# ha7ilm/csdr

Measured on AMD Instinct MI355X. Metric: complex MS/s in->out, WFM demod chain @2.4 MS/s x N streams, higher is better.
Workload: dtype f32

## Files before the change

### csdr_amd/__init__.py

```python
import ctypes as C
import os
import sys
import subprocess
import numpy as np

HERE = os.path.dirname(os.path.abspath(__file__))
LIB_PATH = os.environ.get("CSDR_AMD_LIB") or os.path.join(HERE, "libcsdr_amd.so")
ROOT = os.path.dirname(HERE)

c64 = np.complex64
f32 = np.float32

SHIFT = {"addition": 0, "math": 1, "table": 2, "unroll": 3, "addfast": 4}
WINDOWS = {"BOXCAR": 0, "BLACKMAN": 1, "HAMMING": 2}


class CsdrAmdError(RuntimeError):
    pass


def build(verbose=False):
    r = subprocess.run(["make", "-C", os.path.join(HERE, "csrc"), "-j8"], capture_output=True, text=True)
    if r.returncode != 0:
        raise CsdrAmdError("libcsdr_amd build failed:\n" + r.stdout[-4000:] + r.stderr[-4000:])
    if verbose:
        print(r.stdout)
    return LIB_PATH


class FastDDC(C.Structure):
    _fields_ = [(n, C.c_int) for n in ("pre_decimation", "post_decimation", "taps_length", "taps_min_length",
                                       "overlap_length", "fft_size", "fft_inv_size", "input_size", "post_input_size")] + \
               [("pre_shift", C.c_float), ("startbin", C.c_int), ("v", C.c_int), ("offsetbin", C.c_int),
                ("post_shift", C.c_float), ("output_scrape", C.c_int), ("scrap", C.c_int),
                ("sindelta", C.c_float), ("cosdelta", C.c_float), ("rate", C.c_float)]

    def as_dict(self):
        d = {n: getattr(self, n) for n, _ in self._fields_ if n not in ("sindelta", "cosdelta", "rate")}
        d["dsadata"] = (self.sindelta, self.cosdelta, self.rate)
        return d


_lib = None


def lib():
    global _lib
    if _lib is not None:
        return _lib
    if not os.path.exists(LIB_PATH):
        raise CsdrAmdError("%s is missing -- run `python -c 'import __graft_entry__ as g; g.build()'` first" % LIB_PATH)
    if "torch" not in sys.modules and not os.environ.get("CSDR_AMD_NO_TORCH_PRELOAD"):
        try:
            import torch
        except Exception:
            pass
    L = C.CDLL(LIB_PATH)
    vp, sz, i, fl = C.c_void_p, C.c_size_t, C.c_int, C.c_float
    L.csdr_amd_ctx_create.restype = vp; L.csdr_amd_ctx_create.argtypes = [i, vp]
    L.csdr_amd_ctx_destroy.argtypes = [vp]
    L.csdr_amd_ctx_sync.argtypes = [vp]
    L.csdr_amd_ctx_stream.restype = vp; L.csdr_amd_ctx_stream.argtypes = [vp]
    L.csdr_amd_last_error.restype = C.c_char_p
    L.csdr_amd_device_arch.restype = C.c_char_p; L.csdr_amd_device_arch.argtypes = [vp]
    L.csdr_amd_malloc.restype = vp; L.csdr_amd_malloc.argtypes = [vp, sz]
    L.csdr_amd_free.argtypes = [vp, vp]
    L.csdr_amd_h2d.argtypes = [vp, vp, vp, sz]
    L.csdr_amd_d2h.argtypes = [vp, vp, vp, sz]
    L.csdr_amd_memset.argtypes = [vp, vp, i, sz]
    sh = C.c_short
    L.csdr_amd_d2d.argtypes = [vp, vp, vp, sz]
    L.csdr_amd_amdemod_cf.argtypes = [vp, vp, vp, sz]
    L.csdr_amd_amdemod_estimator_cf.argtypes = [vp, vp, vp, sz, fl, fl]
    L.csdr_amd_realpart_cf.argtypes = [vp, vp, vp, sz]
    L.csdr_amd_logpower_cf.argtypes = [vp, vp, vp, sz, fl]
    L.csdr_amd_fmdemod_atan_cf.argtypes = [vp, vp, vp, i, sz, sz, sz, vp]
    L.csdr_amd_dcblock_ff.argtypes = [vp, vp, vp, i, sz, sz, sz, fl, vp]
    L.csdr_amd_fastdcblock_ff.argtypes = [vp, vp, vp, i, i, i, sz, sz, vp]
    L.csdr_amd_agc_ff.argtypes = [vp, vp, vp, i, sz, i, sz, sz, fl, fl, fl, fl, sh, sh, fl, vp]
    L.csdr_amd_precalculate_window.argtypes = [vp, i, i]; L.csdr_amd_precalculate_window.restype = None
    L.csdr_amd_fftcc_create.restype = vp; L.csdr_amd_fftcc_create.argtypes = [vp, i, i, i, i]
    L.csdr_amd_fftcc_destroy.argtypes = [vp]; L.csdr_amd_fftcc_destroy.restype = None
    L.csdr_amd_fftcc_process.argtypes = [vp, vp, sz, vp, C.POINTER(sz)]
    L.csdr_amd_encode_ima_adpcm_i16_u8.argtypes = [vp, vp, vp, i, sz, sz, sz, vp]
    L.csdr_amd_decode_ima_adpcm_u8_i16.argtypes = [vp, vp, vp, i, sz, sz, sz, vp]
    L.csdr_amd_compress_fft_adpcm_f_u8.argtypes = [vp, vp, vp, i, i]
    L.csdr_amd_waterfall_create.restype = vp; L.csdr_amd_waterfall_create.argtypes = [vp, i, i, i, i, fl, i, i, i, sz]
    L.csdr_amd_waterfall_process.argtypes = [vp, vp, sz, sz, vp, sz, C.POINTER(i)]
    L.csdr_amd_waterfall_reset.argtypes = [vp]
    L.csdr_amd_waterfall_kernel_name.restype = C.c_char_p; L.csdr_amd_waterfall_kernel_name.argtypes = [vp]
    L.csdr_amd_waterfall_force_generic.argtypes = [vp, i]
    L.csdr_amd_waterfall_destroy.argtypes = [vp]; L.csdr_amd_waterfall_destroy.restype = None
    ll = C.c_longlong
    L.csdr_amd_resampler_create.restype = vp; L.csdr_amd_resampler_create.argtypes = [vp, i, i, vp, i, i]
    L.csdr_amd_resampler_process.argtypes = [vp, vp, ll, sz, vp, sz, C.POINTER(ll)]
    L.csdr_amd_resampler_max_out.restype = ll; L.csdr_amd_resampler_max_out.argtypes = [vp, ll]
    L.csdr_amd_resampler_reset.argtypes = [vp]
    L.csdr_amd_resampler_set_cli_bufsize.argtypes = [vp, i]
    L.csdr_amd_resampler_set_last_taps_delay.argtypes = [vp, i]
    L.csdr_amd_resampler_force_generic.argtypes = [vp, i]
    L.csdr_amd_resampler_kernel_name.restype = C.c_char_p; L.csdr_amd_resampler_kernel_name.argtypes = [vp]
    L.csdr_amd_resampler_destroy.argtypes = [vp]; L.csdr_amd_resampler_destroy.restype = None
    L.csdr_amd_resampler_window.argtypes = [i, i, i, i, i, vp]
    L.csdr_amd_interp_create.restype = vp; L.csdr_amd_interp_create.argtypes = [vp, i, vp, i, i]
    L.csdr_amd_interp_process.argtypes = [vp, vp, ll, sz, vp, sz, C.POINTER(ll)]
    L.csdr_amd_interp_max_out.restype = ll; L.csdr_amd_interp_max_out.argtypes = [vp, ll]
    L.csdr_amd_interp_reset.argtypes = [vp]
    L.csdr_amd_interp_set_cli_bufsize.argtypes = [vp, i]
    L.csdr_amd_interp_force_generic.argtypes = [vp, i]
    L.csdr_amd_interp_kernel_name.restype = C.c_char_p; L.csdr_amd_interp_kernel_name.argtypes = [vp]
    L.csdr_amd_interp_destroy.argtypes = [vp]; L.csdr_amd_interp_destroy.restype = None
    L.csdr_amd_psk31_create.restype = vp; L.csdr_amd_psk31_create.argtypes = [vp, vp, i, i, i]
    L.csdr_amd_psk31_process.argtypes = [vp, vp, ll, sz, vp, sz, vp, vp, vp]
    L.csdr_amd_psk31_max_out.restype = ll; L.csdr_amd_psk31_max_out.argtypes = [vp, ll]
    L.csdr_amd_psk31_reset.argtypes = [vp]
    L.csdr_amd_psk31_reset_channel.argtypes = [vp, i]
    L.csdr_amd_psk31_get_channel.argtypes = [vp, i, vp]
    L.csdr_amd_psk31_set_channel.argtypes = [vp, i, vp]
    L.csdr_amd_psk31_set_lanes.argtypes = [vp, i]
    L.csdr_amd_psk31_force_generic.argtypes = [vp, i]
    L.csdr_amd_psk31_lanes.argtypes = [vp]
    L.csdr_amd_psk31_kernel_name.restype = C.c_char_p; L.csdr_amd_psk31_kernel_name.argtypes = [vp]
    L.csdr_amd_psk31_destroy.argtypes = [vp]; L.csdr_amd_psk31_destroy.restype = None
    L.csdr_amd_simple_agc_cc.argtypes = [vp, vp, vp, i, ll, sz, sz, C.c_float, C.c_float, C.c_float, vp]
    L.csdr_amd_psk31_varicode_decoder_push.restype = C.c_char; L.csdr_amd_psk31_varicode_decoder_push.argtypes = [vp, C.c_ubyte]
    L.csdr_amd_psk31_varicode_table.restype = None; L.csdr_amd_psk31_varicode_table.argtypes = [vp]
    L.csdr_amd_debug_psk31_walk.restype = ll; L.csdr_amd_debug_psk31_walk.argtypes = [vp, i, i, vp, ll, vp, i, vp, vp, vp, vp]
    L.csdr_amd_rtty_create.restype = vp; L.csdr_amd_rtty_create.argtypes = [vp, vp, i, i, i]
    L.csdr_amd_rtty_process.argtypes = [vp, vp, ll, sz, vp, sz, vp]
    L.csdr_amd_rtty_max_out.restype = ll; L.csdr_amd_rtty_max_out.argtypes = [vp, ll]
    L.csdr_amd_rtty_reset.argtypes = [vp]
    L.csdr_amd_rtty_reset_channel.argtypes = [vp, i]
    L.csdr_amd_rtty_force_generic.argtypes = [vp, i]
    L.csdr_amd_rtty_kernel_name.restype = C.c_char_p; L.csdr_amd_rtty_kernel_name.argtypes = [vp]
    L.csdr_amd_rtty_destroy.argtypes = [vp]; L.csdr_amd_rtty_destroy.restype = None
    L.csdr_amd_bfsk_demod_cf.argtypes = [vp, vp, vp, i, ll, sz, sz, vp, vp, i, i]
    L.csdr_amd_bfsk_last_kernel.restype = C.c_char_p; L.csdr_amd_bfsk_last_kernel.argtypes = []
    L.csdr_amd_binary_slicer_f_u8.argtypes = [vp, vp, vp, i, ll, sz, sz]
    L.csdr_amd_rtty_line_decoder_u8_u8.argtypes = [vp, vp, vp, i, ll, sz, sz, vp, vp]
    L.csdr_amd_serial_line_decoder_f_u8.argtypes = [vp, vp, vp, i, i, sz, sz, C.c_float, i, C.c_float, C.c_float, vp, vp]
    L.csdr_amd_rtty_baudot_decoder_lookup.restype = C.c_char; L.csdr_amd_rtty_baudot_decoder_lookup.argtypes = [vp, C.c_ubyte]
    L.csdr_amd_rtty_baudot_decoder_push.restype = C.c_char; L.csdr_amd_rtty_baudot_decoder_push.argtypes = [vp, C.c_ubyte]
    L.csdr_amd_firdes_add_peak_c.restype = None; L.csdr_amd_firdes_add_peak_c.argtypes = [vp, i, C.c_float, i, i, i]
    L.csdr_amd_firdes_peak_c.restype = None; L.csdr_amd_firdes_peak_c.argtypes = [vp, i, C.c_float, i]
    L.csdr_amd_debug_rtty_walk.restype = ll; L.csdr_amd_debug_rtty_walk.argtypes = [vp, i, i, vp, ll, vp, i, vp]
    L.csdr_amd_squelch_create.restype = vp; L.csdr_amd_squelch_create.argtypes = [vp, i, i, i, vp, ll]
    L.csdr_amd_squelch_process.argtypes = [vp, vp, ll, sz, vp, sz, vp, sz, vp, vp]
    L.csdr_amd_squelch_set_level.argtypes = [vp, i, fl]
    L.csdr_amd_squelch_get_level.restype = fl; L.csdr_amd_squelch_get_level.argtypes = [vp, i]
    L.csdr_amd_squelch_block_index.restype = ll; L.csdr_amd_squelch_block_index.argtypes = [vp, i]
    L.csdr_amd_squelch_max_blocks.argtypes = [vp]
    L.csdr_amd_squelch_reset.argtypes = [vp]
    L.csdr_amd_squelch_reset_channel.argtypes = [vp, i]
    L.csdr_amd_squelch_force_generic.argtypes = [vp, i]
    L.csdr_amd_squelch_kernel_name.restype = C.c_char_p; L.csdr_amd_squelch_kernel_name.argtypes = [vp]
    L.csdr_amd_squelch_destroy.argtypes = [vp]; L.csdr_amd_squelch_destroy.restype = None
    L.csdr_amd_get_power_c.argtypes = [vp, vp, i, i, i, i, sz, vp]
    L.csdr_amd_get_power_f.argtypes = [vp, vp, i, i, i, i, sz, vp]
    L.csdr_amd_squelch_report_due.argtypes = [i, ll]
    L.csdr_amd_squelch_gate_open.argtypes = [fl, fl]
    L.csdr_amd_debug_squelch_power.restype = fl; L.csdr_amd_debug_squelch_power.argtypes = [vp, i, i, i]
    L.csdr_amd_costas_params.argtypes = [fl, fl, i, vp]
    L.csdr_amd_pll_params_p.argtypes = [fl, vp]
    L.csdr_amd_pll_params_pi.argtypes = [fl, fl, fl, fl, vp]
    L.csdr_amd_carrier_create.restype = vp; L.csdr_amd_carrier_create.argtypes = [vp, vp, i]
    L.csdr_amd_carrier_process.argtypes = [vp, vp, ll, sz, vp, vp, vp, vp, sz]
    L.csdr_amd_carrier_reset.argtypes = [vp]
    L.csdr_amd_carrier_reset_channel.argtypes = [vp, i]
    L.csdr_amd_carrier_get_channel.argtypes = [vp, i, vp]
    L.csdr_amd_carrier_set_channel.argtypes = [vp, i, vp]
    L.csdr_amd_carrier_set_lanes.argtypes = [vp, i]
    L.csdr_amd_carrier_lanes.argtypes = [vp]
    L.csdr_amd_carrier_force_generic.argtypes = [vp, i]
    L.csdr_amd_carrier_kernel_name.restype = C.c_char_p; L.csdr_amd_carrier_kernel_name.argtypes = [vp]
    L.csdr_amd_carrier_destroy.argtypes = [vp]; L.csdr_amd_carrier_destroy.restype = None
    L.csdr_amd_debug_carrier_walk.restype = ll; L.csdr_amd_debug_carrier_walk.argtypes = [vp, vp, ll, vp, i, vp, vp, vp, vp, vp]
    L.csdr_amd_fmmod_fc.argtypes = [vp, vp, vp, i, sz, sz, sz, vp]
    L.csdr_amd_dsb_fc.argtypes = [vp, vp, vp, sz, fl]
    L.csdr_amd_add_dcoffset_cc.argtypes = [vp, vp, vp, sz]
    L.csdr_amd_fixed_amplitude_cc.argtypes = [vp, vp, vp, sz, fl]
    L.csdr_amd_convert_f_samplerf.argtypes = [vp, vp, vp, sz, C.c_uint]
    L.csdr_amd_debug_fmmod_walk.restype = ll; L.csdr_amd_debug_fmmod_walk.argtypes = [vp, ll, vp, i, vp, vp, vp]
    L.csdr_amd_txbank_create.restype = vp; L.csdr_amd_txbank_create.argtypes = [vp, i, i, fl, fl, i, vp, i, vp, i, sz]
    L.csdr_amd_txbank_process.argtypes = [vp, vp, sz, ll, vp, sz, C.POINTER(ll)]
    L.csdr_amd_txbank_set_rate.argtypes = [vp, i, fl]
    L.csdr_amd_txbank_get_rate.restype = fl; L.csdr_amd_txbank_get_rate.argtypes = [vp, i]
    L.csdr_amd_txbank_reset.argtypes = [vp]
    L.csdr_amd_txbank_max_out.restype = ll; L.csdr_amd_txbank_max_out.argtypes = [vp, ll]
    L.csdr_amd_txbank_force_generic.argtypes = [vp, i]
    L.csdr_amd_txbank_kernel_name.restype = C.c_char_p; L.csdr_amd_txbank_kernel_name.argtypes = [vp]
    L.csdr_amd_txbank_destroy.argtypes = [vp]; L.csdr_amd_txbank_destroy.restype = None
    L.csdr_amd_rational_resampler_get_lowpass_f.restype = None; L.csdr_amd_rational_resampler_get_lowpass_f.argtypes = [vp, i, i, i, i]
    L.csdr_amd_debug_resampler_schedule.argtypes = [i, i, i, i, i, vp]
    L.csdr_amd_logaveragepower_cf.argtypes = [vp, vp, vp, i, i, i, fl]
    L.csdr_amd_fft_exchange_sides_ff.argtypes = [vp, vp, vp, i, i]
    L.csdr_amd_accumulate_power_cf.argtypes = [vp, vp, vp, sz]
    L.csdr_amd_log_ff.argtypes = [vp, vp, vp, sz, fl]
    L.csdr_amd_timer_start.argtypes = [vp]
    L.csdr_amd_timer_stop_ms.argtypes = [vp, C.POINTER(fl)]
    L.csdr_amd_firdes_filter_len.argtypes = [fl]
    L.csdr_amd_firdes_lowpass_f.argtypes = [vp, i, fl, i]
    L.csdr_amd_firdes_bandpass_c.argtypes = [vp, i, fl, fl, i]
    L.csdr_amd_nfm_deemph_taps.argtypes = [i, C.POINTER(vp)]
    L.csdr_amd_shift_addition_init.argtypes = [fl, vp]
    for nm in ("u8_f", "s8_f", "s16_f", "f_u8", "f_s8", "f_s16"):
        getattr(L, "csdr_amd_convert_" + nm).argtypes = [vp, vp, vp, sz]
    L.csdr_amd_convert_f_s24.argtypes = [vp, vp, vp, sz, i]
    L.csdr_amd_convert_s24_f.argtypes = [vp, vp, vp, sz, i]
    L.csdr_amd_rotator_generate.argtypes = [vp, i, fl, C.POINTER(fl), vp, sz, i, i]
    L.csdr_amd_mix_cc.argtypes = [vp, vp, vp, vp, i, sz, sz, sz]
    L.csdr_amd_mix_fc.argtypes = [vp, vp, vp, vp, i, sz, sz, sz]
    L.csdr_amd_shift_cc.argtypes = [vp, i, fl, C.POINTER(fl), vp, vp, i, sz, sz, sz, i, i]
    L.csdr_amd_decimating_shift_addition_cc.argtypes = [vp, vp, vp, i, i, sz, sz, vp, i, vp]
    L.csdr_amd_fir_decimate_cc.argtypes = [vp, vp, vp, i, i, sz, sz, i, vp, i]
    L.csdr_amd_fir_last_kernel.restype = C.c_char_p; L.csdr_amd_fir_last_kernel.argtypes = []
    L.csdr_amd_fir_last_instance.restype = C.c_char_p; L.csdr_amd_fir_last_instance.argtypes = []
    L.csdr_amd_fir_ff_last_instance.restype = C.c_char_p; L.csdr_amd_fir_ff_last_instance.argtypes = []
    L.csdr_amd_fir_ff.argtypes = [vp, vp, vp, i, i, sz, sz, vp, i]
    L.csdr_amd_fmdemod_quadri_cf.argtypes = [vp, vp, vp, i, sz, sz, sz, vp]
    L.csdr_amd_limit_ff.argtypes = [vp, vp, vp, sz, fl]
    L.csdr_amd_gain_ff.argtypes = [vp, vp, vp, sz, fl]
    L.csdr_amd_deemphasis_wfm_ff.argtypes = [vp, vp, vp, i, sz, sz, sz, fl, i, vp]
    L.csdr_amd_fastagc_ff.argtypes = [vp, vp, vp, i, i, i, sz, sz, fl, vp]
    L.csdr_amd_fracdec_create.restype = vp; L.csdr_amd_fracdec_create.argtypes = [fl, i, vp, i]
    L.csdr_amd_fracdec_destroy.argtypes = [vp]
    L.csdr_amd_fractional_decimator_ff.argtypes = [vp, vp, vp, vp, i, i, sz, sz, C.POINTER(i)]
    L.csdr_amd_fracdec_set_cli_bufsize.restype = None; L.csdr_amd_fracdec_set_cli_bufsize.argtypes = [vp, i]
    L.csdr_amd_fftfilt_create.restype = vp; L.csdr_amd_fftfilt_create.argtypes = [vp, i, vp, i, i, i]
    L.csdr_amd_fftfilt_destroy.argtypes = [vp]
    L.csdr_amd_fftfilt_input_size.argtypes = [vp]
    L.csdr_amd_fftfilt_reset.argtypes = [vp]
    L.csdr_amd_fftfilt_kernel_name.restype = C.c_char_p; L.csdr_amd_fftfilt_kernel_name.argtypes = [vp]
    L.csdr_amd_fftfilt_window.argtypes = [vp]
    L.csdr_amd_fftfilt_process.argtypes = [vp, vp, vp, i, sz, sz]
    L.csdr_amd_fft_c2c.argtypes = [vp, vp, vp, i, i]
    L.csdr_amd_fastddc_init.argtypes = [vp, fl, i, fl]
    L.csdr_amd_fastddc_fwd_create.restype = vp; L.csdr_amd_fastddc_fwd_create.argtypes = [vp, vp, i]
    L.csdr_amd_fastddc_fwd_destroy.argtypes = [vp]
    L.csdr_amd_fastddc_fwd_process.argtypes = [vp, vp, vp, i]
    L.csdr_amd_fastddc_inv_create.restype = vp; L.csdr_amd_fastddc_inv_create.argtypes = [vp, fl, i, vp, i, i, i]
    L.csdr_amd_fastddc_inv_destroy.argtypes = [vp]
    L.csdr_amd_fastddc_inv_geometry.argtypes = [vp, i, vp]
    L.csdr_amd_fastddc_inv_max_output.argtypes = [vp, i]
    L.csdr_amd_fastddc_inv_process.argtypes = [vp, vp, i, vp, sz, vp]
    L.csdr_amd_fastddc_bank_create.restype = vp; L.csdr_amd_fastddc_bank_create.argtypes = [vp, fl, i, vp, i, i, i]
    L.csdr_amd_fastddc_bank_destroy.argtypes = [vp]; L.csdr_amd_fastddc_bank_destroy.restype = None
    L.csdr_amd_fastddc_bank_set_rate.argtypes = [vp, i, fl]
    L.csdr_amd_fastddc_bank_input_size.argtypes = [vp]
    L.csdr_amd_fastddc_bank_max_output.argtypes = [vp, i]
    L.csdr_amd_fastddc_bank_process.argtypes = [vp, vp, i, vp, sz, vp]
    L.csdr_amd_fastddc_bank_inverse.restype = vp; L.csdr_amd_fastddc_bank_inverse.argtypes = [vp]
    L.csdr_amd_fastddc_bank_submit.argtypes = [vp, vp, i]
    L.csdr_amd_fastddc_bank_collect.argtypes = [vp, vp, sz, vp]
    L.csdr_amd_comm_unique_id.argtypes = [vp]
    L.csdr_amd_comm_create.restype = vp; L.csdr_amd_comm_create.argtypes = [vp, vp, i, i]
    L.csdr_amd_comm_destroy.argtypes = [vp]; L.csdr_amd_comm_destroy.restype = None
    L.csdr_amd_comm_rank.argtypes = [vp]; L.csdr_amd_comm_world.argtypes = [vp]
    L.csdr_amd_comm_broadcast.argtypes = [vp, vp, sz, i]
    L.csdr_amd_comm_dup.restype = vp; L.csdr_amd_comm_dup.argtypes = [vp]
    L.csdr_amd_comm_selftest.argtypes = [vp, sz, C.c_char_p, sz]
    L.csdr_amd_fastddc_bank_create_sharded.restype = vp; L.csdr_amd_fastddc_bank_create_sharded.argtypes = [vp, fl, i, vp, i, i, i, vp]
    L.csdr_amd_fastddc_bank_channel_slice.argtypes = [vp, C.POINTER(i), C.POINTER(i)]
    L.csdr_amd_fastddc_bank_create_sharded_by.restype = vp; L.csdr_amd_fastddc_bank_create_sharded_by.argtypes = [vp, fl, i, vp, i, i, i, vp, i]
    L.csdr_amd_fastddc_bank_shard_mode.argtypes = [vp]
    L.csdr_amd_fastddc_bank_default_shard_mode.argtypes = [i]
    L.csdr_amd_fastddc_bank_local_blocks.argtypes = [vp, i, C.POINTER(i), C.POINTER(i)]
    L.csdr_amd_fastddc_bank_overlap.argtypes = [vp]
    L.csdr_amd_fastddc_bank_submit_local.argtypes = [vp, vp, i]
    if hasattr(L, "csdr_amd_fastddc_bank_process_s16"):
        for nm in ("s16", "u8"):
            getattr(L, "csdr_amd_fastddc_bank_process_" + nm).argtypes = [vp, vp, i, vp, sz, vp]
            getattr(L, "csdr_amd_fastddc_bank_submit_" + nm).argtypes = [vp, vp, i]
            getattr(L, "csdr_amd_fastddc_bank_submit_local_" + nm).argtypes = [vp, vp, i]
    L.csdr_amd_fastddc_bank_finish.argtypes = [vp, vp]
    L.csdr_amd_fastddc_bank_set_rate_global.argtypes = [vp, i, fl]
    L.csdr_amd_loopback_create.restype = vp; L.csdr_amd_loopback_create.argtypes = [i]
    L.csdr_amd_loopback_destroy.argtypes = [vp]; L.csdr_amd_loopback_destroy.restype = None
    L.csdr_amd_loopback_abort.argtypes = [vp]; L.csdr_amd_loopback_abort.restype = None
    L.csdr_amd_comm_create_loopback.restype = vp; L.csdr_amd_comm_create_loopback.argtypes = [vp, vp, i]
    L.csdr_amd_comm_create_null.restype = vp; L.csdr_amd_comm_create_null.argtypes = [vp, i, i]
    L.csdr_amd_comm_create_ipc.restype = vp; L.csdr_amd_comm_create_ipc.argtypes = [vp, C.c_char_p, i, i]
    L.csdr_amd_fastddc_inv_kernel_name.restype = C.c_char_p; L.csdr_amd_fastddc_inv_kernel_name.argtypes = [vp]
    L.csdr_amd_fastddc_inv_set_profiling.argtypes = [vp, i]
    L.csdr_amd_fastddc_inv_kernel_time.argtypes = [vp, C.POINTER(C.c_double), C.POINTER(C.c_long)]
    L.csdr_amd_fastddc_inv_stage_time.argtypes = [vp, i, C.POINTER(C.c_double), C.POINTER(C.c_long)]
    L.csdr_amd_wfm_create.restype = vp; L.csdr_amd_wfm_create.argtypes = [vp, i, fl, i, vp, i, i, fl, i, sz]
    L.csdr_amd_wfm_destroy.argtypes = [vp]
    L.csdr_amd_wfm_reset.argtypes = [vp]
    L.csdr_amd_wfm_process.restype = C.c_long; L.csdr_amd_wfm_process.argtypes = [vp, vp, sz, sz, vp, vp, sz]
    L.csdr_amd_wfm_kernel_name.restype = C.c_char_p; L.csdr_amd_wfm_kernel_name.argtypes = [vp]
    ll = C.c_longlong; db = C.c_double
    L.csdr_amd_wfm_ring_create.restype = vp; L.csdr_amd_wfm_ring_create.argtypes = [vp, i, fl, i, vp, i, i, fl, i, sz, i]
    L.csdr_amd_wfm_ring_destroy.argtypes = [vp]; L.csdr_amd_wfm_ring_destroy.restype = None
    L.csdr_amd_wfm_ring_reset.argtypes = [vp]
    L.csdr_amd_wfm_ring_acquire.argtypes = [vp, ll, db]
    L.csdr_amd_wfm_ring_input.restype = vp; L.csdr_amd_wfm_ring_input.argtypes = [vp, ll, C.POINTER(sz)]
    L.csdr_amd_wfm_ring_submit.restype = ll; L.csdr_amd_wfm_ring_submit.argtypes = [vp]
    L.csdr_amd_wfm_ring_wait.restype = C.c_long; L.csdr_amd_wfm_ring_wait.argtypes = [vp, ll, db]
    L.csdr_amd_wfm_ring_output.restype = vp; L.csdr_amd_wfm_ring_output.argtypes = [vp, ll, C.POINTER(sz)]
    L.csdr_amd_wfm_ring_set_rate.argtypes = [vp, fl]
    L.csdr_amd_wfm_ring_get_rate.restype = fl; L.csdr_amd_wfm_ring_get_rate.argtypes = [vp]
    L.csdr_amd_wfm_ring_set_timeouts.argtypes = [vp, db, db]
    L.csdr_amd_wfm_ring_resident.argtypes = [vp]
    L.csdr_amd_wfm_ring_stop.argtypes = [vp]
    L.csdr_amd_wfm_ring_slots.argtypes = [vp]
    L.csdr_amd_wfm_ring_grid.argtypes = [vp]
    L.csdr_amd_wfm_ring_launches.restype = C.c_long; L.csdr_amd_wfm_ring_launches.argtypes = [vp]
    L.csdr_amd_wfm_ring_submitted.restype = ll; L.csdr_amd_wfm_ring_submitted.argtypes = [vp]
    L.csdr_amd_wfm_ring_block_times.argtypes = [vp, ll, C.POINTER(db), C.POINTER(db)]
    L.csdr_amd_wfm_ring_replay.argtypes = [vp, C.c_long, vp, vp]
    L.csdr_amd_wfm_ring_stats.argtypes = [vp, vp]
    L.csdr_amd_wfm_set_profiling.argtypes = [vp, i]
    L.csdr_amd_wfm_kernel_time.argtypes = [vp, C.POINTER(C.c_double), C.POINTER(C.c_long)]
    L.csdr_amd_ddc_create.restype = vp; L.csdr_amd_ddc_create.argtypes = [vp, i, fl, i, vp, i, sz]
    if hasattr(L, "csdr_amd_ddc_create_rates"):
        L.csdr_amd_ddc_create_rates.restype = vp; L.csdr_amd_ddc_create_rates.argtypes = [vp, i, vp, i, vp, i, sz]
        L.csdr_amd_ddc_set_rate.argtypes = [vp, i, fl]
        L.csdr_amd_ddc_get_rate.restype = fl; L.csdr_amd_ddc_get_rate.argtypes = [vp, i]
        L.csdr_amd_ddc_fallback.argtypes = [vp]
        L.csdr_amd_wfm_fallback.argtypes = [vp]
        L.csdr_amd_wfm_create_rates.restype = vp; L.csdr_amd_wfm_create_rates.argtypes = [vp, i, vp, i, vp, i, i, fl, i, sz]
        L.csdr_amd_wfm_set_rate.argtypes = [vp, i, fl]
        L.csdr_amd_wfm_get_rate.restype = fl; L.csdr_amd_wfm_get_rate.argtypes = [vp, i]
        L.csdr_amd_nfm_create_rates.restype = vp; L.csdr_amd_nfm_create_rates.argtypes = [vp, i, vp, i, vp, i, i, i, fl, fl, sz]
        L.csdr_amd_nfm_set_rate.argtypes = [vp, i, fl]
    L.csdr_amd_ddc_destroy.argtypes = [vp]
    L.csdr_amd_ddc_reset.argtypes = [vp]
    L.csdr_amd_ddc_process.restype = C.c_long; L.csdr_amd_ddc_process.argtypes = [vp, vp, sz, sz, vp, sz]
    L.csdr_amd_ddc_kernel_name.restype = C.c_char_p; L.csdr_amd_ddc_kernel_name.argtypes = [vp]
    L.csdr_amd_ddc_set_profiling.argtypes = [vp, i]
    L.csdr_amd_ddc_kernel_time.argtypes = [vp, C.POINTER(C.c_double), C.POINTER(C.c_long)]
    L.csdr_amd_nfm_create.restype = vp; L.csdr_amd_nfm_create.argtypes = [vp, i, fl, i, vp, i, i, i, fl, fl, sz]
    L.csdr_amd_nfm_destroy.argtypes = [vp]
    L.csdr_amd_nfm_reset.argtypes = [vp]
    L.csdr_amd_nfm_process.restype = C.c_long; L.csdr_amd_nfm_process.argtypes = [vp, vp, sz, sz, vp, vp, sz]
    L.csdr_amd_nfm_front_end.restype = vp; L.csdr_amd_nfm_front_end.argtypes = [vp]
    _lib = L
    return L


def _hp(a):
    return a.ctypes.data_as(C.c_void_p)


class DevBuf:

    def __init__(self, ctx, nbytes):
        self.ctx, self.nbytes = ctx, int(nbytes)
        self.ptr = lib().csdr_amd_malloc(ctx.h, max(self.nbytes, 16))
        if not self.ptr:
            raise CsdrAmdError(ctx.err())

    def free(self):
        if self.ptr and self.ctx.h:
            lib().csdr_amd_free(self.ctx.h, self.ptr)
        self.ptr = None

    def __del__(self):
        try:
            self.free()
        except Exception:
            pass

    def at(self, byte_offset):
        return C.c_void_p(self.ptr + int(byte_offset))


class Waterfall:

    def __init__(self, ctx, fft_size, every_n, avgnumber, add_db, window, in_format, out_format, n_streams, max_samples_per_call):
        self.ctx, self.fft, self.every, self.avg, self.n_streams, self.max_in = ctx, fft_size, every_n, avgnumber, n_streams, int(max_samples_per_call)
        self.in_format, self.out_format = in_format, out_format
        self.h = ctx.L.csdr_amd_waterfall_create(ctx.h, fft_size, every_n, WINDOWS[window], avgnumber, add_db, 1 if in_format == "u8" else 0,
                                                 1 if out_format == "adpcm" else 0, n_streams, self.max_in)
        if not self.h:
            raise CsdrAmdError(ctx.err())
        self.row_bytes = 4 * fft_size if out_format == "db" else (fft_size + 10) // 2

    def max_rows(self, n_in):
        return (n_in + self.fft) // self.every + 2

    def process_dev(self, d_in, n_in, in_pitch, d_out, out_pitch):
        rows = C.c_int(0)
        self.ctx.check(self.ctx.L.csdr_amd_waterfall_process(self.h, d_in, n_in, in_pitch, d_out, out_pitch, C.byref(rows)), "waterfall_process")
        return rows.value

    def process(self, x, calls=None):
        x = np.ascontiguousarray(x, np.uint8 if self.in_format == "u8" else c64)
        if x.ndim == 1:
            x = x[None]
        n = x.shape[1] // 2 if self.in_format == "u8" else x.shape[1]
        eb = 2 if self.in_format == "u8" else 8
        calls = [n] if calls is None else list(calls)
        di = self.ctx.upload(x)
        opitch = (self.max_rows(max(calls)) * self.row_bytes + 255) // 256 * 256
        do = self.ctx.alloc(opitch * self.n_streams + 256)
        out = [[] for _ in range(self.n_streams)]
        at = 0
        for k in calls:
            r = self.process_dev(di.at(eb * at), k, n, do.ptr, opitch)
            if r:
                y = self.ctx.download(do, np.uint8, opitch * self.n_streams).reshape(self.n_streams, opitch)[:, :r * self.row_bytes]
                for s in range(self.n_streams):
                    out[s].append(y[s].copy())
            at += k
        dt = f32 if self.out_format == "db" else np.uint8
        per = self.fft if self.out_format == "db" else self.row_bytes
        return np.stack([np.concatenate(o).view(dt).reshape(-1, per) if o else np.zeros((0, per), dt) for o in out])

    def kernel_name(self):
        return self.ctx.L.csdr_amd_waterfall_kernel_name(self.h).decode()

    def force_generic(self, on=True):
        self.ctx.check(self.ctx.L.csdr_amd_waterfall_force_generic(self.h, int(on)), "waterfall_force_generic")

    def reset(self):
        self.ctx.check(self.ctx.L.csdr_amd_waterfall_reset(self.h), "waterfall_reset")

    def close(self):
        if self.h:
            self.ctx.L.csdr_amd_waterfall_destroy(self.h)
            self.h = None

    def __del__(self):
        try:
            self.close()
        except Exception:
            pass


def rational_resampler_get_lowpass_f(taps_length, interpolation, decimation, window="HAMMING"):
    t = np.zeros(taps_length, f32)
    lib().csdr_amd_rational_resampler_get_lowpass_f(_hp(t), taps_length, interpolation, decimation, WINDOWS[window])
    return t


def fir_interpolate_lowpass_f(taps_length, interpolation, window="HAMMING"):
    t = np.zeros(taps_length, f32)
    lib().csdr_amd_firdes_lowpass_f(_hp(t), taps_length, C.c_float(np.float32(0.5) / np.float32(interpolation)), WINDOWS[window])
    return t


def resampler_schedule(interpolation, decimation, taps_length, n, last_taps_delay=0):
    out = np.zeros((n, 3), np.int32)
    if lib().csdr_amd_debug_resampler_schedule(interpolation, decimation, taps_length, last_taps_delay, n, _hp(out)) < 0:
        raise CsdrAmdError(lib().csdr_amd_last_error().decode())
    return out


def resampler_window(interpolation, decimation, taps_length, input_size, last_taps_delay=0):
    st = np.zeros(3, np.int32)
    if lib().csdr_amd_resampler_window(interpolation, decimation, taps_length, input_size, last_taps_delay, _hp(st)) < 0:
        raise CsdrAmdError(lib().csdr_amd_last_error().decode())
    return tuple(int(v) for v in st)


class _Resampling:
    _dt, _eb, _pre = f32, 4, "resampler"

    def _fn(self, name):
        return getattr(self.ctx.L, "csdr_amd_%s_%s" % (self._pre, name))

    def max_out(self, n_in):
        return int(self._fn("max_out")(self.h, n_in))

    def process_dev(self, d_in, n_in, in_pitch, d_out, out_pitch):
        n = C.c_longlong(0)
        self.ctx.check(self._fn("process")(self.h, d_in, n_in, in_pitch, d_out, out_pitch, C.byref(n)), self._pre + "_process")
        return n.value

    def process(self, x, calls=None):
        x = np.ascontiguousarray(x, self._dt)
        squeeze = x.ndim == 1
        if squeeze:
            x = x[None]
        s, n = x.shape
        calls = [n] if calls is None else list(calls)
        di = self.ctx.upload(x)
        opitch = max(self.max_out(max(calls) if calls else 0), 1)
        do = self.ctx.alloc(self._eb * opitch * s + 256)
        out, at = [], 0
        for k in calls:
            r = self.process_dev(di.at(self._eb * at), k, n, do.ptr, opitch)
            if r:
                out.append(self.ctx.download(do, self._dt, opitch * s).reshape(s, opitch)[:, :r].copy())
            at += k
        y = np.concatenate(out, axis=1) if out else np.zeros((s, 0), self._dt)
        return y[0] if squeeze else y

    def reset(self):
        self.ctx.check(self._fn("reset")(self.h), self._pre + "_reset")

    def set_cli_bufsize(self, the_bufsize):
        self.ctx.check(self._fn("set_cli_bufsize")(self.h, int(the_bufsize)), self._pre + "_set_cli_bufsize")

    def force_generic(self, on=True):
        self.ctx.check(self._fn("force_generic")(self.h, int(on)), self._pre + "_force_generic")

    def kernel_name(self):
        return self._fn("kernel_name")(self.h).decode()

    def close(self):
        if self.h:
            self._fn("destroy")(self.h)
            self.h = None

    def __del__(self):
        try:
            self.close()
        except Exception:
            pass


class Resampler(_Resampling):

    def __init__(self, ctx, interpolation, decimation, taps, n_streams=1, bufsize=None, last_taps_delay=0):
        self.ctx, self.I, self.D, self.n_streams = ctx, interpolation, decimation, n_streams
        self.taps = np.ascontiguousarray(taps, f32)
        self.h = ctx.L.csdr_amd_resampler_create(ctx.h, interpolation, decimation, _hp(self.taps), self.taps.size, n_streams)
        if not self.h:
            raise CsdrAmdError(ctx.err())
        if bufsize:
            self.set_cli_bufsize(bufsize)
        if last_taps_delay:
            self.set_last_taps_delay(last_taps_delay)

    def set_last_taps_delay(self, d):
        self.ctx.check(self.ctx.L.csdr_amd_resampler_set_last_taps_delay(self.h, int(d)), "resampler_set_last_taps_delay")


class Psk31Params(C.Structure):
    _fields_ = [("rate", C.c_float), ("reference", C.c_float), ("max_gain", C.c_float), ("algorithm", C.c_int), ("decimation", C.c_int),
                ("loop_gain", C.c_float), ("max_error", C.c_float), ("use_q", C.c_int)]


class Psk31Chan(C.Structure):
    _fields_ = [("gain", C.c_float), ("tail_len", C.c_int), ("correction_offset", C.c_int), ("base", C.c_uint), ("last_i", C.c_float),
                ("last_q", C.c_float), ("varicode_shr", C.c_ulonglong)]


PSK31_STAGES = {"agc": 0, "timing": 1, "dbpsk": 2, "varicode": 3}
TIMING_ALGORITHMS = {"GARDNER": 0, "EARLYLATE": 1}


def psk31_params(rate=0.001, reference=0.5, max_gain=65535.0, algorithm="GARDNER", decimation=256, loop_gain=0.5, max_error=2.0, use_q=True):
    alg = TIMING_ALGORITHMS[algorithm] if isinstance(algorithm, str) else int(algorithm)
    return Psk31Params(rate, reference, max_gain, alg, decimation, loop_gain, max_error, int(bool(use_q)))


def _psk31_stage(s):
    return PSK31_STAGES[s] if isinstance(s, str) else int(s)


def _psk31_types(first, last):
    return (np.uint8 if first == 3 else c64), (c64 if last <= 1 else np.uint8)


def psk31_debug_walk(params, first="agc", last="varicode", x=None, cuts=(), state=None, with_extras=False):
    f, l = _psk31_stage(first), _psk31_stage(last)
    ti, to = _psk31_types(f, l)
    x = np.ascontiguousarray(x, ti)
    n = x.size
    cap = n + 16 if (f >= 2 or l == 0) else 2 * n // max(params.decimation, 1) + 3 * len(cuts) + 16
    out = np.zeros(cap, to)
    err = np.zeros(cap, f32) if with_extras else None
    idx = np.zeros(cap, np.uint32) if with_extras else None
    cu = np.ascontiguousarray(cuts, np.int64)
    k = lib().csdr_amd_debug_psk31_walk(C.byref(params), f, l, _hp(x), n, _hp(cu) if cu.size else None, cu.size, _hp(out),
                                        _hp(err) if with_extras else None, _hp(idx) if with_extras else None, C.byref(state) if state is not None else None)
    if k < 0:
        raise CsdrAmdError(lib().csdr_amd_last_error().decode())
    return (out[:k], err[:k], idx[:k]) if with_extras else out[:k]


def psk31_varicode_table():
    t = np.zeros(256, np.int32)
    lib().csdr_amd_psk31_varicode_table(_hp(t))
    return t.reshape(128, 2)


class Psk31:

    def __init__(self, ctx, params=None, n_channels=1, first="agc", last="varicode"):
        self.ctx, self.n_channels = ctx, n_channels
        self.params = params if params is not None else psk31_params()
        self.first, self.last = _psk31_stage(first), _psk31_stage(last)
        self.in_dtype, self.out_dtype = _psk31_types(self.first, self.last)
        self.h = ctx.L.csdr_amd_psk31_create(ctx.h, C.byref(self.params), n_channels, self.first, self.last)
        if not self.h:
            raise CsdrAmdError(ctx.err())

    def max_out(self, n_in):
        return int(self.ctx.L.csdr_amd_psk31_max_out(self.h, n_in))
# ... 1406 lines not shown
```

### csdr_amd/csrc/wfm.hip

```cpp
#include "common.hpp"
#include "wfm_mfma.hpp"
#include "seeds.hpp"
#include <math.h>
#include <stdlib.h>
#include <vector>
#include <string>
#include <string.h>
using namespace csdr_amd;

namespace {

constexpr int HIST = WFM_HIST;
constexpr int TILE_A = 64;
constexpr int WARM = 48;

struct WfmParams {
    int D, L, F;
    int T;
    long long B;
    long long j_first;
    int n_audio;
};

__device__ __forceinline__ float u8_to_f(uint32_t v) { return fmaf((float)v, 0x1.010102p-7f, -1.0f); }

__global__ __launch_bounds__(256) void k_wfm_front(const uint8_t *__restrict__ in, size_t in_pitch, const uint8_t *__restrict__ hist,
                                                   const cf32 *__restrict__ rot, const float *__restrict__ taps,
                                                   float *__restrict__ demod, size_t demod_pitch, WfmParams p)
{
    extern __shared__ float4 lds_raw[];
    float2 *win = reinterpret_cast<float2 *>(lds_raw);
    const int s = blockIdx.x;
    const int a0 = blockIdx.y * TILE_A;
    const int na = min(TILE_A, p.n_audio - a0);
    if (na <= 0) return;
    const long long j0 = p.j_first + a0;
    const int DF = p.D * p.F;
    const long long g_first = (long long)p.D * (p.F * j0 + 9);
    const long long g_last = (long long)p.D * (p.F * (j0 + na - 1) + 10) + p.L - 1;
    const long long r_first = (g_first - p.B) & ~7LL;
    const int wl = (int)(g_last - p.B - r_first + 1);
    const int nvec = (wl + 7) / 8;
    const uint8_t *row = in + (size_t)s * in_pitch;
    const uint8_t *hrow = hist + (size_t)s * (2 * HIST);
    float2 *ybuf = win + nvec * 8;
    for (int v = threadIdx.x; v < nvec; v += 256) {
        const long long r0 = r_first + 8LL * v;
        uint4 w = make_uint4(0x80808080u, 0x80808080u, 0x80808080u, 0x80808080u);
        if (r0 < 0) w = *reinterpret_cast<const uint4 *>(hrow + 2 * (r0 + HIST));
        else if (r0 + 8 <= p.T) w = *reinterpret_cast<const uint4 *>(row + 2 * r0);
        else {
            uint32_t b[4] = {0x80808080u, 0x80808080u, 0x80808080u, 0x80808080u};
            for (int k = 0; k < 16; k++) if (r0 + k / 2 < p.T) { const uint32_t by = row[2 * r0 + k]; b[k / 4] = (b[k / 4] & ~(0xffu << (8 * (k & 3)))) | (by << (8 * (k & 3))); }
            w = make_uint4(b[0], b[1], b[2], b[3]);
        }
        const cf32 *rr = rot + (r0 + HIST);
        const uint32_t ww[4] = {w.x, w.y, w.z, w.w};
#pragma unroll
        for (int k = 0; k < 4; k++) {
            const float i0 = u8_to_f(ww[k] & 0xff), q0 = u8_to_f((ww[k] >> 8) & 0xff);
            const float i1 = u8_to_f((ww[k] >> 16) & 0xff), q1 = u8_to_f(ww[k] >> 24);
            const float4 r2 = *reinterpret_cast<const float4 *>(rr + 2 * k);
            float4 o;
            o.x = r2.x * i0 - r2.y * q0; o.y = r2.y * i0 + r2.x * q0;
            o.z = r2.z * i1 - r2.w * q1; o.w = r2.w * i1 + r2.z * q1;
            *reinterpret_cast<float4 *>(win + 8 * v + 2 * k) = o;
        }
    }
    __syncthreads();
    {
        const int pidx = threadIdx.x >> 1, half = threadIdx.x & 1;
        const int a = pidx >> 1, which = pidx & 1;
        float ai = 0.f, aq = 0.f;
        if (a < na) {
            const long long g = (long long)p.D * (p.F * (j0 + a) + 9 + which);
            const float2 *x = win + (int)(g - p.B - r_first);
            const int split = (p.L + 1) / 2;
            const int t0 = half ? split : 0, t1 = half ? p.L : split;
            for (int t = t0; t < t1; t++) { const float h = taps[t]; const float2 v = x[t]; ai = fmaf(v.x, h, ai); aq = fmaf(v.y, h, aq); }
        }
        ai += __shfl_xor(ai, 1, 64); aq += __shfl_xor(aq, 1, 64);
        if (half == 0) ybuf[pidx] = make_float2(ai, aq);
    }
    __syncthreads();
    if (threadIdx.x < na) {
        const float2 pv = ybuf[2 * threadIdx.x], cv = ybuf[2 * threadIdx.x + 1];
        const float dq = cv.y - pv.y, di = cv.x - pv.x;
        const float num = cv.x * dq - cv.y * di, den = cv.x * cv.x + cv.y * cv.y;
        const float K = 0.340447550238101026565118445432744920253753662109375f;
        demod[(size_t)s * demod_pitch + a0 + threadIdx.x] = (den != 0.f) ? (K * num) / den : 0.f;
        (void)DF;
    }
}

constexpr int BK_SEG = 16, BK_CHUNK = 256 * BK_SEG;
__global__ __launch_bounds__(256) void k_wfm_back(const float *__restrict__ demod_base, size_t demod_pitch, int skip, int n_audio, float alpha,
                                                  const float *__restrict__ last_in, float *__restrict__ last_out,
                                                  int16_t *__restrict__ s16, float *__restrict__ audio_f, size_t out_pitch)
{
    __shared__ float seg[(BK_CHUNK + WARM) + (BK_CHUNK + WARM) / 16 + 16];
    const int s = blockIdx.y;
    const int t0 = blockIdx.x * BK_CHUNK;
    const int cnt = min(BK_CHUNK, n_audio - t0);
    if (cnt <= 0) return;
    const float *row = demod_base + (size_t)s * demod_pitch + skip;
    const int lead = (t0 >= WARM) ? WARM : t0;
    for (int q = threadIdx.x; q < cnt + lead; q += 256) seg[q + (q >> 4)] = row[t0 - lead + q];
    __syncthreads();
    const int my0 = threadIdx.x * BK_SEG;
    if (my0 >= cnt) return;
    const float one_minus = 1 - alpha;
    const int back = (my0 + lead >= WARM) ? WARM : (my0 + lead);
    int q = lead + my0 - back;
    float y = 0.f;
    if (t0 + my0 - back == 0) { y = last_in[s]; if (y != y) y = 0.f; }
    for (int k = 0; k < back; k++, q++) y = alpha * seg[q + (q >> 4)] + one_minus * y;
    const int mine = min(BK_SEG, cnt - my0);
    float e[BK_SEG];
#pragma unroll
    for (int k = 0; k < BK_SEG; k++) {
        if (k < mine) { y = alpha * seg[q + (q >> 4)] + one_minus * y; q++; }
        e[k] = y;
    }
    if (t0 + my0 + mine == n_audio) last_out[s] = y;
    uint32_t pk[BK_SEG / 2];
#pragma unroll
    for (int k = 0; k < BK_SEG; k += 2) {
        int iv[2];
#pragma unroll
        for (int h = 0; h < 2; h++) {
            const float scaled = e[k + h] * 32767.0f;
            iv[h] = (scaled >= -2147483648.0f && scaled < 2147483648.0f) ? (int)scaled : (int)0x80000000;
        }
        pk[k / 2] = (uint32_t)(iv[0] & 0xffff) | ((uint32_t)iv[1] << 16);
    }
    int16_t *dst = s16 + (size_t)s * out_pitch + t0 + my0;
    if (mine == BK_SEG && ((((uintptr_t)dst) & 15) == 0)) {
        reinterpret_cast<uint4 *>(dst)[0] = make_uint4(pk[0], pk[1], pk[2], pk[3]);
        reinterpret_cast<uint4 *>(dst)[1] = make_uint4(pk[4], pk[5], pk[6], pk[7]);
    } else {
#pragma unroll
        for (int k = 0; k < BK_SEG; k++) if (k < mine) dst[k] = (int16_t)((k & 1) ? (pk[k / 2] >> 16) : (pk[k / 2] & 0xffff));
    }
    if (audio_f) {
        float *df = audio_f + (size_t)s * out_pitch + t0 + my0;
#pragma unroll
        for (int k = 0; k < BK_SEG; k++) if (k < mine) df[k] = e[k];
    }
}

__global__ __launch_bounds__(256) void k_wfm_save_hist(const uint8_t *__restrict__ in, size_t in_pitch, int T, uint8_t *__restrict__ hist)
{
    const int s = blockIdx.x;
    const uint8_t *src = in + (size_t)s * in_pitch + 2 * (size_t)(T - HIST);
    uint8_t *dst = hist + (size_t)s * (2 * HIST);
    for (int k = threadIdx.x; k < 2 * HIST / 4; k += 256) reinterpret_cast<uint32_t *>(dst)[k] = reinterpret_cast<const uint32_t *>(src)[k];
}

}

struct csdr_amd_wfm {
    csdr_amd_ctx *ctx;
    int n_streams, D, L, F, audio_rate;
    float shift_rate, tau, alpha;
    size_t max_block;
    DevBuf<float> d_taps, d_demod, d_last[2];
    float phase;
    DevBuf<cf32> d_rot;
    DevBuf<uint8_t> d_hist;
    DevBuf<uint8_t> d_head[2]; int hflip;
    size_t demod_pitch;
    long long B, next_j;
    int last_T, flip;
    bool ended;
    std::string kernel_name;
    bool profiling;
    KernelTimer timer;
    double prof_ms; long prof_launches;
    bool use_mfma;
    WfmMfmaDevice mfma;
    DevBuf<> seq_frags; DevBuf<float> seq_cum; DevBuf<float2> dtab;
    DevBuf<float2> d_ctab; size_t ctab_cap;
    float2 c_prev;
    long long tab_first; bool tab_valid;
    bool ps; std::vector<float> rates, h_taps; DevBuf<float> d_scales;
    DevBuf<float2> d_dtab_old; DevBuf<int> d_lead_n; int *d_list; DevBuf<float> d_lead_d; std::vector<int> retuned;
    Owned<csdr_amd::SeedTables, seeds_destroy> seeds;
};

extern "C" {

static int wfm_upload_stream_tables(csdr_amd_wfm *w, int s, float rate)
{
    WfmMfmaTable t;
    wfm_mfma_build_table(w->D, w->L, w->F, rate, w->h_taps.data(), t);
    CSDR_HIP(hipMemcpy((uint8_t *)w->mfma.d_seq_frags + (size_t)s * t.seq_frags.size(), t.seq_frags.data(), t.seq_frags.size(), hipMemcpyHostToDevice));
    CSDR_HIP(hipMemcpy(w->mfma.d_seq_cum + (size_t)s * t.seq_cum.size(), t.seq_cum.data(), t.seq_cum.size() * sizeof(float), hipMemcpyHostToDevice));
    CSDR_HIP(hipMemcpy(w->mfma.d_dtab + (size_t)s * t.dtab.size(), t.dtab.data(), t.dtab.size() * sizeof(float2), hipMemcpyHostToDevice));
    CSDR_HIP(hipMemcpy(w->d_scales.get() + s, &t.seq_scale, sizeof(float), hipMemcpyHostToDevice));
    return 0;
}

static csdr_amd_wfm *wfm_create_impl(csdr_amd_ctx *ctx, int n_streams, const float *rates, bool per_stream, int decimation, const float *host_taps,
                                     int taps_length, int frac_rate, float tau, int audio_rate, size_t max_block_samples)
{
    const float shift_rate = rates ? rates[0] : 0.f;
    if (n_streams <= 0 || decimation <= 0 || taps_length <= 0 || frac_rate <= 1 || !rates) { fail_msg(-3, "wfm: bad parameters"); return nullptr; }
    if (decimation * 1 + taps_length + 8 > HIST) { fail_msg(-3, "wfm: D + taps (%d + %d) exceed the %d-sample history", decimation, taps_length, HIST); return nullptr; }
    if (max_block_samples < 1024) max_block_samples = 1024;
    Owned<csdr_amd_wfm, csdr_amd_wfm_destroy> w(new csdr_amd_wfm());
    w->ctx = ctx; w->n_streams = n_streams; w->D = decimation; w->L = taps_length; w->F = frac_rate; w->audio_rate = audio_rate;
    w->shift_rate = shift_rate; w->tau = tau; w->max_block = max_block_samples;
    const float dt = (float)(1.0 / audio_rate); w->alpha = dt / (tau + dt);
    const size_t max_audio = max_block_samples / ((size_t)decimation * frac_rate) + 8;
    w->demod_pitch = (max_audio + 40 + 63) & ~(size_t)63;
    hipError_t e = hipSuccess;
    auto alloc = [&](auto &p, size_t bytes) { if (e == hipSuccess) e = dev_alloc(p, bytes); };
    w->ps = per_stream;
    {
        const char *force = getenv("CSDR_AMD_WFM_PATH");
        w->use_mfma = !(force && !strcmp(force, "valu")) && wfm_mfma_supported(decimation, taps_length, frac_rate);
    }
    if (per_stream && !w->use_mfma) { fail_msg(-3, "wfm_create_rates: a rate per stream needs the matrix-core chain kernel (decimation x audio decimation even, window <= 256 samples)"); return nullptr; }
    alloc(w->d_taps, sizeof(float) * taps_length);
    alloc(w->d_last[0], sizeof(float) * n_streams);
    alloc(w->d_last[1], sizeof(float) * n_streams);
    if (w->use_mfma) {
        alloc(w->d_head[0], wfm_mfma_head_bytes(n_streams));
        alloc(w->d_head[1], wfm_mfma_head_bytes(n_streams));
    } else {
        alloc(w->d_demod, sizeof(float) * w->demod_pitch * n_streams);
        alloc(w->d_rot, sizeof(cf32) * (HIST + max_block_samples + 64));
        alloc(w->d_hist, (size_t)2 * HIST * n_streams);
    }
    if (e != hipSuccess) { fail(e, "hipMalloc(wfm state)", __FILE__, __LINE__); return nullptr; }
    (void)hipMemcpy(w->d_taps.get(), host_taps, sizeof(float) * taps_length, hipMemcpyHostToDevice);
    w->kernel_name = "k_wfm_front";
    if (w->use_mfma && per_stream) {
        WfmMfmaTable t;
        wfm_mfma_build_table(decimation, taps_length, frac_rate, shift_rate, host_taps, t);
        w->mfma.tile_stride_bytes = t.tile_stride_bytes; w->mfma.win_off_bytes = t.win_off_bytes; w->mfma.seq_scale = t.seq_scale;
        w->rates.assign(rates, rates + n_streams); w->h_taps.assign(host_taps, host_taps + taps_length);
        hipError_t e2 = dev_alloc(w->seq_frags, t.seq_frags.size() * (size_t)n_streams);
        if (e2 == hipSuccess) e2 = dev_alloc(w->seq_cum, t.seq_cum.size() * sizeof(float) * (size_t)n_streams);
        if (e2 == hipSuccess) e2 = dev_alloc(w->dtab, t.dtab.size() * sizeof(float2) * (size_t)n_streams);
        if (e2 == hipSuccess) e2 = dev_alloc(w->d_scales, sizeof(float) * (size_t)n_streams);
        w->mfma.d_seq_frags = w->seq_frags.get(); w->mfma.d_seq_cum = w->seq_cum.get(); w->mfma.d_dtab = w->dtab.get();
        if (e2 != hipSuccess) { fail(e2, "hipMalloc(wfm per-stream tables)", __FILE__, __LINE__); return nullptr; }
        for (int s = 0; s < n_streams; s++) if (wfm_upload_stream_tables(w.get(), s, rates[s])) return nullptr;
        w->seeds.reset(seeds_create(ctx, n_streams, rates, nullptr, 0, max_block_samples));
        if (!w->seeds) return nullptr;
        w->kernel_name = "k_wfm_mfma_seq";
    } else if (w->use_mfma) {
        WfmMfmaTable t;
        wfm_mfma_build_table(decimation, taps_length, frac_rate, shift_rate, host_taps, t);
        w->mfma.tile_stride_bytes = t.tile_stride_bytes; w->mfma.win_off_bytes = t.win_off_bytes; w->mfma.seq_scale = t.seq_scale;
        w->ctab_cap = 16 * (max_block_samples / 1024 + 8);
        hipError_t e2 = dev_alloc(w->d_ctab, w->ctab_cap * sizeof(float2));
        if (e2 == hipSuccess) e2 = dev_alloc(w->seq_frags, t.seq_frags.size());
        if (e2 == hipSuccess) e2 = dev_alloc(w->seq_cum, t.seq_cum.size() * sizeof(float));
        if (e2 == hipSuccess) e2 = dev_alloc(w->dtab, t.dtab.size() * sizeof(float2));
        w->mfma.d_seq_frags = w->seq_frags.get(); w->mfma.d_seq_cum = w->seq_cum.get(); w->mfma.d_dtab = w->dtab.get();
        if (e2 == hipSuccess) e2 = hipMemcpy(w->mfma.d_seq_frags, t.seq_frags.data(), t.seq_frags.size(), hipMemcpyHostToDevice);
        if (e2 == hipSuccess) e2 = hipMemcpy(w->mfma.d_seq_cum, t.seq_cum.data(), t.seq_cum.size() * sizeof(float), hipMemcpyHostToDevice);
        if (e2 == hipSuccess) e2 = hipMemcpy(w->mfma.d_dtab, t.dtab.data(), t.dtab.size() * sizeof(float2), hipMemcpyHostToDevice);
        if (e2 != hipSuccess) { fail(e2, "hipMalloc/hipMemcpy(wfm mfma table)", __FILE__, __LINE__); return nullptr; }
        w->kernel_name = "k_wfm_mfma_seq";
    }
    w->profiling = false; w->prof_ms = 0; w->prof_launches = 0;
    if (csdr_amd_wfm_reset(w.get())) return nullptr;
    return w.release();
}

csdr_amd_wfm *csdr_amd_wfm_create(csdr_amd_ctx *ctx, int n_streams, float shift_rate, int decimation, const float *host_taps,
                                  int taps_length, int frac_rate, float tau, int audio_rate, size_t max_block_samples)
{
    return wfm_create_impl(ctx, n_streams, &shift_rate, false, decimation, host_taps, taps_length, frac_rate, tau, audio_rate, max_block_samples);
}

csdr_amd_wfm *csdr_amd_wfm_create_rates(csdr_amd_ctx *ctx, int n_streams, const float *shift_rates, int decimation, const float *host_taps,
                                        int taps_length, int frac_rate, float tau, int audio_rate, size_t max_block_samples)
{
    return wfm_create_impl(ctx, n_streams, shift_rates, true, decimation, host_taps, taps_length, frac_rate, tau, audio_rate, max_block_samples);
}

int csdr_amd_wfm_set_rate(csdr_amd_wfm *w, int stream, float shift_rate)
{
    if (!w->ps) return fail_msg(-3, "wfm_set_rate: the object shares one rate (create it with csdr_amd_wfm_create_rates)");
    if (stream < 0 || stream >= w->n_streams) return fail_msg(-3, "wfm_set_rate: stream %d out of range", stream);
    if (w->rates[stream] == shift_rate) return 0;
    CSDR_HIP(hipStreamSynchronize(w->ctx->stream));
    if (!w->d_dtab_old) CSDR_HIP(dev_alloc(w->d_dtab_old, sizeof(float2) * 3072 * (size_t)w->n_streams));
    bool listed = false;
    for (int v : w->retuned) listed |= v == stream;
    if (!listed) {
        CSDR_HIP(hipMemcpy(w->d_dtab_old.get() + (size_t)stream * 3072, w->mfma.d_dtab + (size_t)stream * 3072, sizeof(float2) * 3072, hipMemcpyDeviceToDevice));
        w->retuned.push_back(stream);
    }
    const int rc = wfm_upload_stream_tables(w, stream, shift_rate); if (rc) return rc;
    w->rates[stream] = shift_rate;
    return seeds_set_rate(w->seeds.get(), stream, shift_rate, false);
}

float csdr_amd_wfm_get_rate(const csdr_amd_wfm *w, int stream) { return w->ps ? ((stream >= 0 && stream < w->n_streams) ? w->rates[stream] : 0.f) : w->shift_rate; }

void csdr_amd_wfm_destroy(csdr_amd_wfm *w)
{
    if (!w) return;
    (void)hipStreamSynchronize(w->ctx->stream);
    delete w;
}

int csdr_amd_wfm_reset(csdr_amd_wfm *w)
{
    hipStream_t st = w->ctx->stream;
    w->phase = 0.f;
    CSDR_HIP(hipMemsetAsync(w->d_last[0].get(), 0, sizeof(float) * w->n_streams, st));
    CSDR_HIP(hipMemsetAsync(w->d_last[1].get(), 0, sizeof(float) * w->n_streams, st));
    if (w->d_rot) CSDR_HIP(hipMemsetAsync(w->d_rot.get(), 0, sizeof(cf32) * (HIST + w->max_block + 64), st));
    if (w->d_hist) CSDR_HIP(hipMemsetAsync(w->d_hist.get(), 0x80, (size_t)2 * HIST * w->n_streams, st));
    for (int k = 0; k < 2; k++) if (w->d_head[k]) CSDR_HIP(hipMemsetAsync(w->d_head[k].get(), 0x80, wfm_mfma_head_bytes(w->n_streams), st));
    w->hflip = 0;
    w->B = 0; w->next_j = 0; w->last_T = 0; w->flip = 0; w->ended = false;
    w->c_prev = make_float2(1.f, 0.f); w->tab_valid = false; w->tab_first = 0;
    w->retuned.clear();
    if (w->seeds) { const int rc = seeds_reset(w->seeds.get()); if (rc) return rc; }
    return 0;
}

const char *csdr_amd_wfm_kernel_name(const csdr_amd_wfm *w) { return w->kernel_name.c_str(); }
int csdr_amd_wfm_fallback(const csdr_amd_wfm *w) { return w->use_mfma ? 0 : 1; }

int csdr_amd_wfm_set_profiling(csdr_amd_wfm *w, int on)
{
    w->profiling = on != 0; w->timer.reset(); w->prof_ms = 0; w->prof_launches = 0;
    return 0;
}

int csdr_amd_wfm_kernel_time(csdr_amd_wfm *w, double *total_ms, long *launches)
{
    CSDR_HIP(hipStreamSynchronize(w->ctx->stream));
    if (const int rc = w->timer.resolve(&w->prof_ms, &w->prof_launches)) return rc;
    if (total_ms) *total_ms = w->prof_ms;
    if (launches) *launches = w->prof_launches;
    return 0;
}

long csdr_amd_wfm_process(csdr_amd_wfm *w, const uint8_t *in, size_t in_pitch, size_t block_samples,
                          int16_t *audio_s16, float *audio_f, size_t out_pitch)
{
    csdr_amd_ctx *c = w->ctx; hipStream_t st = c->stream;
    if (w->ended) return fail_msg(-3, "wfm: stream already ended by a block that was not a multiple of 1024 samples; reset first");
    if (block_samples == 0) return 0;
    if (block_samples > w->max_block) return fail_msg(-3, "wfm: block of %zu samples exceeds max_block_samples %zu", block_samples, w->max_block);
    if (((uintptr_t)in & 15) || (in_pitch & 15)) return fail_msg(-3, "wfm: input pointer and pitch must be 16-byte aligned");
    const int T = (int)block_samples;
    int rc = 0;
    const float2 *ctab_call = nullptr;
    SeedView sv; memset(&sv, 0, sizeof sv);
    if (w->ps) {
        const size_t nch = ((size_t)T + 1023) / 1024;
        rc = seeds_acquire(w->seeds.get(), w->B / 1024 - 1, nch + 3, (T % 1024) ? 0 : nch, &sv); if (rc) return rc;
        ctab_call = sv.ctab;
    } else
    if (w->use_mfma) {
        const size_t nch = ((size_t)T + 1023) / 1024;
        const long long first = w->B / 1024 - 1;
        const float inc = (w->shift_rate * 2) * PI_F;
        if (nch + 3 > w->ctab_cap) return fail_msg(-3, "wfm: chunk table too small");
        if (!w->tab_valid || first < w->tab_first || first + (long long)nch + 3 > w->tab_first + (long long)w->ctab_cap) {
            float2 *hc = (float2 *)c->pinned_acquire(sizeof(float2) * w->ctab_cap);
            if (!hc) return -2;
            float ph = w->phase;
            hc[0] = w->c_prev;
            for (size_t k = 1; k < w->ctab_cap; k++) {
                hc[k] = make_float2((float)cos((double)ph), (float)sin((double)ph));
                float nx = ph + inc * (float)1024;
                while (nx > PI_F) nx -= 2 * PI_F;
                while (nx < -PI_F) nx += 2 * PI_F;
                ph = nx;
            }
            rc = c->pinned_upload(w->d_ctab.get(), sizeof(float2) * w->ctab_cap); if (rc) return rc;
            w->tab_first = first; w->tab_valid = true;
        }
        ctab_call = w->d_ctab.get() + (first - w->tab_first);
        float ph = w->phase;
        for (size_t m = 0; m < nch; m++) {
            if (m + 1 == nch) w->c_prev = make_float2((float)cos((double)ph), (float)sin((double)ph));
            const int len = ((size_t)T - m * 1024 < 1024) ? (int)((size_t)T - m * 1024) : 1024;
            float nx = ph + inc * (float)len;
            while (nx > PI_F) nx -= 2 * PI_F;
            while (nx < -PI_F) nx += 2 * PI_F;
            ph = nx;
        }
        w->phase = ph;
    } else {
        if (w->last_T) CSDR_HIP(hipMemcpyAsync(w->d_rot.get(), w->d_rot.get() + w->last_T, sizeof(cf32) * HIST, hipMemcpyDeviceToDevice, st));
        rc = csdr_amd_rotator_generate(c, CSDR_SHIFT_ADDITION, w->shift_rate, &w->phase, w->d_rot.get() + HIST, (size_t)T, 1024, 0);
        if (rc) return rc;
    }
    const long long avail_last = w->B + T - 1;
    long long j_hi = -1;
    if (avail_last - (w->L - 1) >= 0) {
        const long long k_max = (avail_last - (w->L - 1)) / w->D;
        if (k_max >= 10) j_hi = (k_max - 10) / w->F;
    }
    const long long n_audio_ll = j_hi - w->next_j + 1;
    const int n_audio = n_audio_ll > 0 ? (int)n_audio_ll : 0;
    if (n_audio > 0 && (size_t)n_audio > out_pitch) return fail_msg(-3, "wfm: out_pitch %zu smaller than the %d audio samples of this block", out_pitch, n_audio);
    hipEvent_t e0 = nullptr, e1 = nullptr;
    if (w->profiling && n_audio > 0) { if (const int trc = w->timer.take(&e0, &e1)) return trc; }
    if (w->use_mfma) {
        WfmBackArgs back;
        back.alpha = w->alpha; back.last_in = w->d_last[w->flip].get(); back.last_out = w->d_last[w->flip ^ 1].get();
        back.s16 = audio_s16; back.af = audio_f; back.out_pitch = out_pitch; back.head_in = w->d_head[w->hflip].get(); back.head_out = w->d_head[w->hflip ^ 1].get();
        WfmPerStream psa; memset(&psa, 0, sizeof psa);
        if (w->ps) {
            psa.tab_pitch = sv.pitch; psa.tab_len = sv.n_entries; psa.d_scales = w->d_scales.get();
            long n_lead = 0; const int lead_max = wfm_lead_max(w->D, w->L, w->F);
            psa.lead_stride = lead_max;
            if (!w->retuned.empty() && n_audio > 0) {
                const long long lim = w->B - 1 - 9LL * w->D;
                if (lim >= 0) n_lead = (long)(lim / ((long long)w->D * w->F) - w->next_j + 1);
                if (n_lead < 0) n_lead = 0;
                if (n_lead > lead_max) n_lead = lead_max;
                if (n_lead > n_audio) n_lead = n_audio;
            }
            if (n_lead > 0) {
                const int nr = (int)w->retuned.size(), S = w->n_streams;
                if (!w->d_lead_n) { CSDR_HIP(dev_alloc(w->d_lead_n, sizeof(int) * 2 * S)); w->d_list = w->d_lead_n.get() + S; CSDR_HIP(dev_alloc(w->d_lead_d, sizeof(float) * (size_t)lead_max * S)); }
                int *hl = (int *)c->pinned_acquire(sizeof(int) * (size_t)(S + nr)); if (!hl) return -2;
                for (int s = 0; s < S; s++) hl[s] = 0;
                for (int k = 0; k < nr; k++) { hl[w->retuned[k]] = (int)n_lead; hl[S + k] = w->retuned[k]; }
                rc = c->pinned_upload(w->d_lead_n.get(), sizeof(int) * (size_t)(S + nr)); if (rc) return rc;
                rc = wfm_mfma_lead(st, in, in_pitch, back.head_in, w->d_taps.get(), sv.ctab, sv.pitch, w->mfma.d_dtab, w->d_dtab_old.get(), w->d_list, nr, w->d_lead_d.get(), lead_max,
                                   w->D, w->L, w->F, w->B, w->next_j, (int)n_lead);
                if (rc) return rc;
                psa.d_lead_d = w->d_lead_d.get(); psa.d_lead_n = w->d_lead_n.get();
            }
        }
        rc = wfm_mfma_launch(st, e0, e1, in, in_pitch, w->mfma, ctab_call, w->n_streams, T, w->B, w->next_j, n_audio, back, w->ps ? &psa : nullptr);
        if (rc) return rc;
        if (n_audio > 0) w->retuned.clear();
        w->hflip ^= 1;
        if (n_audio > 0) w->flip ^= 1;
    } else {
        if ((size_t)n_audio + 40 > w->demod_pitch) return fail_msg(-3, "wfm: internal audio buffer too small");
        if (n_audio > 0) {
            WfmParams p; p.D = w->D; p.L = w->L; p.F = w->F; p.T = T; p.B = w->B; p.j_first = w->next_j; p.n_audio = n_audio;
            const int span = w->D * (w->F * (TILE_A - 1) + 1) + w->L + 16;
            const size_t lds = (size_t)((span + 7) / 8 * 8 + 2 * TILE_A) * sizeof(float2) + 64;
            if (lds > 64 * 1024) { const int arc = lds_attr_once((const void *)k_wfm_front, lds); if (arc) return arc; }
            if (e0) CSDR_HIP(hipEventRecord(e0, st));
            hipLaunchKernelGGL(k_wfm_front, dim3(w->n_streams, cdiv(n_audio, TILE_A)), dim3(256), lds, st,
                               in, in_pitch, w->d_hist.get(), w->d_rot.get(), w->d_taps.get(), w->d_demod.get(), w->demod_pitch, p);
            CSDR_LAUNCH_CHECK();
            if (e1) CSDR_HIP(hipEventRecord(e1, st));
            hipLaunchKernelGGL(k_wfm_back, dim3(cdiv(n_audio, BK_CHUNK), w->n_streams), dim3(256), 0, st,
                               w->d_demod.get(), w->demod_pitch, 0, n_audio, w->alpha, w->d_last[w->flip].get(), w->d_last[w->flip ^ 1].get(), audio_s16, audio_f, out_pitch);
            CSDR_LAUNCH_CHECK();
            w->flip ^= 1;
        }
        if (T >= HIST) {
            hipLaunchKernelGGL(k_wfm_save_hist, dim3(w->n_streams), dim3(256), 0, st, in, in_pitch, T, w->d_hist.get());
            CSDR_LAUNCH_CHECK();
        }
    }
    if (T % 1024) w->ended = true;
    w->B += T; w->next_j += n_audio; w->last_T = T;
    return n_audio;
}

}
```

### csdr_amd/csrc/wfm_mfma.hip

```cpp
#include "common.hpp"
#include "wfm_mfma.hpp"
#include <hip/hip_ext.h>
#include <math.h>
#include <string.h>
#include <stdlib.h>
#include <complex>
#include <vector>
using namespace csdr_amd;

namespace csdr_amd {

bool wfm_mfma_supported(int D, int L, int F)
{
    if ((D * F) & 1) return false;
    const int win_off = (18 * D) & ~15;
    const int span_bytes = 2 * (D * (3 * F + 10) + L) - win_off;
    if (span_bytes > 64 * WFM_NK) return false;
    if (D + L + 3 * D * F + 8 > WFM_HIST) return false;
    return true;
}

void wfm_mfma_build_table(int D, int L, int F, float shift_rate, const float *taps, WfmMfmaTable &t)
{
    t.D = D; t.L = L; t.F = F;
    t.tile_stride_bytes = 8 * D * F;
    t.win_off_bytes = (18 * D) & ~15;
    const float rate2 = shift_rate * 2, inc = rate2 * PI_F;
    const float sd = (float)sin((double)inc), cd = (float)cos((double)inc);
    const std::complex<double> d((double)cd, (double)sd);
    const double mag = std::abs(d), ang = std::arg(d);
    const double a = 2.0 / 255.0;
    const int base_off_samples = t.win_off_bytes / 2;
    {
        t.dtab.resize(3072);
        for (int i = 0; i < 3072; i++) { const std::complex<double> v = std::polar(pow(mag, i - 2048), ang * (i - 2048)); t.dtab[i] = make_float2((float)v.real(), (float)v.imag()); }
        const double dmax = fmax(1.0, pow(mag, 32 * WFM_NK));
        double g2 = 0;
        for (int k = 0; k < L; k++) g2 = fmax(g2, fabs(a * (double)taps[k]));
        g2 *= dmax * 1.0001; if (g2 == 0) g2 = 1;
        const double qs = 4194304.0 / g2;
        t.seq_scale = (float)(g2 / 4194304.0);
        t.seq_frags.assign((size_t)WFM_NK * 3 * 64 * 16, 0);
        const int ngr = 4 * WFM_NK;
        std::vector<double> gsum((size_t)ngr * 16, 0.0);
        for (int r = 0; r < 16; r++) {
            const int q = r / 4, which = (r % 4) / 2, comp = r % 2;
            const long off = (long)D * (F * q + 9 + which) - base_off_samples;
            for (int tp = 0; tp < L; tp++) {
                const long ts = off + tp;
                const std::complex<double> G = a * (double)taps[tp] * std::polar(pow(mag, (double)ts), ang * (double)ts);
                for (int c = 0; c < 2; c++) {
                    const double val = comp == 0 ? (c == 0 ? G.real() : -G.imag()) : (c == 0 ? G.imag() : G.real());
                    const long colb = 2 * ts + c;
                    const int ks = (int)(colb / 64), b = (int)(colb % 64);
                    long qv = lrint(val * qs);
                    const int w2 = (int)(((qv + 128) % 256 + 256) % 256) - 128; qv = (qv - w2) / 256;
                    const int w1 = (int)(((qv + 128) % 256 + 256) % 256) - 128; qv = (qv - w1) / 256;
                    const int dig[3] = {(int)qv, w1, w2};
                    for (int l = 0; l < 3; l++) t.seq_frags[((size_t)(ks * 3 + l) * 64 + (16 * (b / 16) + r)) * 16 + b % 16] = (int8_t)dig[l];
                    gsum[(size_t)(colb / 16) * 16 + r] += val;
                }
            }
        }
        t.seq_cum.assign((size_t)(ngr + 1) * 16, 0.f);
        for (int r = 0; r < 16; r++) {
            double run = 0;
            for (int g = 0; g <= ngr; g++) { t.seq_cum[(size_t)g * 16 + r] = (float)(0.5 * run); if (g < ngr) run += gsum[(size_t)g * 16 + r]; }
        }
    }
}

}

namespace {

typedef int v4i __attribute__((ext_vector_type(4)));

__device__ __forceinline__ float combine_digits(int a0, int a1, int a2)
{
    return fmaf((float)a0, 65536.0f, fmaf((float)a1, 256.0f, (float)a2));
}

__device__ __forceinline__ void tile_rows(const v4i (&acc)[3], const v4i (&snap)[3], bool two, float scale, const float (&k0)[4], const float (&k1)[4],
                                          float2 C0, float2 C1, float &pI, float &pQ, float &cI, float &cQ)
{
    float u0[4];
    if (two) {
        float u1[4];
#pragma unroll
        for (int r = 0; r < 4; r++) {
            u0[r] = fmaf(combine_digits(snap[0][r], snap[1][r], snap[2][r]), scale, k0[r]);
            u1[r] = fmaf(combine_digits(acc[0][r] - snap[0][r], acc[1][r] - snap[1][r], acc[2][r] - snap[2][r]), scale, k1[r]);
        }
        pI = C0.x * u0[0] - C0.y * u0[1] + (C1.x * u1[0] - C1.y * u1[1]); pQ = C0.x * u0[1] + C0.y * u0[0] + (C1.x * u1[1] + C1.y * u1[0]);
        cI = C0.x * u0[2] - C0.y * u0[3] + (C1.x * u1[2] - C1.y * u1[3]); cQ = C0.x * u0[3] + C0.y * u0[2] + (C1.x * u1[3] + C1.y * u1[2]);
    } else {
#pragma unroll
        for (int r = 0; r < 4; r++) u0[r] = fmaf(combine_digits(acc[0][r], acc[1][r], acc[2][r]), scale, k0[r]);
        pI = C0.x * u0[0] - C0.y * u0[1]; pQ = C0.x * u0[1] + C0.y * u0[0];
        cI = C0.x * u0[2] - C0.y * u0[3]; cQ = C0.x * u0[3] + C0.y * u0[2];
    }
}

template <int N> __device__ __forceinline__ void wait_vmcnt() { asm volatile("s_waitcnt vmcnt(%0)" :: "n"(N) : "memory"); }

template <int KB>
__device__ __forceinline__ void wfm_chain(const v4i (&A)[WFM_NK * 3], const v4i (&Bf)[WFM_NK], bool lo_lane, v4i (&acc)[3], v4i (&snap)[3])
{
    const v4i z = {0, 0, 0, 0};
#pragma unroll
    for (int ks = 0; ks < WFM_NK; ks++) {
        if (ks == KB) {
            const v4i lo = lo_lane ? Bf[ks] : z, hi = lo_lane ? z : Bf[ks];
#pragma unroll
            for (int l = 0; l < 3; l++) acc[l] = __builtin_amdgcn_mfma_i32_16x16x64_i8(A[ks * 3 + l], lo, acc[l], 0, 0, 0);
#pragma unroll
            for (int l = 0; l < 3; l++) snap[l] = acc[l];
#pragma unroll
            for (int l = 0; l < 3; l++) acc[l] = __builtin_amdgcn_mfma_i32_16x16x64_i8(A[ks * 3 + l], hi, acc[l], 0, 0, 0);
        } else {
#pragma unroll
            for (int l = 0; l < 3; l++) acc[l] = __builtin_amdgcn_mfma_i32_16x16x64_i8(A[ks * 3 + l], Bf[ks], acc[l], 0, 0, 0);
        }
    }
}

struct SeqParams {
    int n_streams; long long B2; long long tile_first; int n_tiles, tiles_per_seg;
    int stride, win_off; float scale;
    long long two_T;
    float alpha; const float *last_in; float *last_out; int16_t *s16; float *af; size_t out_pitch; long long j_first; int n_audio;
    const uint8_t *head_in; uint8_t *head_out;
    long long col_bytes; int col_chunks, col_audio, n_cols;
    size_t frag_stride, tab_pitch; int tab_len;
    const float *scales;
    const float *lead_d; const int *lead_n; int lead_stride;
};

#ifndef SEQ_RB_KIB
#define SEQ_RB_KIB 9
#endif
constexpr int SEQ_RB = 1024 * SEQ_RB_KIB;
#ifndef SEQ_RING_PAD
#define SEQ_RING_PAD 32
#endif
constexpr int SEQ_RP = SEQ_RB + SEQ_RING_PAD;
constexpr int SEQ_NGR = 4 * WFM_NK;
#ifndef SEQ_TPG_N
#define SEQ_TPG_N 6
#endif
#ifndef SEQ_NLD_N
#define SEQ_NLD_N 2
#endif
constexpr int SEQ_TPG = SEQ_TPG_N;
constexpr int SEQ_NLD = SEQ_NLD_N;
constexpr int SEQ_NW = SEQ_TPG + SEQ_NLD;
constexpr int SEQ_NLW = SEQ_NLD;
constexpr int SEQ_LINE = 64;
constexpr int SEQ_OUTS = (SEQ_LINE - 1 + 3 * 4 * SEQ_TPG + 4 * SEQ_TPG - 1) / (4 * SEQ_TPG);
constexpr int SEQ_OUTR = SEQ_OUTS * 4 * SEQ_TPG;
constexpr int SEQ_OUTP = SEQ_OUTR + 4;
static_assert(16 % SEQ_NLW == 0 && (16 / SEQ_NLW) * 7 <= 63 && SEQ_TPG % 2 == 0, "rows per fetching wave (vmcnt counts to 63); the de-emphasis scan works on pairs");
constexpr int SEQ_HEAD = 1024;

#ifndef WFM_DIAG
#define WFM_DIAG 0
#endif
#ifdef WFM_PROF
__device__ unsigned long long g_wfm_prof[SEQ_NW][8];
__device__ unsigned long long g_wfm_life[SEQ_NW][4];
#define PROF_T(k) { const long long t_now = __builtin_readcyclecounter(); prof[k] += t_now - t_prev; t_prev = t_now; }
#else
#define PROF_T(k)
#endif

constexpr int RES_WARM = 48;
struct ResCtl {
    const uint32_t *desc;
    const uint32_t *ctrl;
    uint32_t *done;
    unsigned *cnt;
    unsigned long long *t_first;
    unsigned long long *next_item;
    unsigned *exiting;
    const uint8_t *in_ring; int16_t *out_ring; size_t in_slot_bytes, out_slot_elems;
    int n_slots, desc_lines, n_wsb, T, D, L, F;
    long long idle_ticks, life_ticks;
    const float *lead_d; int lead_stride;
    const float *lead_state;
    unsigned long long *stats;
    int fence_mode;
};
__device__ __forceinline__ uint32_t sys_load(const uint32_t *p) { return __hip_atomic_load(p, __ATOMIC_RELAXED, __HIP_MEMORY_SCOPE_SYSTEM); }
__device__ __forceinline__ uint32_t res_tag(long long k) { return (uint32_t)((unsigned long long)k % 0xfffffffeull) + 1u; }

template <bool PS, bool RES = false>
__global__ __launch_bounds__(64 * SEQ_NW) void k_wfm_mfma_seq(const uint8_t *__restrict__ in, size_t in_pitch, const v4i *__restrict__ frags, const float *__restrict__ cum,
                                                               const float2 *__restrict__ dtab, const float2 *__restrict__ ctab, SeqParams p_in, ResCtl rc)
{
    static_assert(!(PS && RES), "the resident form exists for the shared-rate kernel");
    constexpr int TPG = SEQ_TPG, SPW = 16 / SEQ_NLW, NTHR = 64 * SEQ_NW;
    extern __shared__ float4 lds_raw[];
    uint8_t *lds_in = reinterpret_cast<uint8_t *>(lds_raw);
    float *lds_out = reinterpret_cast<float *>(lds_in + 16 * SEQ_RP);
    float *lcum = lds_out + 16 * SEQ_OUTP;
    float2 *ctl = reinterpret_cast<float2 *>(lcum + (SEQ_NGR + 1) * 16);
    const int tid = threadIdx.x, wv = __builtin_amdgcn_readfirstlane(tid >> 6), lane = tid & 63, col = lane & 15, q = lane >> 4;
    const bool fetches = wv >= TPG;
#ifdef WFM_PROF
    const long long t_entry = __builtin_readcyclecounter();
    long long t_first = t_entry, t_last = t_entry;
#endif
    const int fw = wv - TPG;
    float scale = p_in.scale;
    if constexpr (PS) { const int sbp = blockIdx.x; frags += (size_t)sbp * p_in.frag_stride; cum += (size_t)sbp * ((SEQ_NGR + 1) * 16); dtab += (size_t)sbp * 3072; ctab += sbp; scale = p_in.scales[sbp]; }
    for (int i = tid; i < (SEQ_NGR + 1) * 16; i += NTHR) lcum[i] = cum[i];
    v4i A[WFM_NK * 3];
#pragma unroll
    for (int s = 0; s < WFM_NK * 3; s++) A[s] = frags[s * 64 + lane];

    float c_lo[4], c_hi[4];
    {
        const float4 a = *reinterpret_cast<const float4 *>(cum + 4 * q), b = *reinterpret_cast<const float4 *>(cum + (size_t)SEQ_NGR * 16 + 4 * q);
        c_lo[0] = a.x; c_lo[1] = a.y; c_lo[2] = a.z; c_lo[3] = a.w; c_hi[0] = b.x; c_hi[1] = b.y; c_hi[2] = b.z; c_hi[3] = b.w;
    }
    const float K = 0.340447550238101026565118445432744920253753662109375f;
    SeqParams p_res;
    if constexpr (RES) p_res = p_in;
    const SeqParams &p = RES ? p_res : p_in;
    unsigned long long item = 0;
    long long res_t_launch = 0;
    uint32_t *const rctl = reinterpret_cast<uint32_t *>(ctl);
    const float2 *const lseed = ctl + 1;
    long long st_wait = 0, st_body = 0, st_done = 0, st_items = 0, st_t = 0;
    if constexpr (RES) { item = rc.next_item[blockIdx.x]; res_t_launch = wall_clock64(); st_t = res_t_launch; }
    bool pend = false; unsigned pend_c = 0; int pend_slot = 0, pend_n = 0; long long pend_k = 0;
    uint32_t pre_v[4] = {0u, 0u, 0u, 0u}; bool pre_valid = false;
    auto res_complete = [&]() {
        if constexpr (RES) {
            if (tid == 0 && pend) {
                pend = false;
                if (pend_c + 1 == (unsigned)rc.n_wsb) {
                    const unsigned long long tf = __hip_atomic_exchange(rc.t_first + pend_slot, ~0ull, __ATOMIC_RELAXED, __HIP_MEMORY_SCOPE_AGENT), td = (unsigned long long)wall_clock64();
                    __hip_atomic_store(rc.cnt + pend_slot, 0u, __ATOMIC_RELAXED, __HIP_MEMORY_SCOPE_AGENT);
                    uint32_t *dn = rc.done + (size_t)pend_slot * 16;
                    __hip_atomic_store(dn + 1, (uint32_t)pend_n, __ATOMIC_RELAXED, __HIP_MEMORY_SCOPE_SYSTEM);
                    __hip_atomic_store(dn + 2, (uint32_t)tf, __ATOMIC_RELAXED, __HIP_MEMORY_SCOPE_SYSTEM); __hip_atomic_store(dn + 3, (uint32_t)(tf >> 32), __ATOMIC_RELAXED, __HIP_MEMORY_SCOPE_SYSTEM);
                    __hip_atomic_store(dn + 4, (uint32_t)td, __ATOMIC_RELAXED, __HIP_MEMORY_SCOPE_SYSTEM); __hip_atomic_store(dn + 5, (uint32_t)(td >> 32), __ATOMIC_RELAXED, __HIP_MEMORY_SCOPE_SYSTEM);
                    asm volatile("s_waitcnt vmcnt(0)" ::: "memory");
                    __hip_atomic_store(dn, res_tag(pend_k), __ATOMIC_RELAXED, __HIP_MEMORY_SCOPE_SYSTEM);
                }
            }
        }
    };
    for (;;) {
    int res_slot = 0, res_lead = 0; long long res_k = 0; bool res_retuned = false;
    const uint8_t *pblock = nullptr;
    if constexpr (RES) {
        res_k = (long long)(item / (unsigned)rc.n_wsb);
        res_slot = (int)(res_k % rc.n_slots);
        if (wv == 0) {
            const uint32_t *dsc = rc.desc + (size_t)res_slot * rc.desc_lines * 16;
            const uint32_t tag = res_tag(res_k);
            const int nd = rc.desc_lines * 16;
            const long long t_wait = wall_clock64();
            uint32_t state = 0;
            for (int iter = 0;; iter++) {
                uint32_t v[4] = {0u, 0u, 0u, 0u};
                bool have = false;
                if (iter == 0 && pre_valid) {
#pragma unroll
                    for (int j = 0; j < 4; j++) v[j] = pre_v[j];
                    have = true;
                } else {
                    const uint32_t t0 = sys_load(dsc);
                    if (t0 == tag) {
#pragma unroll
                        for (int j = 0; j < 4; j++) { const int d = lane + 64 * j; v[j] = d < nd ? sys_load(dsc + d) : 0u; }
                        have = true;
                    }
                }
                const uint32_t ex = __hip_atomic_load(rc.exiting, __ATOMIC_RELAXED, __HIP_MEMORY_SCOPE_AGENT);
                const uint32_t stop = (iter & 7) == 7 ? sys_load(rc.ctrl) : 0u;
                res_complete();
                bool ok = have;
#pragma unroll
                for (int j = 0; j < 4; j++) { const int d = lane + 64 * j; if (d < nd && (d & 15) == 0 && v[j] != tag) ok = false; }
                const bool ready = __all(ok);
                const long long now = wall_clock64();
                const bool old = now - res_t_launch > rc.life_ticks;
                if (ready && !ex && !old) {
#pragma unroll
                    for (int j = 0; j < 4; j++) {
                        const int d = lane + 64 * j, w = d & 15;
                        if (d < nd && w >= 2) rctl[2 + (d >> 4) * 14 + (w - 2)] = v[j];
                        if (d == 1) rctl[1] = v[j];
                    }
                    state = 1; break;
                }
                if (ex || old || stop || now - t_wait > rc.idle_ticks) { state = 2; break; }
                if (iter < 2) __builtin_amdgcn_s_sleep(24); else if (iter < 6) __builtin_amdgcn_s_sleep(64); else { __builtin_amdgcn_s_sleep(127); __builtin_amdgcn_s_sleep(100); }
            }
            pre_valid = false;
            if (lane == 0) rctl[0] = state;
        }
        __syncthreads();
        if (rctl[0] != 1u) {
            if (tid == 0) {
                __hip_atomic_store(rc.exiting, 1u, __ATOMIC_RELAXED, __HIP_MEMORY_SCOPE_AGENT); rc.next_item[blockIdx.x] = item;
                unsigned long long *sp = rc.stats + (size_t)blockIdx.x * 4;
                sp[0] += (unsigned long long)st_wait; sp[1] += (unsigned long long)st_body; sp[2] += (unsigned long long)st_done; sp[3] += (unsigned long long)st_items;
            }
            return;
        }
        if (tid == 0) { const long long t = wall_clock64(); st_wait += t - st_t; st_t = t; }
        res_lead = (int)(rctl[1] & 0xffu); res_retuned = (rctl[1] >> 8) & 1u;
        auto j_hi = [&](long long kk) -> long long {
            if (kk < 0) return -1;
            const long long avail_last = (kk + 1) * rc.T - 1;
            if (avail_last - (rc.L - 1) < 0) return -1;
            const long long k_max = (avail_last - (rc.L - 1)) / rc.D;
            return k_max >= 10 ? (k_max - 10) / rc.F : -1;
        };
        const long long jp = j_hi(res_k - 1), jn = j_hi(res_k);
        p_res.B2 = 2 * res_k * rc.T;
        p_res.j_first = jp + 1; p_res.n_audio = (int)(jn - jp);
        p_res.tile_first = p_res.j_first / 4; p_res.n_tiles = (int)((p_res.j_first + p_res.n_audio - 1) / 4 - p_res.tile_first + 1);
        p_res.tiles_per_seg = p_res.n_tiles;
        p_res.s16 = rc.out_ring + (size_t)res_slot * rc.out_slot_elems;
        if (tid == 0) (void)__hip_atomic_fetch_min(rc.t_first + res_slot, (unsigned long long)wall_clock64(), __ATOMIC_RELAXED, __HIP_MEMORY_SCOPE_AGENT);
    }
    const int sb = RES ? (int)(item % (unsigned)rc.n_wsb) : (int)blockIdx.x;
    const int seg_y = RES ? 0 : (int)blockIdx.y;
    const int col0 = PS ? 16 * seg_y : 0;
    if constexpr (RES) {
        in = rc.in_ring + (size_t)res_slot * rc.in_slot_bytes;
        pblock = rc.in_ring + (size_t)((res_slot + rc.n_slots - 1) % rc.n_slots) * rc.in_slot_bytes + (long long)sb * 16 * (long long)in_pitch;
    }
    const long long t0 = p.tile_first + (long long)seg_y * p.tiles_per_seg * (PS ? 16 : 1);
    long long t1 = t0 + p.tiles_per_seg; if (t1 > p.tile_first + p.n_tiles) t1 = p.tile_first + p.n_tiles;
    if (!RES && t0 >= t1) return;
    const int n_it = (int)(t1 - t0), n_grp = (n_it + TPG - 1) / TPG;
    const int n_lead = RES ? res_lead : ((PS && p.lead_n && seg_y == 0) ? p.lead_n[sb] : 0);
    const int n_warm = RES ? ((res_k > 0 && !res_retuned) ? 2 : 0) : ((PS || seg_y > 0) ? 2 : 0);
    const int last_stream = p.n_streams - 1;
    const int tstride = p.stride;
    const long long org = PS ? (long long)col0 * p.col_bytes : 0LL;
    long long wg = (t0 - (long long)n_warm * TPG) * tstride + p.win_off - p.B2 - org;
    const long long F0 = wg & ~1023LL;
    long long F_end = ((t1 - 1) * tstride + p.win_off - p.B2 - org + 64 * WFM_NK + 1023) & ~1023LL;
    { const long long row_end = ((p.two_T + 1023) & ~1023LL) - org; if (F_end > row_end) F_end = row_end; }
    long long F = F0;
    int fslot = (int)((F0 + 2 * SEQ_RB) % SEQ_RB), wslot = (int)((wg + 2 * SEQ_RB) % SEQ_RB);
    const uint32_t lds_in_addr = (uint32_t)(size_t)(__attribute__((address_space(3))) uint8_t *)lds_in;
    uint32_t voff[SPW], voff_h[SPW];
    long long row_lim[SPW];
#pragma unroll
    for (int r = 0; r < SPW; r++) {
        if constexpr (PS) {
            voff[r] = (uint32_t)((long long)(SPW * fw + r) * p.col_bytes) + 16u * lane;
            voff_h[r] = 16u * lane;
            row_lim[r] = p.two_T - (long long)(col0 + SPW * fw + r) * p.col_bytes;
        } else {
            const int srow = max(min(sb * 16 + SPW * fw + r, last_stream) - sb * 16, 0);
            voff[r] = (uint32_t)srow * (uint32_t)in_pitch + 16u * lane;
            voff_h[r] = (uint32_t)srow * (uint32_t)SEQ_HEAD + 16u * lane;
            row_lim[r] = 0;
        }
    }
    const uint8_t *sblock = PS ? in + (long long)sb * (long long)in_pitch + org : in + (long long)sb * 16 * (long long)in_pitch;
    const uint8_t *hblock = PS ? p.head_in + (size_t)sb * SEQ_HEAD : p.head_in + (size_t)sb * 16 * SEQ_HEAD;
    const bool ragged = (p.two_T & 1023) != 0;
    auto row_step = [&]() {
        if constexpr (PS) {
            const uint32_t ldst = lds_in_addr + (SPW * fw) * SEQ_RP + (uint32_t)fslot;
            const bool head = F < 0 && col0 == 0;
            if (!head && !ragged) {
                uint32_t vo[SPW];
#pragma unroll
                for (int r = 0; r < SPW; r++) vo[r] = F < row_lim[r] ? voff[r] : 16u * lane;
                dma_rows<SPW, SEQ_RP>(vo, sblock + F, __builtin_amdgcn_readfirstlane((int)ldst));
            } else
#pragma unroll
            for (int r = 0; r < SPW; r++) {
                const bool hrow = head && (SPW * fw + r == 0 || F + 1024 > row_lim[r]);
                const bool beyond = !hrow && F >= row_lim[r];
                const uint8_t *sbase = hrow ? hblock : sblock + F;
                const uint32_t vo = hrow ? voff_h[r] : (beyond ? 16u * lane : voff[r]);
                const bool live = hrow || F + 16 * lane < (beyond ? p.two_T - org : row_lim[r]);
                const uint32_t la = __builtin_amdgcn_readfirstlane((int)(ldst + r * SEQ_RP));
                uint32_t keep;
                if (live)
                    asm volatile("s_mov_b32 %0, m0\n\ts_mov_b32 m0, %3\n\ts_nop 0\n\tglobal_load_lds_dwordx4 %1, %2 nt\n\ts_mov_b32 m0, %0"
                                 : "=&s"(keep) : "v"(vo), "s"(sbase), "s"(la) : "memory");
            }
            F += 1024; fslot += 1024; if (fslot >= SEQ_RB) fslot -= SEQ_RB;
            return;
        }
        if constexpr (RES) {
            const uint8_t *sb_res = F < 0 ? pblock + (p.two_T + F) : sblock + F;
            dma_rows<SPW, SEQ_RP>(voff, sb_res, __builtin_amdgcn_readfirstlane((int)(lds_in_addr + (SPW * fw) * SEQ_RP + (uint32_t)fslot)));
            F += 1024; fslot += 1024; if (fslot >= SEQ_RB) fslot -= SEQ_RB;
            return;
        }
        const bool head = F < 0;
        const uint8_t *sbase = head ? hblock : sblock + F;
        const uint32_t ldst = lds_in_addr + (SPW * fw) * SEQ_RP + (uint32_t)fslot;
        const bool mask = ragged && !head;
        const bool live = !mask || F + 16 * lane < p.two_T;
        if (!head && !ragged) dma_rows<SPW, SEQ_RP>(voff, sbase, __builtin_amdgcn_readfirstlane((int)ldst));
        else
#pragma unroll
        for (int r = 0; r < SPW; r++) {
            const uint32_t la = __builtin_amdgcn_readfirstlane((int)(ldst + r * SEQ_RP));
            const uint32_t vo = head ? voff_h[r] : voff[r];
            uint32_t keep;
            if (!mask)
                asm volatile("s_mov_b32 %0, m0\n\ts_mov_b32 m0, %3\n\ts_nop 0\n\tglobal_load_lds_dwordx4 %1, %2 nt\n\ts_mov_b32 m0, %0"
                             : "=&s"(keep) : "v"(vo), "s"(sbase), "s"(la) : "memory");
            else if (live)
                asm volatile("s_mov_b32 %0, m0\n\ts_mov_b32 m0, %3\n\ts_nop 0\n\tglobal_load_lds_dwordx4 %1, %2 nt\n\ts_mov_b32 m0, %0"
                             : "=&s"(keep) : "v"(vo), "s"(sbase), "s"(la) : "memory");
        }
        F += 1024; fslot += 1024; if (fslot >= SEQ_RB) fslot -= SEQ_RB;
    };
    auto wait_newer = [&](long long newer) {
        switch ((int)newer) {
            case 0: wait_vmcnt<0>(); break;
            case 1: wait_vmcnt<SPW>(); break;
            case 2: wait_vmcnt<SPW * 2>(); break;
            case 3: wait_vmcnt<SPW * 3>(); break;
            case 4: wait_vmcnt<SPW * 4>(); break;
            case 5: wait_vmcnt<SPW * 5>(); break;
            case 6: wait_vmcnt<SPW * 6>(); break;
            default: wait_vmcnt<SPW * 7>(); break;
        }
    };
    auto wait_for = [&](long long last_window_start) {
        const long long need_end = (last_window_start + 64 * WFM_NK + 1023) & ~1023LL;
        long long newer = (F - need_end) >> 10;
        if (newer < 0) newer = 0;
        if (newer > 7) newer = 7;
        wait_newer(newer);
    };
    typedef float ps_v2f __attribute__((ext_vector_type(2)));
    ps_v2f psC = {1.f, 0.f};
    const bool ps_wave = PS && wv == 1, ps_lane = ps_wave && lane < 48;
    auto ps_base = [&](long long wgs) { return (int)((((wgs + p.B2) >> 1) >> 10) - (p.B2 >> 11)); };
    auto ps_load = [&](long long wgs) {
        if (ps_lane) {
            int ci = ps_base(wgs) + 1 + (lane >> 4) + (col0 + (lane & 15)) * p.col_chunks;
            ci = min(max(ci, 0), p.tab_len - 1);
            const float2 *pc = ctab + (size_t)ci * p.tab_pitch;
            asm volatile("global_load_dwordx2 %0, %1, off" : "+v"(psC) : "v"(pc) : "memory");
        }
    };
    auto ps_store = [&](int g) {
        asm volatile("s_waitcnt vmcnt(0)" : "+v"(psC) :: "memory");
        if (ps_lane) ctl[((g + 2) & 1) * 48 + lane] = make_float2(psC.x, psC.y);
    };
    if (ps_wave) {
        const long long step_b = (long long)TPG * tstride;
        ps_v2f c0 = {1.f, 0.f}, c1 = {1.f, 0.f};
        if (ps_lane) {
            auto entry = [&](long long wgs) {
                int ci = ps_base(wgs) + 1 + (lane >> 4) + (col0 + (lane & 15)) * p.col_chunks;
                ci = min(max(ci, 0), p.tab_len - 1);
                return ctab + (size_t)ci * p.tab_pitch;
            };
            const float2 *pa = entry(wg), *pb = entry(wg + step_b);
            asm volatile("global_load_dwordx2 %0, %2, off\n\tglobal_load_dwordx2 %1, %3, off" : "+v"(c0), "+v"(c1) : "v"(pa), "v"(pb) : "memory");
        }
        asm volatile("s_waitcnt vmcnt(0)" : "+v"(c0), "+v"(c1) :: "memory");
        if (ps_lane) {
            ctl[((-n_warm + 2) & 1) * 48 + lane] = make_float2(c0.x, c0.y);
            ctl[((-n_warm + 1 + 2) & 1) * 48 + lane] = make_float2(c1.x, c1.y);
        }
        ps_load(wg + 2 * step_b);
    }
    if (fetches) {
        while (F < F_end && F + 1024 <= wg + SEQ_RB) row_step();
        wait_for(wg + (long long)(TPG - 1) * tstride);
    }
    __syncthreads();
    const uint8_t *lrow = lds_in + col * SEQ_RP;
    const int s0 = sb * 16;
    float yst = 0.f;
    const float one_minus = 1 - p.alpha;
    const bool iir_wave = wv == 0, iir_lane = iir_wave && lane < 16;
    constexpr int QL = TPG, SPS = 4 * TPG;
    float bp[QL + 1];
    bp[0] = 1.f;
#pragma unroll
    for (int j = 1; j <= QL; j++) bp[j] = bp[j - 1] * one_minus;
    const float b2q = bp[QL] * bp[QL], b3q = b2q * bp[QL];
    float yst_first = 0.f;
    if (!RES && iir_wave && seg_y == 0) {
        yst = p.last_in[PS ? sb : min(s0 + col, last_stream)]; if (yst != yst) yst = 0.f;
        yst_first = yst;
    }
    if (RES && iir_wave && res_retuned) yst = rc.lead_state[min(s0 + col, last_stream)];
    const long long j_end = p.j_first + p.n_audio;
    const int seg_lo = (int)max(0LL, p.j_first - 4 * t0);
    const int seg_hi = (int)min(4LL * n_it, j_end - 4 * t0);
    const long long idx0 = 4 * t0 - p.j_first;
    auto col_lo = [&](int c) { return PS ? (col0 + c == 0 ? seg_lo : 0) : seg_lo; };
    auto col_hi = [&](int c) { return PS ? (int)max(0LL, min(4LL * n_it, j_end - 4 * (t0 + (long long)c * p.tiles_per_seg))) : seg_hi; };
    const bool emit_vec = ((((size_t)p.s16 | (size_t)p.af) & 15) == 0) && (p.out_pitch & 7) == 0;
    const int emit_a = (int)((SEQ_LINE - (idx0 & (SEQ_LINE - 1))) & (SEQ_LINE - 1));
    typedef unsigned wfm_st4 __attribute__((ext_vector_type(4)));
    auto put16 = [&](int16_t *dst, unsigned a, unsigned b, unsigned c, unsigned d) __attribute__((always_inline)) {
        if constexpr (RES) { const wfm_st4 v = {a, b, c, d}; asm volatile("global_store_dwordx4 %0, %1, off sc0 sc1" :: "v"(dst), "v"(v) : "memory"); }
        else *reinterpret_cast<uint4 *>(dst) = make_uint4(a, b, c, d);
    };
    auto put2 = [&](int16_t *dst, int v) __attribute__((always_inline)) {
        if constexpr (RES) asm volatile("global_store_short %0, %1, off sc0 sc1" :: "v"(dst), "v"(v) : "memory");
        else *dst = (int16_t)v;
    };
    auto s16_of = [](float e) { const float scaled = e * 32767.0f; return (scaled >= -2147483648.0f && scaled < 2147483648.0f) ? (int)scaled : (int)0x80000000; };
    constexpr int EMIT_T0 = 64, EMIT_N = 64 * (TPG - 1);
    auto emit_scalar = [&](int g) {
        if (g < 0 || g >= n_grp || tid < EMIT_T0) return;
#pragma unroll
        for (int e0 = 0; e0 < 16 * SPS; e0 += EMIT_N) {
            const int ei = e0 + tid - EMIT_T0;
            const int srow = ei / SPS, k = ei % SPS, kr = g * SPS + k;
            if (ei >= 16 * SPS) continue;
            if (PS ? (kr < col_lo(srow) || kr >= col_hi(srow)) : (kr < seg_lo || kr >= seg_hi || s0 + srow >= p.n_streams)) continue;
            const float e = lds_out[srow * SEQ_OUTP + (g % SEQ_OUTS) * SPS + k];
            const long long idx = idx0 + kr;
            const size_t at = PS ? (size_t)sb * p.out_pitch + (size_t)srow * p.col_audio + idx : (size_t)(s0 + srow) * p.out_pitch + idx;
            p.s16[at] = (int16_t)s16_of(e);
            if (p.af) p.af[at] = e;
        }
    };
#ifdef WFM_PROF
    long long prof[8] = {0, 0, 0, 0, 0, 0, 0, 0}, t_prev = __builtin_readcyclecounter();
#endif
    if (fetches) {
        typedef unsigned wfm_u4 __attribute__((ext_vector_type(4)));
        constexpr int NST = RES ? 8 : 44;
#define WFM_ST_ALL(X) X(0) X(1) X(2) X(3) X(4) X(5) X(6) X(7) X(8) X(9) X(10) X(11) X(12) X(13) X(14) X(15) X(16) X(17) X(18) X(19) X(20) X(21) X(22) X(23) \
                      X(24) X(25) X(26) X(27) X(28) X(29) X(30) X(31) X(32) X(33) X(34) X(35) X(36) X(37) X(38) X(39) X(40) X(41) X(42) X(43)
#define X(k) wfm_u4 st##k = {0u, 0u, 0u, 0u};
        WFM_ST_ALL(X)
#undef X
        int n_st = 0, st_n0 = 0;
        const int srow = 8 * fw + (lane >> 3), pc = lane & 7;
        const int lo_r = col_lo(srow), hi_r = col_hi(srow);
        const bool row_ok = PS ? hi_r > lo_r : s0 + srow < p.n_streams;
        const size_t row_at = PS ? (size_t)sb * p.out_pitch + (size_t)srow * p.col_audio : (size_t)(s0 + srow) * p.out_pitch;
        int16_t *const orow = p.s16 + row_at;
        auto flush = [&]() __attribute__((always_inline)) {
            if constexpr (PS) {
#define X(j) if (j < NST && j < n_st && row_ok) { const int a = st_n0 + SEQ_LINE * j + 8 * pc;                                                             \
                 if (a + 8 <= hi_r) *reinterpret_cast<uint4 *>(orow + (idx0 + a)) = make_uint4(st##j[0], st##j[1], st##j[2], st##j[3]);        \
                 else for (int i = 0; i < 8; i++) if (a + i < hi_r) orow[idx0 + a + i] = (int16_t)(st##j[i >> 1] >> (16 * (i & 1))); }
                WFM_ST_ALL(X)
#undef X
            } else {
#define X(j) if (j < NST && j < n_st && row_ok) put16(orow + (idx0 + st_n0 + SEQ_LINE * j + 8 * pc), st##j[0], st##j[1], st##j[2], st##j[3]);
                WFM_ST_ALL(X)
#undef X
            }
            n_st = 0;
        };
        auto take_line = [&](int g) __attribute__((always_inline)) {
            if (g < 0 || !emit_vec) return;
            const int k_before = (g * SPS - emit_a) >> 6, k_now = g < n_grp ? ((g + 1) * SPS - emit_a) >> 6 : k_before + 1;
            if (k_now <= k_before) return;
            static_assert(4 * SEQ_TPG < SEQ_LINE && SEQ_LINE == 64 && SEQ_NLD == 2, "one line per step at most; 8 streams x 8 pieces per loader");
            const int nl = emit_a + SEQ_LINE * (k_now - 1), n0 = nl + 8 * pc;
            if (nl + SEQ_LINE <= (PS ? 0 : seg_lo) || nl >= seg_hi) return;
            const float *src = lds_out + srow * SEQ_OUTP;
            float e[8];
#pragma unroll
            for (int i = 0; i < 8; i++) e[i] = src[(n0 + i + SEQ_OUTR) % SEQ_OUTR];
            int v[8];
#pragma unroll
            for (int i = 0; i < 8; i++) v[i] = s16_of(e[i]);
            const wfm_u4 w = {(unsigned)(v[0] & 0xffff) | ((unsigned)v[1] << 16), (unsigned)(v[2] & 0xffff) | ((unsigned)v[3] << 16),
                              (unsigned)(v[4] & 0xffff) | ((unsigned)v[5] << 16), (unsigned)(v[6] & 0xffff) | ((unsigned)v[7] << 16)};
            if (nl >= seg_lo && nl + SEQ_LINE <= seg_hi && !p.af) {
                if (n_st == 0) st_n0 = nl;
#define X(k) if (k < NST) st##k = n_st == k ? w : st##k;
                WFM_ST_ALL(X)
#undef X
                if (++n_st == NST) flush();
            } else if (row_ok) {
                const size_t o = (size_t)(idx0 + n0);
                float *const arow = p.af ? p.af + row_at : nullptr;
                if (n0 >= lo_r && n0 + 8 <= hi_r) {
                    put16(orow + o, w[0], w[1], w[2], w[3]);
                    if (arow) { *reinterpret_cast<float4 *>(arow + o) = make_float4(e[0], e[1], e[2], e[3]); *reinterpret_cast<float4 *>(arow + o + 4) = make_float4(e[4], e[5], e[6], e[7]); }
                } else {
#pragma unroll
                    for (int i = 0; i < 8; i++)
                        if (n0 + i >= lo_r && n0 + i < hi_r) { put2(orow + (o + i), v[i]); if (arow) arow[o + i] = e[i]; }
                }
            }
        };
        PROF_T(7)
#ifdef WFM_PROF
        t_first = __builtin_readcyclecounter();
#endif
        for (int gi = -n_warm; gi < n_grp; gi++) {
            PROF_T(0)
            const long long wg_n = wg + (long long)TPG * tstride;
            if (gi + 1 < n_grp) wait_for(wg_n + (long long)(TPG - 1) * tstride);
            PROF_T(1)
            __syncthreads();
            PROF_T(2)
            if (gi + 1 < n_grp) { while (F < F_end && F + 1024 <= wg_n + SEQ_RB) row_step(); }
            PROF_T(3)
            if (WFM_DIAG < 4) take_line(gi - 1);
            PROF_T(4)
#ifdef WFM_PROF
            prof[6] += 1;
#endif
            wg = wg_n;
        }
#ifdef WFM_PROF
        if (lane == 0) for (int k = 0; k < 8; k++) atomicAdd(&g_wfm_prof[wv][k], (unsigned long long)prof[k]);
        t_last = __builtin_readcyclecounter();
#endif
        __syncthreads();
        if (WFM_DIAG < 4) { take_line(n_grp - 1); take_line(n_grp); flush(); }
#undef WFM_ST_ALL
    } else {
    PROF_T(7)
#ifdef WFM_PROF
    t_first = __builtin_readcyclecounter();
#endif
    for (int gi = -n_warm; gi < n_grp; gi++) {
        const int it = gi * TPG + wv;
        float *lout = lds_out + ((gi + SEQ_OUTS) % SEQ_OUTS) * SPS;
        if (it < n_it && (WFM_DIAG < 3)) {
            const long long ws = wg + (long long)wv * tstride;
            const long long n0 = (ws + p.B2) >> 1;
            const int off = (int)(n0 & 1023);
            const bool two = off + 32 * WFM_NK > 1024;
            const int bo = 2 * (1024 - off);
            const int kb = __builtin_amdgcn_readfirstlane(two ? (bo >> 6) : WFM_NK), hq = __builtin_amdgcn_readfirstlane((bo >> 4) & 3);
            const long long chunk_rel = (n0 >> 10) - (p.B2 >> 11);
            unsigned a0 = (unsigned)(wslot + wv * tstride + 16 * q);
            a0 = min(a0, a0 - (unsigned)SEQ_RB);
            v4i Bf[WFM_NK];
#pragma unroll
            for (int ks = 0; ks < WFM_NK; ks++) {
                unsigned a = a0 + 64u * ks; a = min(a, a - (unsigned)SEQ_RB);
                if (WFM_DIAG == 1) Bf[ks] = v4i{(int)a, lane, ks, gi};
                else Bf[ks] = *reinterpret_cast<const v4i *>(lrow + a) ^ (int)0x80808080;
            }
            v4i acc[3] = {{0, 0, 0, 0}, {0, 0, 0, 0}, {0, 0, 0, 0}}, snap[3] = {{0, 0, 0, 0}, {0, 0, 0, 0}, {0, 0, 0, 0}};
            const bool lo_lane = q < hq;
            if (WFM_DIAG == 2) {
#pragma unroll
                for (int ks = 0; ks < WFM_NK; ks++) { acc[ks % 3] += Bf[ks]; snap[ks % 3] ^= Bf[ks]; }
            } else
            switch (kb) {
                case 0: wfm_chain<0>(A, Bf, lo_lane, acc, snap); break;
                case 1: wfm_chain<1>(A, Bf, lo_lane, acc, snap); break;
                case 2: wfm_chain<2>(A, Bf, lo_lane, acc, snap); break;
                case 3: wfm_chain<3>(A, Bf, lo_lane, acc, snap); break;
                case 4: wfm_chain<4>(A, Bf, lo_lane, acc, snap); break;
                case 5: wfm_chain<5>(A, Bf, lo_lane, acc, snap); break;
                case 6: wfm_chain<6>(A, Bf, lo_lane, acc, snap); break;
                case 7: wfm_chain<7>(A, Bf, lo_lane, acc, snap); break;
                default: wfm_chain<WFM_NK>(A, Bf, lo_lane, acc, snap); break;
            }
            const int kcls = PS ? (int)chunk_rel - ps_base(wg) : 0;
            const float2 *ct = ctl + ((gi + 2) & 1) * 48 + kcls * 16 + col;
            const float2 C0 = PS ? ct[0] : (RES ? lseed[chunk_rel + 4] : ctab[chunk_rel + 1]), D0 = dtab[off + 2048];
            const float2 P0 = make_float2(C0.x * D0.x - C0.y * D0.y, C0.x * D0.y + C0.y * D0.x);
            float2 P1 = make_float2(0.f, 0.f);
            float k0[4], k1[4];
            if (two) {
                const float2 C1 = PS ? ct[16] : (RES ? lseed[chunk_rel + 5] : ctab[chunk_rel + 2]), D1 = dtab[off - 1024 + 2048];
                P1 = make_float2(C1.x * D1.x - C1.y * D1.y, C1.x * D1.y + C1.y * D1.x);
                const float4 cb = *reinterpret_cast<const float4 *>(lcum + (bo >> 4) * 16 + 4 * q);
                k0[0] = cb.x - c_lo[0]; k0[1] = cb.y - c_lo[1]; k0[2] = cb.z - c_lo[2]; k0[3] = cb.w - c_lo[3];
                k1[0] = c_hi[0] - cb.x; k1[1] = c_hi[1] - cb.y; k1[2] = c_hi[2] - cb.z; k1[3] = c_hi[3] - cb.w;
            } else {
#pragma unroll
                for (int r = 0; r < 4; r++) { k0[r] = c_hi[r] - c_lo[r]; k1[r] = 0.f; }
            }
            float pI, pQ, cI, cQ;
            tile_rows(acc, snap, two, scale, k0, k1, P0, P1, pI, pQ, cI, cQ);
            const float dq = cQ - pQ, di = cI - pI;
            const float num = cI * dq - cQ * di, den = cI * cI + cQ * cQ;
            float rd = __builtin_amdgcn_rcpf(den);
            rd = fmaf(fmaf(-den, rd, 1.0f), rd, rd);
            float dval = (den != 0.f) ? (K * num) * rd : 0.f;
            if constexpr (PS) {
                const long long ja = 4 * (t0 + it) + q - p.j_first;
                if (n_lead > 0 && col0 + col == 0 && ja >= 0 && ja < n_lead) dval = p.lead_d[(size_t)sb * p.lead_stride + ja];
            }
            if constexpr (RES) {
                if (n_lead > 0) {
                    const long long ja = 4 * (t0 + it) + q - p.j_first;
                    if (ja >= 0 && ja < n_lead) dval = rc.lead_d[(size_t)min(sb * 16 + col, last_stream) * rc.lead_stride + ja];
                }
            }
            lout[col * SEQ_OUTP + 4 * wv + q] = dval;
        }
        PROF_T(0)
        const long long wg_n = wg + (long long)TPG * tstride;
        __syncthreads();
        PROF_T(2)
        if (!emit_vec) emit_scalar(gi - 1);
        if (ps_wave) { ps_store(gi + 2); ps_load(wg + 3LL * TPG * tstride); }
        PROF_T(4)
        if (iir_wave && WFM_DIAG < 5) {
            if (PS && gi == 0 && col0 + col == 0) yst = yst_first;
            const int lo = (gi == 0 && !(RES && n_warm)) ? col_lo(col) : 0;
            const int hi = gi < 0 ? SPS : max(0, min(SPS, col_hi(col) - gi * SPS));
            if (PS ? __all(lo == 0 && (hi & 3) == 0) : (lo == 0 && (hi & 3) == 0)) {
                float *row = lout + col * SEQ_OUTP + QL * q;
                const int nv = hi;
                float x[QL], z[QL], y[QL];
#pragma unroll
                for (int j = 0; j < QL; j += 2) {
                    const float2 v = *reinterpret_cast<const float2 *>(row + j);
                    const bool ok = QL * q + j < nv;
                    x[j] = ok ? v.x : 0.f; x[j + 1] = ok ? v.y : 0.f;
                }
                z[0] = p.alpha * x[0];
#pragma unroll
                for (int j = 1; j < QL; j++) z[j] = p.alpha * x[j] + one_minus * z[j - 1];
                const float ze_0 = __shfl(z[QL - 1], col, 64), ze_1 = __shfl(z[QL - 1], col + 16, 64), ze_2 = __shfl(z[QL - 1], col + 32, 64);
                float S = yst;
                if (q == 1) S = bp[QL] * yst + ze_0;
                else if (q == 2) S = b2q * yst + (bp[QL] * ze_0 + ze_1);
                else if (q == 3) S = b3q * yst + (b2q * ze_0 + (bp[QL] * ze_1 + ze_2));
#pragma unroll
                for (int j = 0; j < QL; j++) y[j] = z[j] + bp[j + 1] * S;
#pragma unroll
                for (int j = 0; j < QL; j += 2) *reinterpret_cast<float2 *>(row + j) = make_float2(y[j], y[j + 1]);
                if (nv > 0) {
                    const int lq = (nv - 1) / QL, lj = (nv - 1) % QL;
                    float ylast = y[QL - 1];
#pragma unroll
                    for (int j = 1; j < QL - 1; j += 2) if (lj == j) ylast = y[j];
                    yst = __shfl(ylast, col + 16 * lq, 64);
                }
            } else {
                float yv = yst;
                if (lane < 16) {
                    float *row = lout + col * SEQ_OUTP;
                    for (int i = lo; i < hi; i++) { yv = p.alpha * row[i] + one_minus * yv; row[i] = yv; }
                }
                yst = __shfl(yv, col, 64);
            }
        }
        PROF_T(5)
#ifdef WFM_PROF
        prof[6] += 1;
#endif
        wg = wg_n; wslot += TPG * tstride; if (wslot >= SEQ_RB) wslot -= SEQ_RB;
    }
#ifdef WFM_PROF
    if (lane == 0) for (int k = 0; k < 8; k++) atomicAdd(&g_wfm_prof[wv][k], (unsigned long long)prof[k]);
    t_last = __builtin_readcyclecounter();
#endif
    __syncthreads();
    if (!emit_vec) emit_scalar(n_grp - 1);
    }
    if (PS && seg_y + 1 == (int)gridDim.y) {
        if (iir_lane && col0 + lane == p.n_cols - 1) p.last_out[sb] = yst;
        if (tid < 32 && p.two_T >= 512 && (p.two_T & 15) == 0) {
            const uint4 v = *reinterpret_cast<const uint4 *>(in + (size_t)sb * in_pitch + (p.two_T - 512) + 16 * tid);
            *reinterpret_cast<uint4 *>(p.head_out + (size_t)sb * SEQ_HEAD + 512 + 16 * tid) = v;
        }
    } else
    if (!PS && !RES && seg_y + 1 == (int)gridDim.y) {
        if (iir_lane && s0 + lane < p.n_streams) p.last_out[s0 + lane] = yst;
        if (tid < 16 * 32 && p.two_T >= 512 && (p.two_T & 15) == 0 && s0 + tid / 32 < p.n_streams) {
            const int srow = tid / 32, piece = tid % 32;
            const uint4 v = *reinterpret_cast<const uint4 *>(sblock + (size_t)srow * in_pitch + (p.two_T - 512) + 16 * piece);
            *reinterpret_cast<uint4 *>(p.head_out + (size_t)(s0 + srow) * SEQ_HEAD + 512 + 16 * piece) = v;
        }
    }
#ifdef WFM_PROF
    if (lane == 0) {
        asm volatile("s_waitcnt vmcnt(0)" ::: "memory");
        const long long t_exit = __builtin_readcyclecounter();
        atomicAdd(&g_wfm_life[wv][0], (unsigned long long)(t_first - t_entry)); atomicAdd(&g_wfm_life[wv][1], (unsigned long long)(t_last - t_first));
        atomicAdd(&g_wfm_life[wv][2], (unsigned long long)(t_exit - t_last)); atomicAdd(&g_wfm_life[wv][3], 1ULL);
    }
#endif
    if constexpr (!RES) break;
    else {
        if (tid == 0) { const long long t = wall_clock64(); st_body += t - st_t; st_t = t; }
        if (wv == 0) {
            const unsigned long long nx = item + gridDim.x;
            const long long nk = (long long)(nx / (unsigned)rc.n_wsb);
            const uint32_t *dsc = rc.desc + (size_t)(nk % rc.n_slots) * rc.desc_lines * 16;
            const int nd = rc.desc_lines * 16;
#pragma unroll
            for (int j = 0; j < 4; j++) { const int d = lane + 64 * j; pre_v[j] = d < nd ? sys_load(dsc + d) : 0u; }
            pre_valid = true;
        }
        if (rc.fence_mode == 2) __threadfence_system();
        if (wv != 0 || !emit_vec) asm volatile("s_waitcnt vmcnt(0)" ::: "memory");
        __syncthreads();
        if (tid == 0) {
            if (rc.fence_mode == 3) __threadfence_system();
            pend_c = __hip_atomic_fetch_add(rc.cnt + res_slot, 1u, __ATOMIC_RELAXED, __HIP_MEMORY_SCOPE_AGENT);
            pend = true; pend_slot = res_slot; pend_n = p.n_audio; pend_k = res_k;
        }
        item += gridDim.x;
        if (tid == 0) { const long long t = wall_clock64(); st_done += t - st_t; st_t = t; st_items++; }
    }
    }
}

__global__ __launch_bounds__(256) void k_wfm_roll_head(const uint8_t *__restrict__ in, size_t in_pitch, long long two_T, const uint8_t *__restrict__ head_in, uint8_t *__restrict__ head_out)
{
    const int s = blockIdx.x, t = threadIdx.x;
    for (int k = 2 * t; k < 2 * t + 2; k++) {
        const long long pos = two_T - 512 + k;
        head_out[(size_t)s * SEQ_HEAD + 512 + k] = pos >= 0 ? in[(size_t)s * in_pitch + pos] : head_in[(size_t)s * SEQ_HEAD + 512 + (pos + 512)];
    }
}

struct LeadParams { int D, L, F; long long B, j_first, c_first; int n_lead, ja0, lead_stride; float *warm; size_t tab_pitch, dtab_stride, ct_stride, head_pitch, head_off; };
__global__ __launch_bounds__(128) void k_wfm_lead(const uint8_t *__restrict__ in, size_t in_pitch, const uint8_t *__restrict__ head, const float *__restrict__ taps,
                                                 const float2 *__restrict__ ctab, const float2 *__restrict__ dtab, const float2 *__restrict__ dtab_old,
                                                 const int *__restrict__ list, float *__restrict__ lead_d, LeadParams p)
{
    __shared__ float2 yv[2];
    const int s = list[blockIdx.y], ja = (int)blockIdx.x + p.ja0, which = threadIdx.x >> 6, lane = threadIdx.x & 63;
    const long long j = p.j_first + ja, k = (long long)p.F * j + 9 + which;
    const uint8_t *row = in + (size_t)s * in_pitch, *hrow = head + (size_t)s * p.head_pitch + p.head_off;
    const float2 *ct = ctab + (size_t)s * p.ct_stride, *dn = dtab + (size_t)s * p.dtab_stride, *dold = dtab_old + (size_t)s * p.dtab_stride;
    float ai = 0.f, aq = 0.f;
    for (int t = lane; t < p.L; t += 64) {
        const long long n = (long long)p.D * k + t, rel = n - p.B;
        uint32_t vi, vq;
        if (rel < 0) { vi = hrow[2 * (rel + 256)]; vq = hrow[2 * (rel + 256) + 1]; } else { vi = row[2 * rel]; vq = row[2 * rel + 1]; }
        const float2 C = ct[(size_t)((n >> 10) - p.c_first) * p.tab_pitch], Dv = (rel < 0 ? dold : dn)[(int)(n & 1023) + 2048];
        const float2 R = make_float2(C.x * Dv.x - C.y * Dv.y, C.x * Dv.y + C.y * Dv.x);
        const float xi = fmaf((float)vi, 0x1.010102p-7f, -1.0f), xq = fmaf((float)vq, 0x1.010102p-7f, -1.0f);
        const float h = taps[t];
        ai = fmaf(h, xi * R.x - xq * R.y, ai); aq = fmaf(h, xq * R.x + xi * R.y, aq);
    }
#pragma unroll
    for (int o = 32; o >= 1; o >>= 1) { ai += __shfl_xor(ai, o, 64); aq += __shfl_xor(aq, o, 64); }
    if (lane == 0) yv[which] = make_float2(ai, aq);
    __syncthreads();
    if (threadIdx.x == 0) {
        const float K = 0.340447550238101026565118445432744920253753662109375f;
        const float pI = yv[0].x, pQ = yv[0].y, cI = yv[1].x, cQ = yv[1].y;
        const float dq = cQ - pQ, di = cI - pI, num = cI * dq - cQ * di, den = cI * cI + cQ * cQ;
        float rd = __builtin_amdgcn_rcpf(den); rd = fmaf(fmaf(-den, rd, 1.0f), rd, rd);
        const float dv = (den != 0.f) ? (K * num) * rd : 0.f;
        if (ja >= 0) lead_d[(size_t)s * p.lead_stride + ja] = dv; else p.warm[(size_t)s * RES_WARM + (ja + RES_WARM)] = dv;
    }
}

__global__ __launch_bounds__(64) void k_wfm_lead_state(const float *__restrict__ warm, float *__restrict__ state, int n_streams, float alpha)
{
    const int s = blockIdx.x * 64 + threadIdx.x;
    if (s >= n_streams) return;
    float y = 0.f;
    for (int i = 0; i < RES_WARM; i++) y = alpha * warm[(size_t)s * RES_WARM + i] + (1 - alpha) * y;
    state[s] = y;
}

}

namespace csdr_amd {

size_t wfm_mfma_head_bytes(int n_streams) { return (size_t)((n_streams + 15) / 16 * 16) * SEQ_HEAD; }

int wfm_mfma_lead(hipStream_t st, const uint8_t *in, size_t in_pitch, const uint8_t *head, const float *d_taps, const float2 *ctab, size_t tab_pitch, const float2 *d_dtab,
                  const float2 *d_dtab_old, const int *d_list, int n_list, float *d_lead_d, int lead_stride, int D, int L, int F, long long B, long long j_first, int n_lead)
{
    if (n_list <= 0 || n_lead <= 0) return 0;
    LeadParams lp; lp.D = D; lp.L = L; lp.F = F; lp.B = B; lp.j_first = j_first; lp.n_lead = n_lead; lp.tab_pitch = tab_pitch; lp.dtab_stride = 3072;
    lp.ct_stride = 1; lp.head_pitch = SEQ_HEAD; lp.head_off = 512; lp.c_first = (B >> 10) - 1; lp.ja0 = 0; lp.warm = nullptr; lp.lead_stride = lead_stride;
    hipLaunchKernelGGL(k_wfm_lead, dim3(n_lead, n_list), dim3(128), 0, st, in, in_pitch, head, d_taps, ctab, d_dtab, d_dtab_old, d_list, d_lead_d, lp);
    CSDR_LAUNCH_CHECK();
    return 0;
}

int wfm_mfma_lead_shared(hipStream_t st, const uint8_t *in, size_t in_pitch, const uint8_t *prev, size_t two_T, const float *d_taps, const float2 *ctab, const float2 *d_dtab,
                         const float2 *d_dtab_old, const int *d_list, int n_list, float *d_lead_d, int lead_stride, float *d_warm, float *d_state, float alpha,
                         int D, int L, int F, long long B, long long j_first, int n_lead)
{
    if (n_list <= 0) return 0;
    if (j_first < RES_WARM) return fail_msg(-3, "wfm ring: a retune needs %d audio samples in front of the block", RES_WARM);
    LeadParams lp; lp.D = D; lp.L = L; lp.F = F; lp.B = B; lp.j_first = j_first; lp.n_lead = n_lead; lp.tab_pitch = 1; lp.dtab_stride = 0;
    lp.ct_stride = 0; lp.head_pitch = in_pitch; lp.head_off = two_T - 512; lp.c_first = (B >> 10) - 4; lp.ja0 = -RES_WARM; lp.warm = d_warm; lp.lead_stride = lead_stride;
    hipLaunchKernelGGL(k_wfm_lead, dim3(n_lead + RES_WARM, n_list), dim3(128), 0, st, in, in_pitch, prev, d_taps, ctab, d_dtab, d_dtab_old, d_list, d_lead_d, lp);
    CSDR_LAUNCH_CHECK();
    hipLaunchKernelGGL(k_wfm_lead_state, dim3((n_list + 63) / 64), dim3(64), 0, st, d_warm, d_state, n_list, alpha);
    CSDR_LAUNCH_CHECK();
    return 0;
}

int wfm_mfma_launch(hipStream_t st, hipEvent_t ev_begin, hipEvent_t ev_end, const uint8_t *in, size_t in_pitch, const WfmMfmaDevice &dev, const float2 *ctab,
                    int n_streams, int T, long long B, long long j_first, int n_audio, const WfmBackArgs &back, const WfmPerStream *ps)
{
    if (in_pitch * 16 + 4096 >= ((size_t)1 << 32)) return fail_msg(-3, "wfm: in_pitch %zu too large for the matrix-core front end (32-bit row offsets)", in_pitch);
    if (n_audio <= 0) {
        hipLaunchKernelGGL(k_wfm_roll_head, dim3(n_streams), dim3(256), 0, st, in, in_pitch, 2LL * T, back.head_in, back.head_out);
        CSDR_LAUNCH_CHECK();
        return 0;
    }
    SeqParams sp;
    memset((void *)&sp, 0, sizeof sp);
    ResCtl no_res; memset((void *)&no_res, 0, sizeof no_res);
    sp.n_streams = n_streams; sp.B2 = 2 * B; sp.two_T = 2LL * T;
    sp.tile_first = j_first / 4; sp.n_tiles = (int)((j_first + n_audio - 1) / 4 - sp.tile_first + 1);
    sp.stride = dev.tile_stride_bytes; sp.win_off = dev.win_off_bytes; sp.scale = dev.seq_scale;
    const int n_cu = current_device_cu_count();
    const int n_wsb = (n_streams + 15) / 16;
    int n_seg = (n_cu + n_wsb - 1) / n_wsb; if (n_seg < 1) n_seg = 1;
    if (n_seg > sp.n_tiles / 24) n_seg = sp.n_tiles / 24;
    if (n_seg < 1) n_seg = 1;
    sp.tiles_per_seg = ((sp.n_tiles + n_seg - 1) / n_seg + SEQ_TPG - 1) / SEQ_TPG * SEQ_TPG;
    n_seg = (sp.n_tiles + sp.tiles_per_seg - 1) / sp.tiles_per_seg;
    sp.alpha = back.alpha; sp.last_in = back.last_in; sp.last_out = back.last_out; sp.s16 = back.s16; sp.af = back.af; sp.out_pitch = back.out_pitch;
    sp.j_first = j_first; sp.n_audio = n_audio; sp.head_in = back.head_in; sp.head_out = back.head_out;
    if (ps) {
        const long long ts = sp.stride / 2;
        long long per = ts; { long long a = per, b = 1024; while (b) { const long long t = a % b; a = b; b = t; } per = per / a * 1024; }
        int tpp = (int)(per / ts);
        while ((4 * tpp) % SEQ_LINE) tpp *= 2;
        const int n_per = (sp.n_tiles + tpp - 1) / tpp;
        int n_ss = (4 * n_cu + n_streams - 1) / n_streams; if (n_ss < 1) n_ss = 1;
        int np = (n_per + 16 * n_ss - 1) / (16 * n_ss); if (np < 1) np = 1;
        sp.tiles_per_seg = np * tpp;
        sp.n_cols = (sp.n_tiles + sp.tiles_per_seg - 1) / sp.tiles_per_seg;
        n_seg = (sp.n_cols + 15) / 16;
        sp.col_bytes = (long long)sp.tiles_per_seg * sp.stride; sp.col_chunks = (int)(sp.col_bytes / 2048); sp.col_audio = 4 * sp.tiles_per_seg;
        sp.frag_stride = (size_t)WFM_NK * 3 * 64; sp.tab_pitch = ps->tab_pitch; sp.tab_len = ps->tab_len; sp.scales = ps->d_scales;
        sp.lead_d = ps->d_lead_d; sp.lead_n = ps->d_lead_n; sp.lead_stride = ps->lead_stride;
        if (sp.col_bytes * 16 + 4096 >= (1LL << 32)) return fail_msg(-3, "wfm: block too large for the per-stream kernel's 32-bit row offsets");
        const size_t ldsp = (size_t)16 * SEQ_RP + 16 * SEQ_OUTP * sizeof(float) + (SEQ_NGR + 1) * 16 * sizeof(float) + 2 * 48 * sizeof(float2);
        { const int arc = lds_attr_once((const void *)k_wfm_mfma_seq<true>, ldsp); if (arc) return arc; }
        if (ev_begin && ev_end)
            hipExtLaunchKernelGGL(k_wfm_mfma_seq<true>, dim3(n_streams, n_seg), dim3(64 * SEQ_NW), ldsp, st, ev_begin, ev_end, 0, in, in_pitch, (const v4i *)dev.d_seq_frags, dev.d_seq_cum, dev.d_dtab, ctab, sp, no_res);
        else
            hipLaunchKernelGGL(k_wfm_mfma_seq<true>, dim3(n_streams, n_seg), dim3(64 * SEQ_NW), ldsp, st, in, in_pitch, (const v4i *)dev.d_seq_frags, dev.d_seq_cum, dev.d_dtab, ctab, sp, no_res);
        CSDR_LAUNCH_CHECK();
        if (T < 256 || (T & 7)) {
            hipLaunchKernelGGL(k_wfm_roll_head, dim3(n_streams), dim3(256), 0, st, in, in_pitch, 2LL * T, back.head_in, back.head_out);
            CSDR_LAUNCH_CHECK();
        }
        return 0;
    }
    const size_t lds = (size_t)16 * SEQ_RP + 16 * SEQ_OUTP * sizeof(float) + (SEQ_NGR + 1) * 16 * sizeof(float);
    { const int arc = lds_attr_once((const void *)k_wfm_mfma_seq<false>, lds); if (arc) return arc; }
    if (ev_begin && ev_end)
        hipExtLaunchKernelGGL(k_wfm_mfma_seq<false>, dim3(n_wsb, n_seg), dim3(64 * SEQ_NW), lds, st, ev_begin, ev_end, 0, in, in_pitch, (const v4i *)dev.d_seq_frags, dev.d_seq_cum, dev.d_dtab, ctab, sp, no_res);
    else
        hipLaunchKernelGGL(k_wfm_mfma_seq<false>, dim3(n_wsb, n_seg), dim3(64 * SEQ_NW), lds, st, in, in_pitch, (const v4i *)dev.d_seq_frags, dev.d_seq_cum, dev.d_dtab, ctab, sp, no_res);
    CSDR_LAUNCH_CHECK();
    if (T < 256 || (T & 7)) {
        hipLaunchKernelGGL(k_wfm_roll_head, dim3(n_streams), dim3(256), 0, st, in, in_pitch, 2LL * T, back.head_in, back.head_out);
        CSDR_LAUNCH_CHECK();
    }
    return 0;
}

int wfm_mfma_launch_resident(hipStream_t st, hipEvent_t ev_end, const WfmMfmaDevice &dev, int n_streams, size_t in_pitch, float alpha, size_t out_pitch, const WfmResident &rv, int grid)
{
    if (in_pitch * 16 + 4096 >= ((size_t)1 << 32)) return fail_msg(-3, "wfm ring: in_pitch %zu too large (32-bit row offsets)", in_pitch);
    SeqParams sp; memset((void *)&sp, 0, sizeof sp);
    sp.n_streams = n_streams; sp.two_T = 2LL * rv.T; sp.stride = dev.tile_stride_bytes; sp.win_off = dev.win_off_bytes; sp.scale = dev.seq_scale;
    sp.alpha = alpha; sp.out_pitch = out_pitch;
    ResCtl rc; memset((void *)&rc, 0, sizeof rc);
    rc.desc = rv.desc; rc.ctrl = rv.ctrl; rc.done = rv.done; rc.cnt = rv.cnt; rc.t_first = rv.t_first; rc.next_item = rv.next_item; rc.exiting = rv.exiting;
    rc.in_ring = rv.in_ring; rc.out_ring = rv.out_ring; rc.in_slot_bytes = rv.in_slot_bytes; rc.out_slot_elems = rv.out_slot_elems;
    rc.n_slots = rv.n_slots; rc.desc_lines = rv.desc_lines; rc.n_wsb = (n_streams + 15) / 16; rc.T = rv.T; rc.D = rv.D; rc.L = rv.L; rc.F = rv.F;
    rc.idle_ticks = rv.idle_ticks; rc.life_ticks = rv.life_ticks; rc.lead_d = rv.lead_d; rc.lead_stride = rv.lead_stride; rc.lead_state = rv.lead_state; rc.stats = rv.stats; rc.fence_mode = rv.fence_mode;
    if (rv.desc_lines < 1 || rv.desc_lines > 16) return fail_msg(-3, "wfm ring: %d descriptor lines", rv.desc_lines);
    const size_t lds = (size_t)16 * SEQ_RP + 16 * SEQ_OUTP * sizeof(float) + (SEQ_NGR + 1) * 16 * sizeof(float) + 8 + (size_t)rv.desc_lines * 14 * sizeof(float);
    { const int arc = lds_attr_once((const void *)k_wfm_mfma_seq<false, true>, lds); if (arc) return arc; }
    hipLaunchKernelGGL((k_wfm_mfma_seq<false, true>), dim3(grid), dim3(64 * SEQ_NW), lds, st, (const uint8_t *)nullptr, in_pitch, (const v4i *)dev.d_seq_frags, dev.d_seq_cum, dev.d_dtab,
                       (const float2 *)nullptr, sp, rc);
    CSDR_LAUNCH_CHECK();
    if (ev_end) CSDR_HIP(hipEventRecord(ev_end, st));
    return 0;
}
int wfm_resident_max_grid() { return current_device_cu_count(); }

}

#ifdef WFM_PROF
extern "C" int csdr_amd_debug_wfm_prof(unsigned long long *out, int reset)
{
    if (hipMemcpyFromSymbol(out, HIP_SYMBOL(g_wfm_prof), sizeof(unsigned long long) * SEQ_NW * 8) != hipSuccess) return -1;
    if (reset) { static unsigned long long z[SEQ_NW * 8]; if (hipMemcpyToSymbol(HIP_SYMBOL(g_wfm_prof), z, sizeof(z)) != hipSuccess) return -1; }
    return 0;
}
extern "C" int csdr_amd_debug_wfm_life(unsigned long long *out, int reset)
{
    if (hipMemcpyFromSymbol(out, HIP_SYMBOL(g_wfm_life), sizeof(unsigned long long) * SEQ_NW * 4) != hipSuccess) return -1;
    if (reset) { static unsigned long long z[SEQ_NW * 4]; if (hipMemcpyToSymbol(HIP_SYMBOL(g_wfm_life), z, sizeof(z)) != hipSuccess) return -1; }
    return 0;
}
#endif

extern "C" int csdr_amd_debug_wfm_seq_tile(int D, int L, int F, float shift_rate, const float *taps, long long n0, const uint8_t *window,
                                           const float *ctab2, float *out16)
{
    if (!wfm_mfma_supported(D, L, F) || (n0 & 7)) return -1;
    static WfmMfmaTable t; static int cD = 0, cL = 0, cF = 0; static float crate = 0; static std::vector<float> ctaps;
    if (cD != D || cL != L || cF != F || crate != shift_rate || ctaps != std::vector<float>(taps, taps + L)) {
        wfm_mfma_build_table(D, L, F, shift_rate, taps, t); cD = D; cL = L; cF = F; crate = shift_rate; ctaps.assign(taps, taps + L);
    }
    const int off = (int)(n0 & 1023);
    const bool two = off + 32 * WFM_NK > 1024;
    const int bo = 2 * (1024 - off), kb = two ? (bo >> 6) : WFM_NK, hq = (bo >> 4) & 3, gb = bo >> 4;
    const float2 D0 = t.dtab[off + 2048], C0 = make_float2(ctab2[0], ctab2[1]);
    const float2 P0 = make_float2(C0.x * D0.x - C0.y * D0.y, C0.x * D0.y + C0.y * D0.x);
    float2 P1 = make_float2(0.f, 0.f);
    if (two) { const float2 D1 = t.dtab[off - 1024 + 2048], C1 = make_float2(ctab2[2], ctab2[3]); P1 = make_float2(C1.x * D1.x - C1.y * D1.y, C1.x * D1.y + C1.y * D1.x); }
    const int ngr = 4 * WFM_NK;
    float u[16], v[16];
    for (int r = 0; r < 16; r++) {
        long acc[3] = {0, 0, 0}, snap[3] = {0, 0, 0};
        auto step = [&](int ks, int kg_lo, int kg_hi) {
            for (int kg = kg_lo; kg < kg_hi; kg++) for (int b = 0; b < 16; b++) {
                const int x = (int)(int8_t)(window[64 * ks + 16 * kg + b] ^ 0x80);
                for (int l = 0; l < 3; l++) acc[l] += (long)t.seq_frags[((size_t)(ks * 3 + l) * 64 + (16 * kg + r)) * 16 + b] * x;
            }
        };
        for (int ks = 0; ks < WFM_NK; ks++) {
            if (ks == kb) { step(ks, 0, hq); for (int l = 0; l < 3; l++) snap[l] = acc[l]; step(ks, hq, 4); }
            else step(ks, 0, 4);
        }
        const float clo = t.seq_cum[r], chi = t.seq_cum[(size_t)ngr * 16 + r];
        if (two) {
            const float cb = t.seq_cum[(size_t)gb * 16 + r];
            u[r] = fmaf(fmaf((float)snap[0], 65536.0f, fmaf((float)snap[1], 256.0f, (float)snap[2])), t.seq_scale, cb - clo);
            v[r] = fmaf(fmaf((float)(acc[0] - snap[0]), 65536.0f, fmaf((float)(acc[1] - snap[1]), 256.0f, (float)(acc[2] - snap[2]))), t.seq_scale, chi - cb);
        } else {
            u[r] = fmaf(fmaf((float)acc[0], 65536.0f, fmaf((float)acc[1], 256.0f, (float)acc[2])), t.seq_scale, chi - clo);
            v[r] = 0.f;
        }
    }
    for (int k = 0; k < 8; k++) {
        out16[2 * k] = P0.x * u[2 * k] - P0.y * u[2 * k + 1] + (P1.x * v[2 * k] - P1.y * v[2 * k + 1]);
        out16[2 * k + 1] = P0.x * u[2 * k + 1] + P0.y * u[2 * k] + (P1.x * v[2 * k + 1] + P1.y * v[2 * k]);
    }
    return 0;
}
```

### csdr_amd/csrc/wfm_mfma.hpp

```cpp
#pragma once
#include "common.hpp"
#include <vector>

namespace csdr_amd {

constexpr int WFM_HIST = 256;
constexpr int WFM_NK = 8;

struct WfmMfmaTable {
    int D, L, F, tile_stride_bytes, win_off_bytes;
    std::vector<int8_t> seq_frags;
    std::vector<float> seq_cum;
    std::vector<float2> dtab;
    float seq_scale;
};

struct WfmMfmaDevice {
    int tile_stride_bytes, win_off_bytes;
    void *d_seq_frags; float *d_seq_cum; float2 *d_dtab; float seq_scale;
};

struct WfmBackArgs {
    float alpha; const float *last_in; float *last_out; int16_t *s16; float *af; size_t out_pitch; const uint8_t *head_in; uint8_t *head_out;
};

struct WfmPerStream { size_t tab_pitch; int tab_len; const float *d_scales; const float *d_lead_d; const int *d_lead_n; int lead_stride; };
inline int wfm_lead_max(int D, int L, int F) { return (D + L - 1) / (D * F) + 2; }

struct WfmResident {
    const uint32_t *desc, *ctrl; uint32_t *done;
    unsigned *cnt; unsigned long long *t_first, *next_item; unsigned *exiting;
    const uint8_t *in_ring; int16_t *out_ring; size_t in_slot_bytes, out_slot_elems;
    int n_slots, desc_lines, T, D, L, F;
    long long idle_ticks, life_ticks;
    const float *lead_d, *lead_state; int lead_stride;
    unsigned long long *stats; int fence_mode;
};
constexpr int WFM_RES_WARM = 48;
int wfm_mfma_launch_resident(hipStream_t st, hipEvent_t ev_end, const WfmMfmaDevice &dev, int n_streams, size_t in_pitch, float alpha, size_t out_pitch, const WfmResident &rv, int grid);
int wfm_resident_max_grid();
int wfm_mfma_lead_shared(hipStream_t st, const uint8_t *in, size_t in_pitch, const uint8_t *prev, size_t two_T, const float *d_taps, const float2 *ctab, const float2 *d_dtab,
                         const float2 *d_dtab_old, const int *d_list, int n_list, float *d_lead_d, int lead_stride, float *d_warm, float *d_state, float alpha,
                         int D, int L, int F, long long B, long long j_first, int n_lead);

bool wfm_mfma_supported(int D, int L, int F);
void wfm_mfma_build_table(int D, int L, int F, float shift_rate, const float *taps, WfmMfmaTable &t);
size_t wfm_mfma_head_bytes(int n_streams);
int wfm_mfma_launch(hipStream_t st, hipEvent_t ev_begin, hipEvent_t ev_end, const uint8_t *in, size_t in_pitch, const WfmMfmaDevice &dev, const float2 *ctab,
                    int n_streams, int T, long long B, long long j_first, int n_audio, const WfmBackArgs &back, const WfmPerStream *ps = nullptr);
int wfm_mfma_lead(hipStream_t st, const uint8_t *in, size_t in_pitch, const uint8_t *head, const float *d_taps, const float2 *ctab, size_t tab_pitch, const float2 *d_dtab,
                  const float2 *d_dtab_old, const int *d_list, int n_list, float *d_lead_d, int lead_stride, int D, int L, int F, long long B, long long j_first, int n_lead);

}
```

### include/csdr_amd.h

```cpp
#ifndef CSDR_AMD_H
#define CSDR_AMD_H
#include <stddef.h>
#include <stdint.h>

#ifdef __cplusplus
extern "C" {
#endif

typedef struct csdr_complexf_s { float i, q; } csdr_complexf;

typedef enum { CSDR_WINDOW_BOXCAR = 0, CSDR_WINDOW_BLACKMAN = 1, CSDR_WINDOW_HAMMING = 2 } csdr_window_t;

typedef struct csdr_amd_ctx csdr_amd_ctx;

csdr_amd_ctx *csdr_amd_ctx_create(int device, void *hip_stream);
void          csdr_amd_ctx_destroy(csdr_amd_ctx *ctx);
int           csdr_amd_ctx_sync(csdr_amd_ctx *ctx);
void         *csdr_amd_ctx_stream(csdr_amd_ctx *ctx);
const char   *csdr_amd_last_error(void);
int           csdr_amd_device_count(void);
const char   *csdr_amd_device_arch(csdr_amd_ctx *ctx);

void *csdr_amd_malloc(csdr_amd_ctx *ctx, size_t bytes);
void  csdr_amd_free(csdr_amd_ctx *ctx, void *dptr);
// ... 76 lines not shown
int  csdr_amd_resampler_process(csdr_amd_resampler *r, const float *in, long long n_in, size_t in_pitch, float *out, size_t out_pitch, long long *n_out);
long long csdr_amd_resampler_max_out(const csdr_amd_resampler *r, long long n_in);
int  csdr_amd_resampler_reset(csdr_amd_resampler *r);
int  csdr_amd_resampler_set_cli_bufsize(csdr_amd_resampler *r, int the_bufsize);
int  csdr_amd_resampler_force_generic(csdr_amd_resampler *r, int on);
int  csdr_amd_resampler_set_last_taps_delay(csdr_amd_resampler *r, int last_taps_delay);
int  csdr_amd_resampler_window(int interpolation, int decimation, int taps_length, int input_size, int last_taps_delay, int *state);
const char *csdr_amd_resampler_kernel_name(const csdr_amd_resampler *r);
void csdr_amd_resampler_destroy(csdr_amd_resampler *r);
typedef struct csdr_amd_interp csdr_amd_interp;
csdr_amd_interp *csdr_amd_interp_create(csdr_amd_ctx *ctx, int interpolation, const float *host_taps, int taps_length, int n_streams);
int  csdr_amd_interp_process(csdr_amd_interp *p, const csdr_complexf *in, long long n_in, size_t in_pitch, csdr_complexf *out, size_t out_pitch, long long *n_out);
long long csdr_amd_interp_max_out(const csdr_amd_interp *p, long long n_in);
int  csdr_amd_interp_reset(csdr_amd_interp *p);
int  csdr_amd_interp_set_cli_bufsize(csdr_amd_interp *p, int the_bufsize);
int  csdr_amd_interp_force_generic(csdr_amd_interp *p, int on);
const char *csdr_amd_interp_kernel_name(const csdr_amd_interp *p);
void csdr_amd_interp_destroy(csdr_amd_interp *p);
void csdr_amd_rational_resampler_get_lowpass_f(float *output, int output_size, int interpolation, int decimation, int window);
int  csdr_amd_debug_resampler_schedule(int interpolation, int decimation, int taps_length, int last_taps_delay, int n, int *out);

enum { CSDR_AMD_PSK31_AGC = 0, CSDR_AMD_PSK31_TIMING = 1, CSDR_AMD_PSK31_DBPSK = 2, CSDR_AMD_PSK31_VARICODE = 3 };
typedef struct csdr_amd_psk31_params {
    float rate, reference, max_gain;
    int algorithm, decimation;
    float loop_gain, max_error;
    int use_q;
} csdr_amd_psk31_params;
typedef struct csdr_amd_psk31_chan {
    float gain;
    int tail_len, correction_offset;
    unsigned base;
    float last_i, last_q;
    unsigned long long varicode_shr;
} csdr_amd_psk31_chan;
typedef struct csdr_amd_psk31 csdr_amd_psk31;
csdr_amd_psk31 *csdr_amd_psk31_create(csdr_amd_ctx *ctx, const csdr_amd_psk31_params *params, int n_channels, int first_stage, int last_stage);
int  csdr_amd_psk31_process(csdr_amd_psk31 *p, const void *in, long long n_in, size_t in_pitch, void *out, size_t out_pitch, int *counts, float *err, unsigned *idx);
long long csdr_amd_psk31_max_out(const csdr_amd_psk31 *p, long long n_in);
int  csdr_amd_psk31_reset(csdr_amd_psk31 *p);
int  csdr_amd_psk31_reset_channel(csdr_amd_psk31 *p, int channel);
int  csdr_amd_psk31_get_channel(csdr_amd_psk31 *p, int channel, csdr_amd_psk31_chan *state);
int  csdr_amd_psk31_set_channel(csdr_amd_psk31 *p, int channel, const csdr_amd_psk31_chan *state);
int  csdr_amd_psk31_set_lanes(csdr_amd_psk31 *p, int lanes);
int  csdr_amd_psk31_force_generic(csdr_amd_psk31 *p, int on);
int  csdr_amd_psk31_lanes(const csdr_amd_psk31 *p);
const char *csdr_amd_psk31_kernel_name(const csdr_amd_psk31 *p);
void csdr_amd_psk31_destroy(csdr_amd_psk31 *p);
int  csdr_amd_simple_agc_cc(csdr_amd_ctx *ctx, const csdr_complexf *in, csdr_complexf *out, int n_streams, long long n, size_t in_pitch, size_t out_pitch,
                            float rate, float reference, float max_gain, float *gain_io);
char csdr_amd_psk31_varicode_decoder_push(unsigned long long *status_shr, unsigned char symbol);
void csdr_amd_psk31_varicode_table(int *out);
long long csdr_amd_debug_psk31_walk(const csdr_amd_psk31_params *params, int first_stage, int last_stage, const void *in, long long n, const long long *cuts,
                                    int n_cuts, void *out, float *err, unsigned *idx, csdr_amd_psk31_chan *state_io);

enum { CSDR_AMD_RTTY_BFSK = 0, CSDR_AMD_RTTY_SERIAL = 1, CSDR_AMD_RTTY_BAUDOT = 2 };
typedef struct csdr_amd_rtty_params {
    float spacing;
    int filter_length;
    int window;
    float samples_per_bits;
    int databits;
    float stopbits;
    float bit_sampling_width_ratio;
    int cli_bufsize;
} csdr_amd_rtty_params;
typedef struct csdr_amd_rtty csdr_amd_rtty;
csdr_amd_rtty *csdr_amd_rtty_create(csdr_amd_ctx *ctx, const csdr_amd_rtty_params *params, int n_channels, int first_stage, int last_stage);
int  csdr_amd_rtty_process(csdr_amd_rtty *r, const void *in, long long n_in, size_t in_pitch, void *out, size_t out_pitch, int *counts);
long long csdr_amd_rtty_max_out(const csdr_amd_rtty *r, long long n_in);
int  csdr_amd_rtty_reset(csdr_amd_rtty *r);
int  csdr_amd_rtty_reset_channel(csdr_amd_rtty *r, int channel);
int  csdr_amd_rtty_force_generic(csdr_amd_rtty *r, int on);
const char *csdr_amd_rtty_kernel_name(const csdr_amd_rtty *r);
void csdr_amd_rtty_destroy(csdr_amd_rtty *r);
int  csdr_amd_bfsk_demod_cf(csdr_amd_ctx *ctx, const csdr_complexf *in, float *out, int n_streams, long long n, size_t in_pitch, size_t out_pitch,
                            const csdr_complexf *mark_filter, const csdr_complexf *space_filter, int taps_length, int force_generic);
const char *csdr_amd_bfsk_last_kernel(void);
int  csdr_amd_binary_slicer_f_u8(csdr_amd_ctx *ctx, const float *in, uint8_t *out, int n_streams, long long n, size_t in_pitch, size_t out_pitch);
typedef struct csdr_amd_rtty_push_state { int fig_mode, character_received, shr, bit_cntr, state; } csdr_amd_rtty_push_state;
int  csdr_amd_rtty_line_decoder_u8_u8(csdr_amd_ctx *ctx, const uint8_t *in, uint8_t *out, int n_streams, long long n, size_t in_pitch, size_t out_pitch,
                                      csdr_amd_rtty_push_state *state, int *counts);
int  csdr_amd_serial_line_decoder_f_u8(csdr_amd_ctx *ctx, const float *in, void *out, int n_streams, int n, size_t in_pitch, size_t out_pitch,
                                       float samples_per_bits, int databits, float stopbits, float bit_sampling_width_ratio, int *counts, int *used);
char csdr_amd_rtty_baudot_decoder_lookup(unsigned char *fig_mode, unsigned char c);
char csdr_amd_rtty_baudot_decoder_push(csdr_amd_rtty_push_state *s, unsigned char symbol);
void csdr_amd_firdes_add_peak_c(csdr_complexf *output, int length, float rate, int window, int add, int normalize);
void csdr_amd_firdes_peak_c(csdr_complexf *taps, int length, float rate, int window);
long long csdr_amd_debug_rtty_walk(const csdr_amd_rtty_params *params, int first_stage, int last_stage, const void *in, long long n, const long long *cuts,
                                   int n_cuts, void *out);

typedef struct csdr_amd_squelch csdr_amd_squelch;
csdr_amd_squelch *csdr_amd_squelch_create(csdr_amd_ctx *ctx, int n_channels, int block_size, int use_every_nth, const float *levels, long long max_samples_per_call);
int  csdr_amd_squelch_process(csdr_amd_squelch *s, const csdr_complexf *in, long long n_in, size_t in_pitch, csdr_complexf *out, size_t out_pitch, float *power,
                              size_t power_pitch, uint8_t *open_flags, int *n_blocks_out);
int  csdr_amd_squelch_set_level(csdr_amd_squelch *s, int channel, float level);
float csdr_amd_squelch_get_level(const csdr_amd_squelch *s, int channel);
long long csdr_amd_squelch_block_index(const csdr_amd_squelch *s, int channel);
int  csdr_amd_squelch_max_blocks(const csdr_amd_squelch *s);
int  csdr_amd_squelch_reset(csdr_amd_squelch *s);
int  csdr_amd_squelch_reset_channel(csdr_amd_squelch *s, int channel);
int  csdr_amd_squelch_force_generic(csdr_amd_squelch *s, int on);
const char *csdr_amd_squelch_kernel_name(const csdr_amd_squelch *s);
void csdr_amd_squelch_destroy(csdr_amd_squelch *s);
int  csdr_amd_get_power_c(csdr_amd_ctx *ctx, const csdr_complexf *in, int n_streams, int n_blocks, int block_size, int decimation, size_t in_pitch, float *power_out);
int  csdr_amd_get_power_f(csdr_amd_ctx *ctx, const float *in, int n_streams, int n_blocks, int block_size, int decimation, size_t in_pitch, float *power_out);
int  csdr_amd_squelch_report_due(int report_every_nth, long long block_index);
int  csdr_amd_squelch_gate_open(float power, float level);
float csdr_amd_debug_squelch_power(const float *in, int block_size, int decimation, int is_complex);

enum { CSDR_AMD_CARRIER_COSTAS = 0, CSDR_AMD_CARRIER_COSTAS_DD = 1, CSDR_AMD_CARRIER_PLL_P = 2, CSDR_AMD_CARRIER_PLL_PI = 3 };
typedef struct csdr_amd_carrier_params { int mode; float alpha, beta, dphase_max; int dphase_max_reset_to_zero; } csdr_amd_carrier_params;
typedef struct csdr_amd_carrier_chan { float phase, dphase, freq; } csdr_amd_carrier_chan;
typedef struct csdr_amd_carrier csdr_amd_carrier;
int  csdr_amd_costas_params(float bandwidth, float damping, int decision_directed, csdr_amd_carrier_params *p);
int  csdr_amd_pll_params_p(float alpha, csdr_amd_carrier_params *p);
int  csdr_amd_pll_params_pi(float bandwidth, float ko, float kd, float damping, csdr_amd_carrier_params *p);
csdr_amd_carrier *csdr_amd_carrier_create(csdr_amd_ctx *ctx, const csdr_amd_carrier_params *params, int n_channels);
int  csdr_amd_carrier_process(csdr_amd_carrier *p, const csdr_complexf *in, long long n, size_t in_pitch, csdr_complexf *out, float *error, float *dphase,
                              csdr_complexf *nco, size_t out_pitch);
int  csdr_amd_carrier_reset(csdr_amd_carrier *p);
int  csdr_amd_carrier_reset_channel(csdr_amd_carrier *p, int channel);
int  csdr_amd_carrier_get_channel(csdr_amd_carrier *p, int channel, csdr_amd_carrier_chan *out);
int  csdr_amd_carrier_set_channel(csdr_amd_carrier *p, int channel, const csdr_amd_carrier_chan *state);
int  csdr_amd_carrier_set_lanes(csdr_amd_carrier *p, int lanes);
int  csdr_amd_carrier_lanes(const csdr_amd_carrier *p);
int  csdr_amd_carrier_force_generic(csdr_amd_carrier *p, int on);
const char *csdr_amd_carrier_kernel_name(const csdr_amd_carrier *p);
void csdr_amd_carrier_destroy(csdr_amd_carrier *p);
long long csdr_amd_debug_carrier_walk(const csdr_amd_carrier_params *params, const csdr_complexf *in, long long n, const long long *cuts, int n_cuts,
                                      csdr_complexf *out, float *error, float *dphase, csdr_complexf *nco, csdr_amd_carrier_chan *state_io);

int csdr_amd_fmmod_fc(csdr_amd_ctx *ctx, const float *in, csdr_complexf *out, int n_streams, size_t n, size_t in_pitch, size_t out_pitch, float *phase_io);
int csdr_amd_dsb_fc(csdr_amd_ctx *ctx, const float *in, csdr_complexf *out, size_t n, float q_value);
int csdr_amd_add_dcoffset_cc(csdr_amd_ctx *ctx, const csdr_complexf *in, csdr_complexf *out, size_t n);
int csdr_amd_fixed_amplitude_cc(csdr_amd_ctx *ctx, const csdr_complexf *in, csdr_complexf *out, size_t n, float new_amplitude);
int csdr_amd_convert_f_samplerf(csdr_amd_ctx *ctx, const float *in, void *out, size_t n, unsigned wait_for_this_sample);
long long csdr_amd_debug_fmmod_walk(const float *in, long long n, const long long *cuts, int n_cuts, float *phases, csdr_complexf *out, float *state_io);

enum { CSDR_TX_FM = 0, CSDR_TX_AM = 1, CSDR_TX_DSB = 2 };
enum { CSDR_TX_OUT_CF32 = 0, CSDR_TX_OUT_U8 = 1 };
typedef struct csdr_amd_txbank csdr_amd_txbank;
csdr_amd_txbank *csdr_amd_txbank_create(csdr_amd_ctx *ctx, int n_streams, int mode, float gain, float q_value, int interpolation, const float *host_taps,
                                        int taps_length, const float *shift_rates, int out_format, size_t max_in_samples);
int  csdr_amd_txbank_process(csdr_amd_txbank *p, const int16_t *in_s16, size_t in_pitch, long long n_in, void *out, size_t out_pitch, long long *n_out);
int  csdr_amd_txbank_set_rate(csdr_amd_txbank *p, int stream, float rate);
float csdr_amd_txbank_get_rate(const csdr_amd_txbank *p, int stream);
int  csdr_amd_txbank_reset(csdr_amd_txbank *p);
long long csdr_amd_txbank_max_out(const csdr_amd_txbank *p, long long n_in);
int  csdr_amd_txbank_force_generic(csdr_amd_txbank *p, int on);
const char *csdr_amd_txbank_kernel_name(const csdr_amd_txbank *p);
void csdr_amd_txbank_destroy(csdr_amd_txbank *p);

int csdr_amd_amdemod_cf(csdr_amd_ctx *ctx, const csdr_complexf *in, float *out, size_t n);
int csdr_amd_amdemod_estimator_cf(csdr_amd_ctx *ctx, const csdr_complexf *in, float *out, size_t n, float alpha, float beta);
int csdr_amd_realpart_cf(csdr_amd_ctx *ctx, const csdr_complexf *in, float *out, size_t n);
int csdr_amd_logpower_cf(csdr_amd_ctx *ctx, const csdr_complexf *in, float *out, size_t n, float add_db);
int csdr_amd_fmdemod_atan_cf(csdr_amd_ctx *ctx, const csdr_complexf *in, float *out, int n_streams, size_t n,
                             size_t in_pitch, size_t out_pitch, float *last_phase_io);
int csdr_amd_dcblock_ff(csdr_amd_ctx *ctx, const float *in, float *out, int n_streams, size_t n, size_t in_pitch, size_t out_pitch,
                        float a, float *state_io);
int csdr_amd_fastdcblock_ff(csdr_amd_ctx *ctx, const float *in, float *out, int n_streams, int n_blocks, int block,
                            size_t in_pitch, size_t out_pitch, float *last_dc_io);
int csdr_amd_agc_ff(csdr_amd_ctx *ctx, const float *in, float *out, int n_streams, size_t n, int block, size_t in_pitch, size_t out_pitch,
                    float reference, float attack_rate, float decay_rate, float max_gain, short hang_time, short attack_wait_time,
                    float gain_filter_alpha, float *last_gain_io);
void csdr_amd_precalculate_window(float *host_windowt, int size, int window);
typedef struct csdr_amd_fftcc csdr_amd_fftcc;
csdr_amd_fftcc *csdr_amd_fftcc_create(csdr_amd_ctx *ctx, int fft_size, int every_n_samples, int window, int max_frames);
void csdr_amd_fftcc_destroy(csdr_amd_fftcc *f);
int  csdr_amd_fftcc_process(csdr_amd_fftcc *f, const csdr_complexf *in, size_t n_in, csdr_complexf *out, size_t *consumed);

typedef struct csdr_amd_waterfall csdr_amd_waterfall;
enum { CSDR_AMD_WF_IN_CF32 = 0, CSDR_AMD_WF_IN_U8 = 1 };
enum { CSDR_AMD_WF_OUT_DB = 0, CSDR_AMD_WF_OUT_ADPCM = 1 };
csdr_amd_waterfall *csdr_amd_waterfall_create(csdr_amd_ctx *ctx, int fft_size, int every_n_samples, int window, int avgnumber,
                                              float add_db, int in_format, int out_format, int n_streams, size_t max_samples_per_call);
int  csdr_amd_waterfall_process(csdr_amd_waterfall *w, const void *in, size_t n_in, size_t in_pitch, void *out, size_t out_pitch, int *rows_out);
int  csdr_amd_waterfall_reset(csdr_amd_waterfall *w);
const char *csdr_amd_waterfall_kernel_name(const csdr_amd_waterfall *w);
int  csdr_amd_waterfall_force_generic(csdr_amd_waterfall *w, int on);
void csdr_amd_waterfall_destroy(csdr_amd_waterfall *w);
int  csdr_amd_logaveragepower_cf(csdr_amd_ctx *ctx, const csdr_complexf *in, float *out, int n_rows, int fft_size, int avgnumber, float add_db);
int  csdr_amd_fft_exchange_sides_ff(csdr_amd_ctx *ctx, const float *in, float *out, int n_rows, int fft_size);
int  csdr_amd_accumulate_power_cf(csdr_amd_ctx *ctx, const csdr_complexf *in, float *acc_io, size_t n);
int  csdr_amd_log_ff(csdr_amd_ctx *ctx, const float *in, float *out, size_t n, float add_db);

int csdr_amd_encode_ima_adpcm_i16_u8(csdr_amd_ctx *ctx, const int16_t *in, uint8_t *out, int n_streams, size_t n,
                                     size_t in_pitch, size_t out_pitch, int *state_io);
int csdr_amd_decode_ima_adpcm_u8_i16(csdr_amd_ctx *ctx, const uint8_t *in, int16_t *out, int n_streams, size_t n,
                                     size_t in_pitch, size_t out_pitch, int *state_io);
int csdr_amd_compress_fft_adpcm_f_u8(csdr_amd_ctx *ctx, const float *in, uint8_t *out, int n_blocks, int fft_size);

typedef struct csdr_amd_fftfilt csdr_amd_fftfilt;
csdr_amd_fftfilt *csdr_amd_fftfilt_create(csdr_amd_ctx *ctx, int fft_size, const csdr_complexf *host_taps,
                                          int taps_length, int n_streams, int max_blocks);
void csdr_amd_fftfilt_destroy(csdr_amd_fftfilt *f);
int  csdr_amd_fftfilt_set_taps(csdr_amd_fftfilt *f, const csdr_complexf *host_taps, int taps_length);
int  csdr_amd_fftfilt_input_size(const csdr_amd_fftfilt *f);
const char *csdr_amd_fftfilt_kernel_name(const csdr_amd_fftfilt *f);
int  csdr_amd_fftfilt_window(const csdr_amd_fftfilt *f);
int  csdr_amd_fftfilt_reset(csdr_amd_fftfilt *f);
int  csdr_amd_fftfilt_process(csdr_amd_fftfilt *f, const csdr_complexf *in, csdr_complexf *out,
                              int n_blocks, size_t in_pitch, size_t out_pitch);

int csdr_amd_fft_c2c(csdr_amd_ctx *ctx, const csdr_complexf *in, csdr_complexf *out, int n, int forward);
int csdr_amd_bin_product(csdr_amd_ctx *ctx, const csdr_complexf *a, const csdr_complexf *b, csdr_complexf *out, size_t n);
int csdr_amd_scale_add(csdr_amd_ctx *ctx, csdr_complexf *io, size_t n, float scale, const csdr_complexf *add, size_t n_add);

typedef struct csdr_fastddc_s {
    int pre_decimation, post_decimation, taps_length, taps_min_length, overlap_length,
        fft_size, fft_inv_size, input_size, post_input_size;
    float pre_shift; int startbin, v, offsetbin; float post_shift; int output_scrape, scrap;
    struct { float sindelta, cosdelta, rate; } dsadata;
} csdr_fastddc_t;
int csdr_amd_fastddc_init(csdr_fastddc_t *ddc, float transition_bw, int decimation, float shift_rate);

typedef struct csdr_amd_fastddc_fwd csdr_amd_fastddc_fwd;
csdr_amd_fastddc_fwd *csdr_amd_fastddc_fwd_create(csdr_amd_ctx *ctx, const csdr_fastddc_t *ddc, int max_blocks);
void csdr_amd_fastddc_fwd_destroy(csdr_amd_fastddc_fwd *f);
int  csdr_amd_fastddc_fwd_process(csdr_amd_fastddc_fwd *f, const csdr_complexf *in, csdr_complexf *spectra, int n_blocks);

typedef struct csdr_amd_fastddc_inv csdr_amd_fastddc_inv;
csdr_amd_fastddc_inv *csdr_amd_fastddc_inv_create(csdr_amd_ctx *ctx, float transition_bw, int decimation,
                                                  const float *host_shift_rates, int n_channels, int window,
                                                  int max_blocks);
void csdr_amd_fastddc_inv_destroy(csdr_amd_fastddc_inv *f);
int  csdr_amd_fastddc_inv_set_rate(csdr_amd_fastddc_inv *f, int channel, float shift_rate);
int  csdr_amd_fastddc_inv_geometry(const csdr_amd_fastddc_inv *f, int channel, csdr_fastddc_t *ddc);
int  csdr_amd_fastddc_inv_max_output(const csdr_amd_fastddc_inv *f, int n_blocks);
int  csdr_amd_fastddc_inv_process(csdr_amd_fastddc_inv *f, const csdr_complexf *spectra, int n_blocks,
                                  csdr_complexf *out, size_t out_pitch, int *out_counts);
const char *csdr_amd_fastddc_inv_kernel_name(const csdr_amd_fastddc_inv *f);
int  csdr_amd_fastddc_inv_set_profiling(csdr_amd_fastddc_inv *f, int on);
int  csdr_amd_fastddc_inv_kernel_time(csdr_amd_fastddc_inv *f, double *total_ms, long *launches);
int  csdr_amd_fastddc_inv_stage_time(csdr_amd_fastddc_inv *f, int stage, double *total_ms, long *launches);
typedef struct csdr_amd_fastddc_bank csdr_amd_fastddc_bank;
csdr_amd_fastddc_bank *csdr_amd_fastddc_bank_create(csdr_amd_ctx *ctx, float transition_bw, int decimation, const float *host_shift_rates, int n_channels,
                                                    int window, int max_blocks);
void csdr_amd_fastddc_bank_destroy(csdr_amd_fastddc_bank *b);
int  csdr_amd_fastddc_bank_set_rate(csdr_amd_fastddc_bank *b, int channel, float shift_rate);
int  csdr_amd_fastddc_bank_input_size(const csdr_amd_fastddc_bank *b);
int  csdr_amd_fastddc_bank_max_output(const csdr_amd_fastddc_bank *b, int n_blocks);
int  csdr_amd_fastddc_bank_process(csdr_amd_fastddc_bank *b, const csdr_complexf *in, int n_blocks, csdr_complexf *out, size_t out_pitch, int *out_counts);
int  csdr_amd_fastddc_bank_submit(csdr_amd_fastddc_bank *b, const csdr_complexf *in, int n_blocks);
int  csdr_amd_fastddc_bank_collect(csdr_amd_fastddc_bank *b, csdr_complexf *out, size_t out_pitch, int *out_counts);

typedef struct csdr_amd_comm csdr_amd_comm;
int  csdr_amd_comm_unique_id(char id128[128]);
csdr_amd_comm *csdr_amd_comm_create(csdr_amd_ctx *ctx, const char id128[128], int rank, int world);
void csdr_amd_comm_destroy(csdr_amd_comm *c);
int  csdr_amd_comm_rank(const csdr_amd_comm *c);
int  csdr_amd_comm_world(const csdr_amd_comm *c);
int  csdr_amd_comm_broadcast(csdr_amd_comm *c, void *dev_buf, size_t bytes, int root);
csdr_amd_comm *csdr_amd_comm_dup(csdr_amd_comm *c);
int  csdr_amd_comm_selftest(csdr_amd_comm *c, size_t n_floats, char *report, size_t report_cap);
typedef struct csdr_amd_loopback csdr_amd_loopback;
csdr_amd_loopback *csdr_amd_loopback_create(int world);
void csdr_amd_loopback_destroy(csdr_amd_loopback *g);
void csdr_amd_loopback_abort(csdr_amd_loopback *g);
csdr_amd_comm *csdr_amd_comm_create_loopback(csdr_amd_ctx *ctx, csdr_amd_loopback *g, int rank);
csdr_amd_comm *csdr_amd_comm_create_null(csdr_amd_ctx *ctx, int rank, int world);
csdr_amd_comm *csdr_amd_comm_create_ipc(csdr_amd_ctx *ctx, const char *path_prefix, int rank, int world);
int csdr_amd_debug_comm_exchange(csdr_amd_comm *c, const float *send_buf, float *recv_buf, size_t n, int peer, int n_sends);
enum { CSDR_AMD_SHARD_CHANNELS = 0, CSDR_AMD_SHARD_BLOCKS = 1 };
csdr_amd_fastddc_bank *csdr_amd_fastddc_bank_create_sharded(csdr_amd_ctx *ctx, float transition_bw, int decimation, const float *host_shift_rates_all, int n_channels_total,
                                                            int window, int max_blocks, csdr_amd_comm *comm);
csdr_amd_fastddc_bank *csdr_amd_fastddc_bank_create_sharded_by(csdr_amd_ctx *ctx, float transition_bw, int decimation, const float *host_shift_rates_all, int n_channels_total,
                                                               int window, int max_blocks, csdr_amd_comm *comm, int shard_mode);
int  csdr_amd_fastddc_bank_channel_slice(const csdr_amd_fastddc_bank *b, int *first, int *count);
int  csdr_amd_fastddc_bank_shard_mode(const csdr_amd_fastddc_bank *b);
int  csdr_amd_fastddc_bank_default_shard_mode(int world);
int  csdr_amd_fastddc_bank_local_blocks(const csdr_amd_fastddc_bank *b, int n_blocks, int *first, int *count);
int  csdr_amd_fastddc_bank_overlap(const csdr_amd_fastddc_bank *b);
int  csdr_amd_fastddc_bank_submit_local(csdr_amd_fastddc_bank *b, const csdr_complexf *in_run, int n_blocks);
int  csdr_amd_fastddc_bank_process_s16(csdr_amd_fastddc_bank *b, const int16_t *in_iq, int n_blocks, csdr_complexf *out, size_t out_pitch, int *out_counts);
int  csdr_amd_fastddc_bank_process_u8(csdr_amd_fastddc_bank *b, const uint8_t *in_iq, int n_blocks, csdr_complexf *out, size_t out_pitch, int *out_counts);
int  csdr_amd_fastddc_bank_submit_s16(csdr_amd_fastddc_bank *b, const int16_t *in_iq, int n_blocks);
int  csdr_amd_fastddc_bank_submit_u8(csdr_amd_fastddc_bank *b, const uint8_t *in_iq, int n_blocks);
int  csdr_amd_fastddc_bank_submit_local_s16(csdr_amd_fastddc_bank *b, const int16_t *in_run_iq, int n_blocks);
int  csdr_amd_fastddc_bank_submit_local_u8(csdr_amd_fastddc_bank *b, const uint8_t *in_run_iq, int n_blocks);
int  csdr_amd_fastddc_bank_finish(csdr_amd_fastddc_bank *b, int *out_counts);
int  csdr_amd_fastddc_bank_set_rate_global(csdr_amd_fastddc_bank *b, int channel, float shift_rate);
csdr_amd_fastddc_inv *csdr_amd_fastddc_bank_inverse(csdr_amd_fastddc_bank *b);

int  csdr_amd_fastddc_inv_block(csdr_amd_ctx *ctx, const csdr_complexf *d_spectrum, const csdr_complexf *d_taps_fft,
                                const csdr_fastddc_t *ddc, void *status_io, csdr_complexf *d_inv_in, csdr_complexf *d_td,
                                csdr_complexf *d_out);

typedef struct csdr_amd_wfm csdr_amd_wfm;
csdr_amd_wfm *csdr_amd_wfm_create(csdr_amd_ctx *ctx, int n_streams, float shift_rate, int decimation,
                                  const float *host_taps, int taps_length, int frac_rate,
                                  float tau, int audio_rate, size_t max_block_samples);
csdr_amd_wfm *csdr_amd_wfm_create_rates(csdr_amd_ctx *ctx, int n_streams, const float *shift_rates, int decimation,
                                        const float *host_taps, int taps_length, int frac_rate,
                                        float tau, int audio_rate, size_t max_block_samples);
int   csdr_amd_wfm_set_rate(csdr_amd_wfm *w, int stream, float shift_rate);
float csdr_amd_wfm_get_rate(const csdr_amd_wfm *w, int stream);
void csdr_amd_wfm_destroy(csdr_amd_wfm *w);
int  csdr_amd_wfm_reset(csdr_amd_wfm *w);
long csdr_amd_wfm_process(csdr_amd_wfm *w, const uint8_t *in, size_t in_pitch, size_t block_samples,
                          int16_t *audio_s16, float *audio_f, size_t out_pitch);
const char *csdr_amd_wfm_kernel_name(const csdr_amd_wfm *w);
int csdr_amd_wfm_fallback(const csdr_amd_wfm *w);
int csdr_amd_wfm_set_profiling(csdr_amd_wfm *w, int on);
int csdr_amd_wfm_kernel_time(csdr_amd_wfm *w, double *total_ms, long *launches);

typedef struct csdr_amd_wfm_ring csdr_amd_wfm_ring;
csdr_amd_wfm_ring *csdr_amd_wfm_ring_create(csdr_amd_ctx *ctx, int n_streams, float shift_rate, int decimation, const float *host_taps, int taps_length, int frac_rate,
                                            float tau, int audio_rate, size_t block_samples, int n_slots);
void csdr_amd_wfm_ring_destroy(csdr_amd_wfm_ring *r);
int  csdr_amd_wfm_ring_reset(csdr_amd_wfm_ring *r);
int  csdr_amd_wfm_ring_acquire(csdr_amd_wfm_ring *r, long long seq, double timeout_s);
uint8_t *csdr_amd_wfm_ring_input(csdr_amd_wfm_ring *r, long long seq, size_t *pitch_bytes);
long long csdr_amd_wfm_ring_submit(csdr_amd_wfm_ring *r);
long csdr_amd_wfm_ring_wait(csdr_amd_wfm_ring *r, long long seq, double timeout_s);
const int16_t *csdr_amd_wfm_ring_output(csdr_amd_wfm_ring *r, long long seq, size_t *pitch_samples);
int  csdr_amd_wfm_ring_set_rate(csdr_amd_wfm_ring *r, float shift_rate);
float csdr_amd_wfm_ring_get_rate(const csdr_amd_wfm_ring *r);
int  csdr_amd_wfm_ring_set_timeouts(csdr_amd_wfm_ring *r, double idle_us, double life_ms);
int  csdr_amd_wfm_ring_resident(csdr_amd_wfm_ring *r);
int  csdr_amd_wfm_ring_stop(csdr_amd_wfm_ring *r);
int  csdr_amd_wfm_ring_slots(const csdr_amd_wfm_ring *r);
int  csdr_amd_wfm_ring_grid(const csdr_amd_wfm_ring *r);
long csdr_amd_wfm_ring_launches(const csdr_amd_wfm_ring *r);
long long csdr_amd_wfm_ring_submitted(const csdr_amd_wfm_ring *r);
int  csdr_amd_wfm_ring_stats(csdr_amd_wfm_ring *r, double out[4]);
int  csdr_amd_wfm_ring_replay(csdr_amd_wfm_ring *r, long n_blocks, double *t_first_us, double *t_done_us);
int  csdr_amd_wfm_ring_block_times(csdr_amd_wfm_ring *r, long long seq, double *t_first_us, double *t_done_us);

typedef struct csdr_amd_ddc csdr_amd_ddc;
csdr_amd_ddc *csdr_amd_ddc_create(csdr_amd_ctx *ctx, int n_streams, float shift_rate, int decimation,
                                  const float *host_taps, int taps_length, size_t max_block_samples);
csdr_amd_ddc *csdr_amd_ddc_create_rates(csdr_amd_ctx *ctx, int n_streams, const float *shift_rates, int decimation,
                                        const float *host_taps, int taps_length, size_t max_block_samples);
int   csdr_amd_ddc_set_rate(csdr_amd_ddc *d, int stream, float shift_rate);
float csdr_amd_ddc_get_rate(const csdr_amd_ddc *d, int stream);
int   csdr_amd_ddc_fallback(const csdr_amd_ddc *d);
void csdr_amd_ddc_destroy(csdr_amd_ddc *d);
int  csdr_amd_ddc_reset(csdr_amd_ddc *d);
long csdr_amd_ddc_process(csdr_amd_ddc *d, const uint8_t *in, size_t in_pitch, size_t block_samples,
                          csdr_complexf *out, size_t out_pitch);
const char *csdr_amd_ddc_kernel_name(const csdr_amd_ddc *d);
int csdr_amd_ddc_set_profiling(csdr_amd_ddc *d, int on);
int csdr_amd_ddc_kernel_time(csdr_amd_ddc *d, double *total_ms, long *launches);
int csdr_amd_debug_ddc_mfma_tile(int D, int L, float shift_rate, const float *taps, long long n0, const uint8_t *window,
                                 const float *ctab3, float *out16);

typedef struct csdr_amd_nfm csdr_amd_nfm;
csdr_amd_nfm *csdr_amd_nfm_create(csdr_amd_ctx *ctx, int n_streams, float shift_rate, int decimation, const float *host_taps, int taps_length,
                                  int audio_rate, int agc_block, float agc_reference, float limit_max, size_t max_block_samples);
csdr_amd_nfm *csdr_amd_nfm_create_rates(csdr_amd_ctx *ctx, int n_streams, const float *shift_rates, int decimation, const float *host_taps, int taps_length,
                                        int audio_rate, int agc_block, float agc_reference, float limit_max, size_t max_block_samples);
int  csdr_amd_nfm_set_rate(csdr_amd_nfm *w, int stream, float shift_rate);
void csdr_amd_nfm_destroy(csdr_amd_nfm *w);
int  csdr_amd_nfm_reset(csdr_amd_nfm *w);
long csdr_amd_nfm_process(csdr_amd_nfm *w, const uint8_t *in, size_t in_pitch, size_t block_samples,
                          int16_t *audio_s16, float *audio_f, size_t out_pitch);
csdr_amd_ddc *csdr_amd_nfm_front_end(csdr_amd_nfm *w);

int csdr_amd_debug_wfm_seq_tile(int D, int L, int F, float shift_rate, const float *taps, long long n0, const uint8_t *window,
                                const float *ctab2, float *out16);
void csdr_amd_debug_dft16(const float *in32, float *out32, int inverse);
int  csdr_amd_debug_fftfilt_lds(int n, const float *taps_iq, int taps_len, const float *x_iq, long m_new, float *y_iq);
void csdr_amd_debug_dft8(const float *in16, float *out16, int inverse);
int  csdr_amd_debug_ddc_chain(int mode, float rate2, int post_in, int post_dec, int n_blocks, int *remain_io, float *phase_io, float *phases_out, int *count_out);
int csdr_amd_debug_nfm_deemph_tile(int audio_rate, float max_amp, const float *x, float *out16);
int csdr_amd_debug_waterfall_row(int fft_size, int every_n_samples, int window, int avgnumber, float add_db, int in_format, const void *in, long long n_in,
                                 float *db_row, float *power_row);
#ifdef __cplusplus
}
#endif
#endif
```

Baseline: 2.962 million.

## Add persistent walking grid to shared-rate WFM kernel when items exceed CUs

Adds a WALK variant of the shared-rate matrix-core WFM kernel in which each workgroup loops over several (stream-block, segment) items strided by the grid size. The fetch waves prefetch the next item's input rows into the LDS ring while the current item finishes, and output-ring and IIR state carry over between items. The launch path picks this variant by default when the number of items exceeds the CU count, or when a new max-workgroups knob is set. It aims to remove the per-workgroup ramp-up and the tail effects of a grid larger than the device. In exchange it adds considerable control-flow and state-carry complexity, and serializes items within a workgroup.

```diff
diff --git a/csdr_amd/__init__.py b/csdr_amd/__init__.py
--- a/csdr_amd/__init__.py
+++ b/csdr_amd/__init__.py
@@ -289,6 +289,8 @@
     L.csdr_amd_wfm_reset.argtypes = [vp]
     L.csdr_amd_wfm_process.restype = C.c_long; L.csdr_amd_wfm_process.argtypes = [vp, vp, sz, sz, vp, vp, sz]
     L.csdr_amd_wfm_kernel_name.restype = C.c_char_p; L.csdr_amd_wfm_kernel_name.argtypes = [vp]
+    L.csdr_amd_wfm_kernel_instance.restype = C.c_char_p; L.csdr_amd_wfm_kernel_instance.argtypes = [vp]
+    L.csdr_amd_wfm_set_max_workgroups.argtypes = [vp, i]
     ll = C.c_longlong; db = C.c_double
     L.csdr_amd_wfm_ring_create.restype = vp; L.csdr_amd_wfm_ring_create.argtypes = [vp, i, fl, i, vp, i, i, fl, i, sz, i]
     L.csdr_amd_wfm_ring_destroy.argtypes = [vp]; L.csdr_amd_wfm_ring_destroy.restype = None
diff --git a/csdr_amd/csrc/wfm.hip b/csdr_amd/csrc/wfm.hip
--- a/csdr_amd/csrc/wfm.hip
+++ b/csdr_amd/csrc/wfm.hip
@@ -174,6 +174,8 @@
     int last_T, flip;
     bool ended;
     std::string kernel_name;
+    const char *kernel_instance;
+    int max_workgroups;
     bool profiling;
     KernelTimer timer;
     double prof_ms; long prof_launches;
@@ -235,7 +237,7 @@
     }
     if (e != hipSuccess) { fail(e, "hipMalloc(wfm state)", __FILE__, __LINE__); return nullptr; }
     (void)hipMemcpy(w->d_taps.get(), host_taps, sizeof(float) * taps_length, hipMemcpyHostToDevice);
-    w->kernel_name = "k_wfm_front";
+    w->kernel_name = "k_wfm_front"; w->kernel_instance = "k_wfm_front"; w->max_workgroups = 0;
     if (w->use_mfma && per_stream) {
         WfmMfmaTable t;
         wfm_mfma_build_table(decimation, taps_length, frac_rate, shift_rate, host_taps, t);
@@ -329,6 +331,14 @@
 }
 
 const char *csdr_amd_wfm_kernel_name(const csdr_amd_wfm *w) { return w->kernel_name.c_str(); }
+const char *csdr_amd_wfm_kernel_instance(const csdr_amd_wfm *w) { return w->kernel_instance; }
+int csdr_amd_wfm_set_max_workgroups(csdr_amd_wfm *w, int n)
+{
+    if (n < 0) return fail_msg(-3, "wfm_set_max_workgroups: %d", n);
+    if (n > 0 && (w->ps || !w->use_mfma)) return fail_msg(-3, "wfm_set_max_workgroups: only the shared-rate matrix-core chain kernel walks");
+    w->max_workgroups = n;
+    return 0;
+}
 int csdr_amd_wfm_fallback(const csdr_amd_wfm *w) { return w->use_mfma ? 0 : 1; }
 
 int csdr_amd_wfm_set_profiling(csdr_amd_wfm *w, int on)
@@ -439,7 +449,8 @@
                 psa.d_lead_d = w->d_lead_d.get(); psa.d_lead_n = w->d_lead_n.get();
             }
         }
-        rc = wfm_mfma_launch(st, e0, e1, in, in_pitch, w->mfma, ctab_call, w->n_streams, T, w->B, w->next_j, n_audio, back, w->ps ? &psa : nullptr);
+        rc = wfm_mfma_launch(st, e0, e1, in, in_pitch, w->mfma, ctab_call, w->n_streams, T, w->B, w->next_j, n_audio, back, w->ps ? &psa : nullptr,
+                             w->max_workgroups, &w->kernel_instance);
         if (rc) return rc;
         if (n_audio > 0) w->retuned.clear();
         w->hflip ^= 1;
diff --git a/csdr_amd/csrc/wfm_mfma.hip b/csdr_amd/csrc/wfm_mfma.hip
--- a/csdr_amd/csrc/wfm_mfma.hip
+++ b/csdr_amd/csrc/wfm_mfma.hip
@@ -194,11 +194,12 @@
 __device__ __forceinline__ uint32_t sys_load(const uint32_t *p) { return __hip_atomic_load(p, __ATOMIC_RELAXED, __HIP_MEMORY_SCOPE_SYSTEM); }
 __device__ __forceinline__ uint32_t res_tag(long long k) { return (uint32_t)((unsigned long long)k % 0xfffffffeull) + 1u; }
 
-template <bool PS, bool RES = false>
+template <bool PS, bool RES = false, bool WALK = false>
 __global__ __launch_bounds__(64 * SEQ_NW) void k_wfm_mfma_seq(const uint8_t *__restrict__ in, size_t in_pitch, const v4i *__restrict__ frags, const float *__restrict__ cum,
                                                                const float2 *__restrict__ dtab, const float2 *__restrict__ ctab, SeqParams p_in, ResCtl rc)
 {
     static_assert(!(PS && RES), "the resident form exists for the shared-rate kernel");
+    static_assert(!(WALK && (PS || RES)), "the walk over a call's items exists for the plain shared-rate launch");
     constexpr int TPG = SEQ_TPG, SPW = 16 / SEQ_NLW, NTHR = 64 * SEQ_NW;
     extern __shared__ float4 lds_raw[];
     uint8_t *lds_in = reinterpret_cast<uint8_t *>(lds_raw);
@@ -206,9 +207,9 @@
     float *lcum = lds_out + 16 * SEQ_OUTP;
     float2 *ctl = reinterpret_cast<float2 *>(lcum + (SEQ_NGR + 1) * 16);
     const int tid = threadIdx.x, wv = __builtin_amdgcn_readfirstlane(tid >> 6), lane = tid & 63, col = lane & 15, q = lane >> 4;
-    const bool fetches = wv >= TPG;
+    const bool fetches_wave = wv >= TPG;
 #ifdef WFM_PROF
-    const long long t_entry = __builtin_readcyclecounter();
+    long long t_entry = __builtin_readcyclecounter();
     long long t_first = t_entry, t_last = t_entry;
 #endif
     const int fw = wv - TPG;
@@ -253,6 +254,29 @@
             }
         }
     };
+    const int w_wsb = WALK ? (p.n_streams + 15) / 16 : 1, w_seg = WALK ? (p.n_tiles + p.tiles_per_seg - 1) / p.tiles_per_seg : 1;
+    const int w_items = w_wsb * w_seg;
+    int w_item = WALK ? (int)blockIdx.x : 0;
+    long long w_G0 = 0;
+    int w_run = 0;
+    float w_yst_next = 0.f;
+    int f_item = w_item; long long fdel = 0;
+    const uint8_t *f_sblock = nullptr, *f_hblock = nullptr;
+    auto item_span = [&](int it, long long &wg0, long long &fe) {
+        const int sy = it / w_wsb;
+        const long long a0 = p.tile_first + (long long)sy * p.tiles_per_seg;
+        long long a1 = a0 + p.tiles_per_seg; if (a1 > p.tile_first + p.n_tiles) a1 = p.tile_first + p.n_tiles;
+        wg0 = (a0 - (sy > 0 ? 2LL * SEQ_TPG : 0LL)) * p.stride + p.win_off - p.B2;
+        fe = ((a1 - 1) * p.stride + p.win_off - p.B2 + 64 * WFM_NK + 1023) & ~1023LL;
+        const long long row_end = (p.two_T + 1023) & ~1023LL; if (fe > row_end) fe = row_end;
+    };
+    long long w_F = 0, w_F_end = 0; int w_fslot = 0;
+    uint32_t w_voff[SPW], w_voff_h[SPW];
+    int role = 0;
+#pragma unroll
+    do {
+    if (!WALK || fetches_wave == (role == 1)) {
+    const bool fetches = WALK ? role == 1 : fetches_wave;
     for (;;) {
     int res_slot = 0, res_lead = 0; long long res_k = 0; bool res_retuned = false;
     const uint8_t *pblock = nullptr;
@@ -330,8 +354,9 @@
         p_res.s16 = rc.out_ring + (size_t)res_slot * rc.out_slot_elems;
         if (tid == 0) (void)__hip_atomic_fetch_min(rc.t_first + res_slot, (unsigned long long)wall_clock64(), __ATOMIC_RELAXED, __HIP_MEMORY_SCOPE_AGENT);
     }
-    const int sb = RES ? (int)(item % (unsigned)rc.n_wsb) : (int)blockIdx.x;
-    const int seg_y = RES ? 0 : (int)blockIdx.y;
+    const int sb = RES ? (int)(item % (unsigned)rc.n_wsb) : (WALK ? w_item % w_wsb : (int)blockIdx.x);
+    const int seg_y = RES ? 0 : (WALK ? w_item / w_wsb : (int)blockIdx.y);
+    const bool w_first = !WALK || w_item == (int)blockIdx.x, w_next = WALK && w_item + (int)gridDim.x < w_items;
     const int col0 = PS ? 16 * seg_y : 0;
     if constexpr (RES) {
         in = rc.in_ring + (size_t)res_slot * rc.in_slot_bytes;
@@ -348,13 +373,32 @@
     const long long org = PS ? (long long)col0 * p.col_bytes : 0LL;
     long long wg = (t0 - (long long)n_warm * TPG) * tstride + p.win_off - p.B2 - org;
     const long long F0 = wg & ~1023LL;
-    long long F_end = ((t1 - 1) * tstride + p.win_off - p.B2 - org + 64 * WFM_NK + 1023) & ~1023LL;
-    { const long long row_end = ((p.two_T + 1023) & ~1023LL) - org; if (F_end > row_end) F_end = row_end; }
-    long long F = F0;
-    int fslot = (int)((F0 + 2 * SEQ_RB) % SEQ_RB), wslot = (int)((wg + 2 * SEQ_RB) % SEQ_RB);
+    long long F_end_i = ((t1 - 1) * tstride + p.win_off - p.B2 - org + 64 * WFM_NK + 1023) & ~1023LL;
+    { const long long row_end = ((p.two_T + 1023) & ~1023LL) - org; if (F_end_i > row_end) F_end_i = row_end; }
+    long long F_i = F0;
+    int fslot_i = (int)((F0 + 2 * SEQ_RB) % SEQ_RB), wslot = (int)((wg + 2 * SEQ_RB) % SEQ_RB);
     const uint32_t lds_in_addr = (uint32_t)(size_t)(__attribute__((address_space(3))) uint8_t *)lds_in;
-    uint32_t voff[SPW], voff_h[SPW];
+    uint32_t voff_i[SPW], voff_h_i[SPW];
     long long row_lim[SPW];
+    long long &F = *(WALK ? &w_F : &F_i), &F_end = *(WALK ? &w_F_end : &F_end_i); int &fslot = *(WALK ? &w_fslot : &fslot_i);
+    uint32_t (&voff)[SPW] = *(WALK ? &w_voff : &voff_i), (&voff_h)[SPW] = *(WALK ? &w_voff_h : &voff_h_i);
+    auto set_rows = [&](int sbx) {
+#pragma unroll
+        for (int r = 0; r < SPW; r++) {
+            const int srow = max(min(sbx * 16 + SPW * fw + r, last_stream) - sbx * 16, 0);
+            voff[r] = (uint32_t)srow * (uint32_t)in_pitch + 16u * lane;
+            voff_h[r] = (uint32_t)srow * (uint32_t)SEQ_HEAD + 16u * lane;
+        }
+        f_sblock = in + (long long)sbx * 16 * (long long)in_pitch; f_hblock = p.head_in + (size_t)sbx * 16 * SEQ_HEAD;
+    };
+    if constexpr (WALK) {
+        wslot = (int)(w_G0 % SEQ_RB) + (int)(wg & 1023);
+        if (fetches) {
+            wg = w_G0 + (wg & 1023);
+            if (w_first) { F = 0; fslot = 0; fdel = F0; F_end = F_end_i - F0; set_rows(sb); }
+        }
+    }
+    if constexpr (!WALK)
 #pragma unroll
     for (int r = 0; r < SPW; r++) {
         if constexpr (PS) {
@@ -403,11 +447,12 @@
             F += 1024; fslot += 1024; if (fslot >= SEQ_RB) fslot -= SEQ_RB;
             return;
         }
-        const bool head = F < 0;
-        const uint8_t *sbase = head ? hblock : sblock + F;
+        const long long Fr = WALK ? F + fdel : F;
+        const bool head = Fr < 0;
+        const uint8_t *sbase = head ? (WALK ? f_hblock : hblock) : (WALK ? f_sblock : sblock) + Fr;
         const uint32_t ldst = lds_in_addr + (SPW * fw) * SEQ_RP + (uint32_t)fslot;
         const bool mask = ragged && !head;
-        const bool live = !mask || F + 16 * lane < p.two_T;
+        const bool live = !mask || Fr + 16 * lane < p.two_T;
         if (!head && !ragged) dma_rows<SPW, SEQ_RP>(voff, sbase, __builtin_amdgcn_readfirstlane((int)ldst));
         else
 #pragma unroll
@@ -478,11 +523,32 @@
         }
         ps_load(wg + 2 * step_b);
     }
-    if (fetches) {
-        while (F < F_end && F + 1024 <= wg + SEQ_RB) row_step();
-        wait_for(wg + (long long)(TPG - 1) * tstride);
-    }
-    __syncthreads();
+    auto fill = [&](long long lim) {
+        if constexpr (WALK) {
+            for (;;) {
+                if (F >= F_end) {
+                    const int nx = f_item + (int)gridDim.x;
+                    if (nx >= w_items) break;
+                    long long w0, fe; item_span(nx, w0, fe);
+                    const long long f0 = w0 & ~1023LL;
+                    f_item = nx; fdel = f0 - F; F_end = F + (fe - f0); set_rows(nx % w_wsb);
+                }
+                if (F + 1024 > lim) break;
+                row_step();
+            }
+        } else
+            while (F < F_end && F + 1024 <= lim) row_step();
+    };
+    long long w_wg_next = 0;
+    if constexpr (WALK) if (w_next) { long long w0, fe; item_span(w_item + (int)gridDim.x, w0, fe); w_wg_next = w_G0 + (F_end_i - F0) + (w0 & 1023); }
+    const int obias = WALK ? (w_run + n_warm) % SEQ_OUTS + SEQ_OUTS : SEQ_OUTS;
+    if (w_first) {
+        if (fetches) {
+            fill(wg + SEQ_RB);
+            wait_for(wg + (long long)(TPG - 1) * tstride);
+        }
+        __syncthreads();
+    }
     const uint8_t *lrow = lds_in + col * SEQ_RP;
     const int s0 = sb * 16;
     float yst = 0.f;
@@ -496,8 +562,12 @@
     const float b2q = bp[QL] * bp[QL], b3q = b2q * bp[QL];
     float yst_first = 0.f;
     if (!RES && iir_wave && seg_y == 0) {
-        yst = p.last_in[PS ? sb : min(s0 + col, last_stream)]; if (yst != yst) yst = 0.f;
+        yst = (WALK && !w_first) ? w_yst_next : p.last_in[PS ? sb : min(s0 + col, last_stream)]; if (yst != yst) yst = 0.f;
         yst_first = yst;
+    }
+    if constexpr (WALK) {
+        const int nx = w_item + (int)gridDim.x;
+        if (iir_wave && w_next && nx / w_wsb == 0) w_yst_next = p.last_in[min((nx % w_wsb) * 16 + col, last_stream)];
     }
     if (RES && iir_wave && res_retuned) yst = rc.lead_state[min(s0 + col, last_stream)];
     const long long j_end = p.j_first + p.n_audio;
@@ -527,7 +597,7 @@
             const int srow = ei / SPS, k = ei % SPS, kr = g * SPS + k;
             if (ei >= 16 * SPS) continue;
             if (PS ? (kr < col_lo(srow) || kr >= col_hi(srow)) : (kr < seg_lo || kr >= seg_hi || s0 + srow >= p.n_streams)) continue;
-            const float e = lds_out[srow * SEQ_OUTP + (g % SEQ_OUTS) * SPS + k];
+            const float e = lds_out[srow * SEQ_OUTP + (WALK ? (g + obias) % SEQ_OUTS : g % SEQ_OUTS) * SPS + k];
             const long long idx = idx0 + kr;
             const size_t at = PS ? (size_t)sb * p.out_pitch + (size_t)srow * p.col_audio + idx : (size_t)(s0 + srow) * p.out_pitch + idx;
             p.s16[at] = (int16_t)s16_of(e);
@@ -575,7 +645,7 @@
             const float *src = lds_out + srow * SEQ_OUTP;
             float e[8];
 #pragma unroll
-            for (int i = 0; i < 8; i++) e[i] = src[(n0 + i + SEQ_OUTR) % SEQ_OUTR];
+            for (int i = 0; i < 8; i++) e[i] = src[(n0 + i + obias * SPS) % SEQ_OUTR];
             int v[8];
 #pragma unroll
             for (int i = 0; i < 8; i++) v[i] = s16_of(e[i]);
@@ -606,12 +676,14 @@
 #endif
         for (int gi = -n_warm; gi < n_grp; gi++) {
             PROF_T(0)
-            const long long wg_n = wg + (long long)TPG * tstride;
-            if (gi + 1 < n_grp) wait_for(wg_n + (long long)(TPG - 1) * tstride);
+            long long wg_n = wg + (long long)TPG * tstride;
+            bool more = gi + 1 < n_grp;
+            if constexpr (WALK) if (!more && w_next) { wg_n = w_wg_next; more = true; }
+            if (more) wait_for(wg_n + (long long)(TPG - 1) * tstride);
             PROF_T(1)
             __syncthreads();
             PROF_T(2)
-            if (gi + 1 < n_grp) { while (F < F_end && F + 1024 <= wg_n + SEQ_RB) row_step(); }
+            if (more) fill(wg_n + SEQ_RB);
             PROF_T(3)
             if (WFM_DIAG < 4) take_line(gi - 1);
             PROF_T(4)
@@ -634,7 +706,7 @@
 #endif
     for (int gi = -n_warm; gi < n_grp; gi++) {
         const int it = gi * TPG + wv;
-        float *lout = lds_out + ((gi + SEQ_OUTS) % SEQ_OUTS) * SPS;
+        float *lout = lds_out + ((gi + obias) % SEQ_OUTS) * SPS;
         if (it < n_it && (WFM_DIAG < 3)) {
             const long long ws = wg + (long long)wv * tstride;
             const long long n0 = (ws + p.B2) >> 1;
@@ -773,7 +845,17 @@
             *reinterpret_cast<uint4 *>(p.head_out + (size_t)sb * SEQ_HEAD + 512 + 16 * tid) = v;
         }
     } else
-    if (!PS && !RES && seg_y + 1 == (int)gridDim.y) {
+    if (WALK && seg_y + 1 == w_seg) {
+        if (iir_lane && s0 + lane < p.n_streams) p.last_out[s0 + lane] = yst;
+        if (tid >= 64 && tid < 64 * TPG && p.two_T >= 512 && (p.two_T & 15) == 0)
+            for (int e = tid - 64; e < 16 * 32; e += 64 * (TPG - 1)) {
+                const int srow = e / 32, piece = e % 32;
+                if (s0 + srow >= p.n_streams) continue;
+                const uint4 v = *reinterpret_cast<const uint4 *>(sblock + (size_t)srow * in_pitch + (p.two_T - 512) + 16 * piece);
+                *reinterpret_cast<uint4 *>(p.head_out + (size_t)(s0 + srow) * SEQ_HEAD + 512 + 16 * piece) = v;
+            }
+    } else
+    if (!PS && !RES && !WALK && seg_y + 1 == (int)gridDim.y) {
         if (iir_lane && s0 + lane < p.n_streams) p.last_out[s0 + lane] = yst;
         if (tid < 16 * 32 && p.two_T >= 512 && (p.two_T & 15) == 0 && s0 + tid / 32 < p.n_streams) {
             const int srow = tid / 32, piece = tid % 32;
@@ -783,12 +865,18 @@
     }
 #ifdef WFM_PROF
     if (lane == 0) {
-        asm volatile("s_waitcnt vmcnt(0)" ::: "memory");
+        if constexpr (!WALK) asm volatile("s_waitcnt vmcnt(0)" ::: "memory");
         const long long t_exit = __builtin_readcyclecounter();
         atomicAdd(&g_wfm_life[wv][0], (unsigned long long)(t_first - t_entry)); atomicAdd(&g_wfm_life[wv][1], (unsigned long long)(t_last - t_first));
         atomicAdd(&g_wfm_life[wv][2], (unsigned long long)(t_exit - t_last)); atomicAdd(&g_wfm_life[wv][3], 1ULL);
-    }
-#endif
+        t_entry = t_exit;
+    }
+#endif
+    if constexpr (WALK) {
+        w_G0 += F_end_i - F0; w_run = (w_run + n_warm + n_grp) % SEQ_OUTS;
+        w_item += (int)gridDim.x;
+        if (w_item >= w_items) break;
+    } else
     if constexpr (!RES) break;
     else {
         if (tid == 0) { const long long t = wall_clock64(); st_body += t - st_t; st_t = t; }
@@ -813,6 +901,8 @@
         if (tid == 0) { const long long t = wall_clock64(); st_done += t - st_t; st_t = t; st_items++; }
     }
     }
+    }
+    } while (WALK && ++role < 2);
 }
 
 __global__ __launch_bounds__(256) void k_wfm_roll_head(const uint8_t *__restrict__ in, size_t in_pitch, long long two_T, const uint8_t *__restrict__ head_in, uint8_t *__restrict__ head_out)
@@ -901,8 +991,9 @@
 }
 
 int wfm_mfma_launch(hipStream_t st, hipEvent_t ev_begin, hipEvent_t ev_end, const uint8_t *in, size_t in_pitch, const WfmMfmaDevice &dev, const float2 *ctab,
-                    int n_streams, int T, long long B, long long j_first, int n_audio, const WfmBackArgs &back, const WfmPerStream *ps)
-{
+                    int n_streams, int T, long long B, long long j_first, int n_audio, const WfmBackArgs &back, const WfmPerStream *ps, int max_workgroups, const char **instance)
+{
+    if (instance) *instance = "k_wfm_roll_head";
     if (in_pitch * 16 + 4096 >= ((size_t)1 << 32)) return fail_msg(-3, "wfm: in_pitch %zu too large for the matrix-core front end (32-bit row offsets)", in_pitch);
     if (n_audio <= 0) {
         hipLaunchKernelGGL(k_wfm_roll_head, dim3(n_streams), dim3(256), 0, st, in, in_pitch, 2LL * T, back.head_in, back.head_out);
@@ -941,6 +1032,7 @@
         if (sp.col_bytes * 16 + 4096 >= (1LL << 32)) return fail_msg(-3, "wfm: block too large for the per-stream kernel's 32-bit row offsets");
         const size_t ldsp = (size_t)16 * SEQ_RP + 16 * SEQ_OUTP * sizeof(float) + (SEQ_NGR + 1) * 16 * sizeof(float) + 2 * 48 * sizeof(float2);
         { const int arc = lds_attr_once((const void *)k_wfm_mfma_seq<true>, ldsp); if (arc) return arc; }
+        if (instance) *instance = "k_wfm_mfma_seq<true, false, false>";
         if (ev_begin && ev_end)
             hipExtLaunchKernelGGL(k_wfm_mfma_seq<true>, dim3(n_streams, n_seg), dim3(64 * SEQ_NW), ldsp, st, ev_begin, ev_end, 0, in, in_pitch, (const v4i *)dev.d_seq_frags, dev.d_seq_cum, dev.d_dtab, ctab, sp, no_res);
         else
@@ -953,7 +1045,24 @@
         return 0;
     }
     const size_t lds = (size_t)16 * SEQ_RP + 16 * SEQ_OUTP * sizeof(float) + (SEQ_NGR + 1) * 16 * sizeof(float);
+    const int n_items = n_wsb * n_seg;
+    if (max_workgroups > 0 || n_items > n_cu) {
+        int grid = max_workgroups > 0 ? max_workgroups : n_cu; if (grid > n_items) grid = n_items;
+        { const int arc = lds_attr_once((const void *)k_wfm_mfma_seq<false, false, true>, lds); if (arc) return arc; }
+        if (instance) *instance = "k_wfm_mfma_seq<false, false, true>";
+        if (ev_begin && ev_end)
+            hipExtLaunchKernelGGL((k_wfm_mfma_seq<false, false, true>), dim3(grid), dim3(64 * SEQ_NW), lds, st, ev_begin, ev_end, 0, in, in_pitch, (const v4i *)dev.d_seq_frags, dev.d_seq_cum, dev.d_dtab, ctab, sp, no_res);
+        else
+            hipLaunchKernelGGL((k_wfm_mfma_seq<false, false, true>), dim3(grid), dim3(64 * SEQ_NW), lds, st, in, in_pitch, (const v4i *)dev.d_seq_frags, dev.d_seq_cum, dev.d_dtab, ctab, sp, no_res);
+        CSDR_LAUNCH_CHECK();
+        if (T < 256 || (T & 7)) {
+            hipLaunchKernelGGL(k_wfm_roll_head, dim3(n_streams), dim3(256), 0, st, in, in_pitch, 2LL * T, back.head_in, back.head_out);
+            CSDR_LAUNCH_CHECK();
+        }
+        return 0;
+    }
     { const int arc = lds_attr_once((const void *)k_wfm_mfma_seq<false>, lds); if (arc) return arc; }
+    if (instance) *instance = "k_wfm_mfma_seq<false, false, false>";
     if (ev_begin && ev_end)
         hipExtLaunchKernelGGL(k_wfm_mfma_seq<false>, dim3(n_wsb, n_seg), dim3(64 * SEQ_NW), lds, st, ev_begin, ev_end, 0, in, in_pitch, (const v4i *)dev.d_seq_frags, dev.d_seq_cum, dev.d_dtab, ctab, sp, no_res);
     else
diff --git a/csdr_amd/csrc/wfm_mfma.hpp b/csdr_amd/csrc/wfm_mfma.hpp
--- a/csdr_amd/csrc/wfm_mfma.hpp
+++ b/csdr_amd/csrc/wfm_mfma.hpp
@@ -47,7 +47,8 @@
 void wfm_mfma_build_table(int D, int L, int F, float shift_rate, const float *taps, WfmMfmaTable &t);
 size_t wfm_mfma_head_bytes(int n_streams);
 int wfm_mfma_launch(hipStream_t st, hipEvent_t ev_begin, hipEvent_t ev_end, const uint8_t *in, size_t in_pitch, const WfmMfmaDevice &dev, const float2 *ctab,
-                    int n_streams, int T, long long B, long long j_first, int n_audio, const WfmBackArgs &back, const WfmPerStream *ps = nullptr);
+                    int n_streams, int T, long long B, long long j_first, int n_audio, const WfmBackArgs &back, const WfmPerStream *ps = nullptr,
+                    int max_workgroups = 0, const char **instance = nullptr);
 int wfm_mfma_lead(hipStream_t st, const uint8_t *in, size_t in_pitch, const uint8_t *head, const float *d_taps, const float2 *ctab, size_t tab_pitch, const float2 *d_dtab,
                   const float2 *d_dtab_old, const int *d_list, int n_list, float *d_lead_d, int lead_stride, int D, int L, int F, long long B, long long j_first, int n_lead);
 
diff --git a/include/csdr_amd.h b/include/csdr_amd.h
--- a/include/csdr_amd.h
+++ b/include/csdr_amd.h
@@ -402,6 +402,8 @@
 long csdr_amd_wfm_process(csdr_amd_wfm *w, const uint8_t *in, size_t in_pitch, size_t block_samples,
                           int16_t *audio_s16, float *audio_f, size_t out_pitch);
 const char *csdr_amd_wfm_kernel_name(const csdr_amd_wfm *w);
+const char *csdr_amd_wfm_kernel_instance(const csdr_amd_wfm *w);
+int csdr_amd_wfm_set_max_workgroups(csdr_amd_wfm *w, int n);
 int csdr_amd_wfm_fallback(const csdr_amd_wfm *w);
 int csdr_amd_wfm_set_profiling(csdr_amd_wfm *w, int on);
 int csdr_amd_wfm_kernel_time(csdr_amd_wfm *w, double *total_ms, long *launches);
```

Result: slower. 2.915 million (-1.6%).
